# rapidsai/cuvs

Measured on AMD Instinct MI355X. Metric: QPS @ recall@10>=0.9, 100Mx128 fp32 IVF-PQ, batch=10k, higher is better.
Workload: dtype u8 codes, f16 LUT, f32 score; 1 GPU; IVF-PQ 100000000x128 fp32, pq_dim=64 pq_bits=8 n_lists=16384 n_probes=128 batch=10000 k=10; rows and held-out queries from bench.gen_rows (seed 1234 / 4321): Gaussian mixture of 65536 modes ~ N(0, I) in a 32-d latent space, spread 0.35 per mode, embedded in R^128 by a fixed random map + N(0, 0.03^2 I) - NOT SURVEY 8d's generator: the same step on that one is the top-level entry contract_corpus (--; parallelism=single GPU, lut_dtype=f16, internal_distance_dtype=f32

## Files before the change

### cuvs_amd/csrc/common.hpp

```cpp
#pragma once

#include <hip/hip_runtime.h>
#include <hip/hip_fp16.h>

#include <dlpack/dlpack.h>

#include <cstdarg>
#include <cstdint>
#include <cstdio>
#include <cstring>
#include <memory>
#include <stdexcept>
#include <string>
#include <chrono>
#include <vector>

namespace cuvs_amd {

struct error : public std::runtime_error {
  explicit error(const std::string& s) : std::runtime_error(s) {}
};

[[noreturn]] inline void fail(const char* file, int line, const char* fmt, ...)
{
  char buf[1024];
  va_list ap;
  va_start(ap, fmt);
  vsnprintf(buf, sizeof(buf), fmt, ap);
  va_end(ap);
  char out[1200];
  snprintf(out, sizeof(out), "%s (%s:%d)", buf, file, line);
  throw error(out);
}

#define CUVS_EXPECTS(cond, ...)                                              \
  do {                                                                       \
    if (!(cond)) { ::cuvs_amd::fail(__FILE__, __LINE__, __VA_ARGS__); }      \
  } while (0)
#define CUVS_FAIL(...) ::cuvs_amd::fail(__FILE__, __LINE__, __VA_ARGS__)
#define HIP_TRY(expr)                                                                        \
  do {                                                                                       \
    hipError_t e__ = (expr);                                                                 \
    if (e__ != hipSuccess) {                                                                 \
      ::cuvs_amd::fail(__FILE__, __LINE__, "HIP error %d (%s) in %s", (int)e__,              \
                       hipGetErrorString(e__), #expr);                                       \
    }                                                                                        \
  } while (0)

std::string& last_error_text();

template <typename Fn>
int translate_exceptions(Fn&& fn)
{
  try {
    fn();
    return 1;
  } catch (const std::exception& e) {
    last_error_text() = e.what();
    return 0;
  } catch (...) {
    last_error_text() = "unknown exception";
    return 0;
  }
}

struct tuning {
  int pq_head_probes    = -1;
  int pq_scan2          = 1;
  int pq_scan3          = 1;
  int coarse_lowp       = 1;
  int pq_head_rows      = -1;
  int pq_overlap        = 1;
  int coarse_grouped    = 1;
  int pq_filter4        = 1;
  int flat_scan3        = 1;
  int flat_filter2      = 1;
  int flat_bound_head   = 1;
  int pq_wide           = 1;
  int pq_wide_heads     = 0;
  int pq_wide_blocks    = 1;
  bool pq_encode_plain  = false;
  int pq3_surv_cap      = 0;
  int pq_qcap           = 0;
  int scan_debug        = 0;
  int alloc_cache       = 1;
  bool shard_coarse_replicated = false;
  bool bf_fused = false, bf_no_threshold = false, bf_no_fused_filter = false;
  bool bf_host_flags = false;
  bool dist_old         = false;
  int tile_dbg          = 0;
  int flat_head_probes  = -1;
  int cagra_pq_lists = 0, cagra_pq_probes = 0, cagra_kpq = 0, cagra_rank_chunk = 0, prune_dbg = 0;
  bool cagra_auto_multi = false;
  int tiered_path       = 0;
  bool native_format    = false;
  int hnsw_pack_rows    = 0;
  int hnsw_pack_host    = 0;
  int eps_slab_rows     = 0;
};
tuning load_tuning_from_env();

struct resources {
  tuning tune;
  int device              = 0;
  hipStream_t stream      = nullptr;
  bool owns_stream        = false;
  int num_cus             = 256;
  size_t lds_per_block    = 160 * 1024;
  size_t workspace_limit  = size_t(2) << 30;
  size_t ivf_batch_limit  = size_t(8) << 30;
  std::vector<int> mg_devices;
  hipMemPool_t pool       = nullptr;
  hipStream_t aux_stream  = nullptr;
  hipEvent_t aux_events[5] = {nullptr, nullptr, nullptr, nullptr, nullptr};
  bool cagra_guarantee_connectivity = false;
  uint32_t* host_word = nullptr;
  unsigned long long* cagra_work = nullptr;
  struct scratch_cache* cache = nullptr;
};

inline resources* as_res(uintptr_t h)
{
  CUVS_EXPECTS(h != 0, "null cuvsResources_t");
  return reinterpret_cast<resources*>(h);
}

void ensure_aux_stream(resources& res);
void* device_alloc(resources& res, size_t bytes);
void device_free(resources& res, void* p);
void scratch_cache_flush_all();

template <typename T>
struct dev_buf {
  resources* res = nullptr;
  T* ptr         = nullptr;
  size_t n       = 0;
  dev_buf() = default;
  dev_buf(resources& r, size_t count) : res(&r), n(count)
  {
    ptr = count ? static_cast<T*>(device_alloc(r, count * sizeof(T))) : nullptr;
  }
  static dev_buf persistent(size_t count)
  {
    dev_buf b;
    b.n = count;
    if (count) {
      void* p = nullptr;
      if (hipMalloc(&p, count * sizeof(T)) != hipSuccess) {
        (void)hipGetLastError();
        scratch_cache_flush_all();
        HIP_TRY(hipMalloc(&p, count * sizeof(T)));
      }
      b.ptr = static_cast<T*>(p);
    }
    return b;
  }
  dev_buf(const dev_buf&)            = delete;
  dev_buf& operator=(const dev_buf&) = delete;
  dev_buf(dev_buf&& o) noexcept : res(o.res), ptr(o.ptr), n(o.n) { o.ptr = nullptr; o.n = 0; }
  dev_buf& operator=(dev_buf&& o) noexcept
  {
    if (this != &o) {
      release();
      res = o.res; ptr = o.ptr; n = o.n;
      o.ptr = nullptr; o.n = 0;
    }
    return *this;
  }
  ~dev_buf() { release(); }
  void release()
  {
    if (ptr) {
      if (res) device_free(*res, ptr); else (void)hipFree(ptr);
      ptr = nullptr; n = 0;
    }
  }
  T* data() const { return ptr; }
  size_t size() const { return n; }
  size_t bytes() const { return n * sizeof(T); }
};

inline void copy_async(resources& res, void* dst, const void* src, size_t bytes)
{
  if (bytes) HIP_TRY(hipMemcpyAsync(dst, src, bytes, hipMemcpyDefault, res.stream));
}
inline void sync(resources& res) { HIP_TRY(hipStreamSynchronize(res.stream)); }

template <typename T>
std::vector<T> to_host(resources& res, const T* d, size_t n)
{
  std::vector<T> h(n);
  copy_async(res, h.data(), d, n * sizeof(T));
  sync(res);
  return h;
}

inline uint32_t read_word(resources& res, const uint32_t* d)
{
  if (res.host_word == nullptr) HIP_TRY(hipHostMalloc(reinterpret_cast<void**>(&res.host_word), 64));
  HIP_TRY(hipMemcpyAsync(res.host_word, d, sizeof(uint32_t), hipMemcpyDeviceToHost, res.stream));
  sync(res);
  return *res.host_word;
}

struct host_trace {
  bool on;
  const char* what;
  std::vector<std::pair<const char*, std::chrono::steady_clock::time_point>> marks;
  host_trace(bool enabled, const char* name) : on(enabled), what(name) { mark("begin"); }
  void mark(const char* name)
  {
    if (on) marks.emplace_back(name, std::chrono::steady_clock::now());
  }
  ~host_trace()
  {
    if (!on) return;
    mark("buffers freed");
    fprintf(stderr, "[host trace %s]", what);
    for (size_t i = 1; i < marks.size(); ++i)
      fprintf(stderr, " %s %.3f", marks[i].first, std::chrono::duration<double, std::milli>(marks[i].second - marks[i - 1].second).count());
    fprintf(stderr, " | total %.3f ms\n", std::chrono::duration<double, std::milli>(marks.back().second - marks.front().second).count());
  }
};

inline bool is_device_accessible(const DLTensor& t)
// ... 94 lines not shown
```

### cuvs_amd/csrc/core.hip

```cpp
#include <cuvs/version_config.h>
#include "common.hpp"

#include <cuvs/core/c_api.h>

#include "scratch_cache.hpp"

#include <algorithm>
#include <cstdlib>
#include <mutex>
#include <vector>

namespace cuvs_amd {

std::string& last_error_text()
{
  thread_local std::string text;
  return text;
}

namespace {

void* raw_alloc(resources& res, size_t bytes, bool* failed)
{
  void* p = nullptr;
  hipError_t e = res.pool != nullptr ? hipMallocFromPoolAsync(&p, bytes, res.pool, res.stream)
                                     : hipMallocAsync(&p, bytes, res.stream);
  if (e != hipSuccess) {
    (void)hipGetLastError();
    if (failed != nullptr) { *failed = true; return nullptr; }
    HIP_TRY(hipStreamSynchronize(res.stream));
    HIP_TRY(hipMalloc(&p, bytes));
  }
  return p;
}

void raw_free(void* stream_v, void* p)
{
  hipStream_t stream = static_cast<hipStream_t>(stream_v);
  hipError_t e = hipFreeAsync(p, stream);
  if (e != hipSuccess) {
    (void)hipGetLastError();
    (void)hipStreamSynchronize(stream);
    (void)hipFree(p);
  }
}

}

unsigned long long g_pq3_last_stats[6] = {0, 0, 0, 0, 0, 0};

static void flush_cache(scratch_cache& c)
{
  if (!c.caller_stream) { c.flush(raw_free); return; }
  bool drained = false;
  c.flush([&](void*, void* p) {
    if (!drained) { (void)hipDeviceSynchronize(); drained = true; }
    (void)hipFree(p);
    (void)hipGetLastError();
  });
}
void scratch_cache_flush(resources& res)
{
  if (res.cache != nullptr) flush_cache(*res.cache);
}

namespace {
std::mutex g_caches_mu;
std::vector<scratch_cache*> g_caches;
}
void scratch_cache_register(scratch_cache* c, bool add)
{
  std::lock_guard<std::mutex> lk(g_caches_mu);
  if (add) g_caches.push_back(c);
  else g_caches.erase(std::remove(g_caches.begin(), g_caches.end(), c), g_caches.end());
}
void scratch_cache_flush_all()
{
  {
    std::lock_guard<std::mutex> lk(g_caches_mu);
    for (scratch_cache* c : g_caches) flush_cache(*c);
  }
  (void)hipDeviceSynchronize();
  (void)hipGetLastError();
}

void ensure_aux_stream(resources& res)
{
  if (res.aux_stream != nullptr) return;
  int lo = 0, hi = 0;
  HIP_TRY(hipDeviceGetStreamPriorityRange(&lo, &hi));
  HIP_TRY(hipStreamCreateWithPriority(&res.aux_stream, hipStreamNonBlocking, hi));
  for (auto& ev : res.aux_events) HIP_TRY(hipEventCreateWithFlags(&ev, hipEventDisableTiming));
}

void* device_alloc(resources& res, size_t bytes)
{
  if (res.cache == nullptr) return raw_alloc(res, bytes, nullptr);
  return res.cache->alloc(
    res.stream, bytes, [&](size_t n, bool* failed) { return raw_alloc(res, n, failed); }, raw_free);
}

void device_free(resources& res, void* p)
{
  if (!p) return;
  if (res.cache == nullptr) raw_free(res.stream, p);
  else res.cache->release(res.stream, p, raw_free);
}

void fill_dl_view(DLManagedTensor* out, void* data, DLDataType dt, int64_t rows, int64_t cols,
                  int ndim, int device_id)
{
  CUVS_EXPECTS(out != nullptr, "output DLManagedTensor is null");
  out->dl_tensor.data        = data;
  out->dl_tensor.device      = DLDevice{kDLCUDA, device_id};
  out->dl_tensor.ndim        = ndim;
  out->dl_tensor.dtype       = dt;
  out->dl_tensor.shape       = new int64_t[2]{rows, cols};
  out->dl_tensor.strides     = nullptr;
  out->dl_tensor.byte_offset = 0;
  out->manager_ctx           = nullptr;
  out->deleter               = [](DLManagedTensor* self) {
    delete[] self->dl_tensor.shape;
    self->dl_tensor.shape = nullptr;
  };
}

static int g_log_level = CUVS_LOG_LEVEL_INFO;

struct prof_rec {
  std::string name;
  hipEvent_t start, stop;
};
static bool g_prof_on = false;
static std::vector<prof_rec> g_prof;
static std::mutex g_prof_mu;

void profile_begin(resources& res, const char* name)
{
  if (!g_prof_on) return;
  std::lock_guard<std::mutex> lk(g_prof_mu);
  prof_rec r;
  r.name = name;
  HIP_TRY(hipEventCreate(&r.start));
  HIP_TRY(hipEventCreate(&r.stop));
  HIP_TRY(hipEventRecord(r.start, res.stream));
  g_prof.push_back(r);
}
void profile_end(resources& res, const char* name)
{
  if (!g_prof_on) return;
  std::lock_guard<std::mutex> lk(g_prof_mu);
  for (auto it = g_prof.rbegin(); it != g_prof.rend(); ++it)
    if (it->name == name) { HIP_TRY(hipEventRecord(it->stop, res.stream)); return; }
}

static bool debug_switches_on()
{
#ifdef CUVS_AMD_NO_DEBUG_SWITCHES
  return false;
#else
  const char* g = getenv("CUVS_AMD_DEBUG_SWITCHES");
  return g != nullptr && g[0] == '1';
#endif
}

tuning load_tuning_from_env()
{
  tuning t;
  if (!debug_switches_on()) return t;
  auto geti = [](const char* name, int dflt) { const char* e = getenv(name); return e ? atoi(e) : dflt; };
  auto set  = [](const char* name) { return getenv(name) != nullptr; };
  t.pq_head_probes   = geti("CUVS_AMD_PQ_HEAD_PROBES", -1);
  t.pq_scan2         = geti("CUVS_AMD_PQ_SCAN2", 1);
  t.pq_scan3         = geti("CUVS_AMD_PQ_SCAN3", 1);
  t.pq_filter4       = geti("CUVS_AMD_PQ_FILTER4", 1);
  t.coarse_grouped   = geti("CUVS_AMD_COARSE_GROUPED", 1);
  t.pq_overlap       = geti("CUVS_AMD_PQ_OVERLAP", 1);
  t.pq_head_rows     = geti("CUVS_AMD_PQ_HEAD_ROWS", -1);
  t.coarse_lowp      = geti("CUVS_AMD_COARSE_LOWP", 1);
  t.flat_scan3       = geti("CUVS_AMD_FLAT_SCAN3", 1);
  t.flat_filter2     = geti("CUVS_AMD_FLAT_FILTER2", 1);
  t.flat_bound_head  = geti("CUVS_AMD_FLAT_BOUND_HEAD", 1);
  t.pq_wide          = geti("CUVS_AMD_PQ_WIDE", 1);
  t.pq_wide_heads    = geti("CUVS_AMD_PQ_WIDE_HEADS", 0);
  t.pq_wide_blocks   = geti("CUVS_AMD_PQ_WIDE_BLOCKS", 1);
  if (const char* e = getenv("CUVS_AMD_PQ_ENCODE")) t.pq_encode_plain = strcmp(e, "plain") == 0;
  t.pq3_surv_cap     = geti("CUVS_AMD_PQ3_SURV_CAP", 0);
  t.pq_qcap          = geti("CUVS_AMD_PQ_QCAP", 0);
  t.scan_debug       = geti("CUVS_AMD_SCAN_DEBUG", 0);
  t.alloc_cache      = geti("CUVS_AMD_ALLOC_CACHE", 1);
  t.shard_coarse_replicated = set("CUVS_AMD_SHARD_COARSE_REPLICATED");
  t.bf_fused           = set("CUVS_AMD_BF_FUSED");
  t.bf_no_threshold    = set("CUVS_AMD_BF_NO_THRESHOLD");
  t.bf_no_fused_filter = set("CUVS_AMD_BF_NO_FUSED_FILTER");
  t.bf_host_flags = set("CUVS_AMD_BF_HOST_FLAGS");
  t.dist_old           = set("CUVS_AMD_DIST_OLD");
  t.tile_dbg           = geti("CUVS_AMD_TILE_DBG", 0);
  t.flat_head_probes   = geti("CUVS_AMD_FLAT_HEAD_PROBES", -1);
  t.cagra_pq_lists     = geti("CUVS_AMD_CAGRA_PQ_LISTS", 0);
  t.cagra_pq_probes    = geti("CUVS_AMD_CAGRA_PQ_PROBES", 0);
  t.cagra_kpq          = geti("CUVS_AMD_CAGRA_KPQ", 0);
  t.cagra_rank_chunk   = geti("CUVS_AMD_CAGRA_RANK_CHUNK", 0);
  t.prune_dbg          = geti("CUVS_AMD_PRUNE_DBG", 0);
  if (const char* e = getenv("CUVS_AMD_CAGRA_AUTO")) t.cagra_auto_multi = e[0] == 'm';
  if (const char* e = getenv("CUVS_AMD_TIERED_PATH")) t.tiered_path = strcmp(e, "composed") == 0 ? 1 : (strcmp(e, "fused") == 0 ? 2 : 0);
  if (const char* e = getenv("CUVS_AMD_NATIVE_FORMAT")) t.native_format = e[0] == '1';
  t.hnsw_pack_rows   = geti("CUVS_AMD_HNSW_PACK_ROWS", 0);
  t.hnsw_pack_host   = geti("CUVS_AMD_HNSW_PACK_HOST", 0);
  t.eps_slab_rows    = geti("CUVS_AMD_EPS_SLAB_ROWS", 0);
  return t;
}

}

using namespace cuvs_amd;

extern "C" {

const char* cuvsGetLastErrorText()
{
  auto& t = last_error_text();
  return t.empty() ? nullptr : t.c_str();
}

void cuvsSetLastErrorText(const char* error) { last_error_text() = error ? error : ""; }

cuvsLogLevel_t cuvsGetLogLevel() { return (cuvsLogLevel_t)g_log_level; }
void cuvsSetLogLevel(cuvsLogLevel_t l) { g_log_level = (int)l; }

cuvsError_t cuvsResourcesCreate(cuvsResources_t* res)
{
  return (cuvsError_t)translate_exceptions([=] {
    CUVS_EXPECTS(res != nullptr, "res is null");
    auto* r = new resources();
    int dev = 0;
    HIP_TRY(hipGetDevice(&dev));
    r->device = dev;
    hipDeviceProp_t prop;
    HIP_TRY(hipGetDeviceProperties(&prop, dev));
    r->num_cus       = prop.multiProcessorCount;
    r->lds_per_block = prop.sharedMemPerBlock;
    HIP_TRY(hipStreamCreateWithFlags(&r->stream, hipStreamDefault));
    r->owns_stream = true;
    r->tune = load_tuning_from_env();
    {
      size_t free_b = 0, total_b = 0;
      if (hipMemGetInfo(&free_b, &total_b) == hipSuccess && free_b > 0)
        r->ivf_batch_limit = std::max<size_t>(size_t(256) << 20, std::min<size_t>(r->ivf_batch_limit, free_b / 4));
      else
        (void)hipGetLastError();
    }
    if (const char* ws = debug_switches_on() ? getenv("CUVS_AMD_WORKSPACE_MB") : nullptr) {
      long mb = atol(ws);
      if (mb > 0) r->workspace_limit = r->ivf_batch_limit = (size_t)mb << 20;
    }
    hipMemPoolProps props{};
    props.allocType     = hipMemAllocationTypePinned;
    props.handleTypes   = hipMemHandleTypeNone;
    props.location.type = hipMemLocationTypeDevice;
    props.location.id   = dev;
    if (hipMemPoolCreate(&r->pool, &props) == hipSuccess) {
      uint64_t thresh = UINT64_MAX;
      (void)hipMemPoolSetAttribute(r->pool, hipMemPoolAttrReleaseThreshold, &thresh);
    } else {
      r->pool = nullptr;
    }
    (void)hipGetLastError();
    if (r->tune.alloc_cache != 0) {
      r->cache         = new scratch_cache();
      scratch_cache_register(r->cache, true);
      r->cache->stream = r->stream;
      size_t free_b = 0, total_b = 0;
      if (hipMemGetInfo(&free_b, &total_b) != hipSuccess) { (void)hipGetLastError(); total_b = size_t(64) << 30; }
      r->cache->cap_bytes = std::min<size_t>(total_b / 8, size_t(16) << 30);
      if (const char* mb = debug_switches_on() ? getenv("CUVS_AMD_ALLOC_CACHE_MB") : nullptr) r->cache->cap_bytes = (size_t)std::max(0L, atol(mb)) << 20;
    }
    *res = reinterpret_cast<uintptr_t>(r);
  });
}

static std::mutex g_handle_teardown_mu;

cuvsError_t cuvsResourcesDestroy(cuvsResources_t res)
{
  return (cuvsError_t)translate_exceptions([=] {
    auto* r = as_res(res);
    (void)hipStreamSynchronize(r->stream);
    std::lock_guard<std::mutex> teardown(g_handle_teardown_mu);
    if (r->aux_stream != nullptr) {
      (void)hipStreamSynchronize(r->aux_stream);
      (void)hipStreamDestroy(r->aux_stream);
      for (auto& e : r->aux_events) if (e != nullptr) (void)hipEventDestroy(e);
    }
    if (r->cagra_work != nullptr) (void)hipFree(r->cagra_work);
    if (r->host_word != nullptr) (void)hipHostFree(r->host_word);
    if (r->cache != nullptr) {
      scratch_cache_flush(*r);
      (void)hipStreamSynchronize(r->stream);
      scratch_cache_register(r->cache, false);
      delete r->cache;
      r->cache = nullptr;
    }
    if (r->pool != nullptr) (void)hipMemPoolDestroy(r->pool);
    if (r->owns_stream && r->stream) (void)hipStreamDestroy(r->stream);
    delete r;
  });
}

cuvsError_t cuvsStreamSet(cuvsResources_t res, cudaStream_t stream)
{
  return (cuvsError_t)translate_exceptions([=] {
    auto* r = as_res(res);
    if (r->cache != nullptr) {
      scratch_cache_flush(*r);
      if (r->owns_stream) HIP_TRY(hipStreamSynchronize(r->stream));
    }
    if (r->owns_stream && r->stream) {
      HIP_TRY(hipStreamSynchronize(r->stream));
      HIP_TRY(hipStreamDestroy(r->stream));
    }
    r->stream      = reinterpret_cast<hipStream_t>(stream);
    r->owns_stream = false;
    if (r->cache != nullptr) {
      std::lock_guard<std::mutex> lk(r->cache->mu);
      r->cache->stream        = r->stream;
      r->cache->caller_stream = true;
    }
  });
}

// ... 197 lines not shown
```

### cuvs_amd/csrc/ivf_pq_filter4.hip

```cpp
#include "ivf_pq_filter_common.hpp"

#include <cfloat>
#include <type_traits>

namespace cuvs_amd {

namespace {

struct bprep_params {
  const uint32_t* sorted_pairs;
  const uint32_t* pair_off;
  uint32_t n_lists;
  uint32_t lbase;
  const uint32_t* probes;
  const float* rot_queries;
  const float* centers_rot;
  const uint32_t* query_kth;
  uint32_t* qflag;
  uint4* bq;
  float* thr;
  uint32_t n_probes, rot_dim;
  float sc, c1, eps, alpha, cbmax, dmax, bound_max;
  int is_ip, flat;
  uint32_t lpl;
  float4* norms;
};

template <int NST, int PART>
__global__ __launch_bounds__(256) void pq_bprep_kernel(const bprep_params a)
{
  constexpr uint32_t LPP = 2 * NST <= 2 ? 2u : 2 * NST <= 4 ? 4u : 2 * NST <= 8 ? 8u : 2 * NST <= 16 ? 16u : 32u;
  constexpr uint32_t PPW = 64u / LPP;
  const uint32_t s_base = a.pair_off[a.lbase], s_end = a.pair_off[a.lbase + a.n_lists];
  const uint32_t lane = threadIdx.x & 63u, slot = lane % LPP, st = slot >> 1, h = slot & 1u;
  const uint32_t w0 = (blockIdx.x * 4u + (threadIdx.x >> 6)) * 32u;
  if (s_base + w0 >= s_end) return;
  const uint32_t d0 = ((16u * (st >> a.lpl) + 8u * h) << a.lpl) + 8u * (st & ((1u << a.lpl) - 1u));
#pragma unroll 2
  for (uint32_t pass = 0; pass < 32u / PPW; ++pass) {
    const uint32_t s  = s_base + w0 + pass * PPW + lane / LPP;
    const bool pair_ok = s < s_end;
    const bool valid  = pair_ok && slot < 2u * NST;
    const uint32_t p  = a.sorted_pairs[pair_ok ? s : s_end - 1u];
    const uint32_t q  = p / a.n_probes, L = a.probes[p];
    float rn = 0.f, big = 0.f, qc = 0.f, cn = 0.f;
    if (valid) {
      const float* rq = a.rot_queries + (size_t)q * a.rot_dim + d0;
      const float* ct = a.centers_rot + (size_t)L * a.rot_dim + d0;
      const float4 q0 = *reinterpret_cast<const float4*>(rq), q1 = *reinterpret_cast<const float4*>(rq + 4);
      float r[8] = {q0.x, q0.y, q0.z, q0.w, q1.x, q1.y, q1.z, q1.w};
      const float4 c0 = *reinterpret_cast<const float4*>(ct), c1 = *reinterpret_cast<const float4*>(ct + 4);
      const float c[8] = {c0.x, c0.y, c0.z, c0.w, c1.x, c1.y, c1.z, c1.w};
      if (!a.is_ip) {
#pragma unroll
        for (int e = 0; e < 8; ++e) r[e] -= c[e];
      } else {
#pragma unroll
        for (int e = 0; e < 8; ++e) { qc = __fmaf_rn(r[e], c[e], qc); cn = __fmaf_rn(c[e], c[e], cn); }
      }
      f16x8_t v;
#pragma unroll
      for (int e = 0; e < 8; ++e) {
        rn   = __fmaf_rn(r[e], r[e], rn);
        const float x = a.sc * r[e];
        big  = fmaxf(big, fabsf(x));
        v[e] = (_Float16)fminf(fmaxf(x, -60000.f), 60000.f);
      }
      a.bq[(size_t)(s - s_base) * NST * 2 + slot] = __builtin_bit_cast(uint4, v);
    }
#pragma unroll
    for (uint32_t o = 1; o < LPP; o <<= 1) {
      rn += __shfl_xor(rn, o); qc += __shfl_xor(qc, o); cn += __shfl_xor(cn, o);
      big = fmaxf(big, __shfl_xor(big, o));
    }
    if (!pair_ok || slot != 0u) continue;
    if constexpr (PART == 1) {
      a.norms[s - s_base] = make_float4(rn, cn, qc, big);
    } else {
      const uint32_t kk = a.query_kth[q];
      const float bound = key_to_float(kk);
      const bool served = kk < 0xff800000u && big < 60000.f && fabsf(bound) <= a.bound_max;
      if (!a.flat && !served) a.qflag[q] = 1u;
      const float t = a.is_ip ? filter_threshold_ip(bound, rn, cn, qc, a) : filter_threshold(bound, rn, a);
      a.thr[s - s_base] = served ? t / a.c1 : (a.flat ? -INFINITY : INFINITY);
    }
  }
}

__global__ __launch_bounds__(256) void pq_thr_kernel(const bprep_params a)
{
  const uint32_t s_base = a.pair_off[a.lbase], s_end = a.pair_off[a.lbase + a.n_lists];
  const uint32_t s = s_base + blockIdx.x * 256u + threadIdx.x;
  if (s >= s_end) return;
  const uint32_t q  = a.sorted_pairs[s] / a.n_probes;
  const float4 nm   = a.norms[s - s_base];
  const float rn = nm.x, cn = nm.y, qc = nm.z, big = nm.w;
  const uint32_t kk = a.query_kth[q];
  const float bound = key_to_float(kk);
  const bool served = kk < 0xff800000u && big < 60000.f && fabsf(bound) <= a.bound_max;
  if (!a.flat && !served) a.qflag[q] = 1u;
  const float t = a.is_ip ? filter_threshold_ip(bound, rn, cn, qc, a) : filter_threshold(bound, rn, a);
  a.thr[s - s_base] = served ? t / a.c1 : (a.flat ? -INFINITY : INFINITY);
}

constexpr int kF4Threads = 256;
constexpr uint32_t kSurvChunk = 256u;

struct filter4_params {
  const filter_unit* units;
  const uint32_t* n_units;
  uint32_t* xcd_ticket;
  const uint32_t* sorted_pairs;
  const uint32_t* pair_off;
  uint32_t n_lists;
  const uint4* bq;
  const float* thr;
  const uint32_t* cb16;
  const uint8_t* codes;
  const uint32_t* list_offsets;
  const uint32_t* list_sizes;
  const float* row_term;
  uint32_t* qflag;
  uint2* surv;
  uint32_t* surv_cnt;
  uint32_t n_chunks, n_probes, unit_rows;
  unsigned long long* stats;
};

template <int BYTE>
__device__ inline void table_addr(uint32_t& addr, const uint32_t two, const uint32_t w)
{
  if constexpr (BYTE == 0)
    asm("v_lshlrev_b32_sdwa %0, %1, %2 dst_sel:WORD_0 dst_unused:UNUSED_PRESERVE src0_sel:DWORD src1_sel:BYTE_0" : "+v"(addr) : "v"(two), "v"(w));
  else if constexpr (BYTE == 1)
    asm("v_lshlrev_b32_sdwa %0, %1, %2 dst_sel:WORD_0 dst_unused:UNUSED_PRESERVE src0_sel:DWORD src1_sel:BYTE_1" : "+v"(addr) : "v"(two), "v"(w));
  else if constexpr (BYTE == 2)
    asm("v_lshlrev_b32_sdwa %0, %1, %2 dst_sel:WORD_0 dst_unused:UNUSED_PRESERVE src0_sel:DWORD src1_sel:BYTE_2" : "+v"(addr) : "v"(two), "v"(w));
  else
    asm("v_lshlrev_b32_sdwa %0, %1, %2 dst_sel:WORD_0 dst_unused:UNUSED_PRESERVE src0_sel:DWORD src1_sel:BYTE_3" : "+v"(addr) : "v"(two), "v"(w));
}

typedef __attribute__((address_space(3))) const uint32_t lds_u32_t;

template <int NCH, int PL, bool TERM, int DBG, bool STATS = false, bool PC = false>
__global__ __launch_bounds__(kF4Threads) void pq_filter4_kernel(const filter4_params a)
{
  constexpr int NST = PL * NCH;
  constexpr int NGM = NST <= 8 ? 4 : 2;
  constexpr int NGA = 8 / PL;
  constexpr uint32_t kEntry = 2u * PL;
  constexpr uint32_t kSlot  = 256u * kEntry;
  constexpr uint32_t kHalf1 = 65536u;
  extern __shared__ __attribute__((aligned(16))) char smem[];
  uint32_t s_chunk = 0xffffffffu, s_fill = kSurvChunk;
  for (uint32_t i = threadIdx.x; i < (PC ? 0u : (uint32_t)NCH * 16u * (kSlot / 16u)); i += kF4Threads) {
    const uint32_t s = i / (kSlot / 16u), half = (s >> 3) & 1u, slot = (s >> 4) * 8u + (s & 7u);
    *reinterpret_cast<uint4*>(smem + half * kHalf1 + slot * kSlot + (i % (kSlot / 16u)) * 16u) = reinterpret_cast<const uint4*>(a.cb16)[i];
  }
  __syncthreads();

  const uint32_t lane = threadIdx.x & 63u, ql = lane & 31u, h = lane >> 5;
  const uint32_t n_units = *a.n_units;
  const uint32_t chunk   = (n_units + 7u) / 8u;
  const uint32_t s_base  = a.pair_off[a.n_lists];
  uint32_t xcd = blockIdx.x & 7u, hops = 0u;
  const uint32_t two = PL == 1 ? 1u : PL == 2 ? 2u : PL == 4 ? 3u : 4u;
  const uint32_t lane_code_off = ql * 16u + h * 8u, lane_term_off = h * 16u;

  unsigned long long st_pairs = 0, st_surv = 0, st_sub = 0, st_slow = 0, st_units = 0, st_t[3] = {0, 0, 0};
  uint32_t tk_v = 0u;
  uint4 d0 = {0u, 0u, 0u, 0u};
  uint2 d1 = {0u, 0u};
  bool desc_ok = false;
  auto draw_ticket = [&]() {
    if (lane == 0) tk_v = atomicAdd(a.xcd_ticket + xcd * 32, 1u);
  };
  auto load_desc = [&]() {
    const uint32_t share0 = min(n_units, xcd * chunk), share_len = min(chunk, n_units - share0);
    const uint32_t t = __builtin_amdgcn_readfirstlane(tk_v);
    desc_ok = t < share_len;
    if (desc_ok) {
      const filter_unit* up = a.units + share0 + t;
      d0 = *reinterpret_cast<const uint4*>(up);
      d1 = *reinterpret_cast<const uint2*>(reinterpret_cast<const char*>(up) + 16);
    }
  };
  draw_ticket();
  load_desc();
  for (;;) {
    while (!desc_ok) {
      if (++hops == 8u) break;
      xcd = (xcd + 1u) & 7u;
      draw_ticket();
      load_desc();
    }
    if (!desc_ok) break;
    if constexpr (PC) {
      const uint32_t list = __builtin_amdgcn_readfirstlane(d0.x);
      const uint4* src    = reinterpret_cast<const uint4*>(a.cb16) + (size_t)list * (kSlot / 16u);
      char* dst           = smem + (threadIdx.x >> 6) * 4096u;
#pragma unroll
      for (uint32_t i = 0; i < (kSlot / 16u + 63u) / 64u; ++i)
        if (i * 64u + lane < kSlot / 16u) *reinterpret_cast<uint4*>(dst + (i * 64u + lane) * 16u) = src[i * 64u + lane];
    }
    const uint32_t first = __builtin_amdgcn_readfirstlane(d0.y), count = __builtin_amdgcn_readfirstlane(d0.z),
                   row0 = __builtin_amdgcn_readfirstlane(d0.w), base_row = __builtin_amdgcn_readfirstlane(d1.x),
                   r_end = __builtin_amdgcn_readfirstlane(d1.y);
    const uint32_t u0 = row0 >> 5, u1 = (r_end + 31u) >> 5;
    const unsigned long long t_unit = STATS ? __builtin_readcyclecounter() : 0ull;
    unsigned long long t_loop = 0ull;
    draw_ticket();
    bool desc_pending = true;
    const char* code_base = reinterpret_cast<const char*>(a.codes) + (size_t)(base_row >> 6) * NCH * 1024;
    const char* term_base = reinterpret_cast<const char*>(a.row_term + base_row);

    auto load_codes = [&](const uint32_t u, uint2 (&cw)[NCH]) {
      uint32_t uc = min(u, u1 - 1u);
      if constexpr ((DBG & 64) != 0) uc = u0;
      const char* p = code_base + ((size_t)(uc >> 1) * NCH * 1024 + (uc & 1u) * 512u) + lane_code_off;
#pragma unroll
      for (int c = 0; c < NCH; ++c) {
        if constexpr ((DBG & 8) != 0) cw[c] = make_uint2(u * 2654435761u + c, lane);
        else cw[c] = *reinterpret_cast<const uint2*>(p + c * 1024);
      }
    };
    uint32_t ad[NGA];
#pragma unroll
    for (int e = 0; e < NGA; ++e) ad[e] = h << 16;
    auto decode_addr = [&](const uint2 (&cw)[NCH], const int st) {
      const int c = st / PL, b0 = (st % PL) * NGA;
      if constexpr (PC) {
        const uint32_t base = (threadIdx.x >> 6) * 4096u;
#pragma unroll
        for (int e = 0; e < NGA; ++e) {
          const int b = b0 + e;
          const uint32_t w = b < 4 ? cw[c].x : cw[c].y;
          ad[e] = base + (((w >> (8 * (b & 3))) & 255u) << two);
        }
        return;
      }
      if constexpr ((DBG & 1) != 0) {
        const uint32_t w = ql * 0x01010101u;
        if constexpr (NGA >= 1) table_addr<0>(ad[0], two, w);
        if constexpr (NGA >= 2) table_addr<1>(ad[1], two, w);
        if constexpr (NGA >= 4) { table_addr<2>(ad[2], two, w); table_addr<3>(ad[3], two, w); }
        return;
      }
      auto one = [&](const int e) {
        const int b = b0 + e;
        const uint32_t w = b < 4 ? cw[c].x : cw[c].y;
        switch (b & 3) {
          case 0: table_addr<0>(ad[e], two, w); break;
          case 1: table_addr<1>(ad[e], two, w); break;
          case 2: table_addr<2>(ad[e], two, w); break;
          default: table_addr<3>(ad[e], two, w); break;
        }
      };
#pragma unroll
      for (int e = 0; e < NGA; ++e) one(e);
    };
    auto decode_gather = [&](const int st, u32x4_t (&av)[NST]) {
      constexpr uint32_t kNone = 0u;
      const uint32_t slot0 = PC ? 0u : (8u * (st / PL) + (uint32_t)((st % PL) * NGA)) * kSlot;
      constexpr uint32_t kStep = PC ? 0u : kSlot;
      if constexpr ((DBG & 2) != 0) {
#pragma unroll
        for (int e = 0; e < 4; ++e) av[st][e] = ad[e % NGA] + kNone;
        return;
      }
      if constexpr (PL == 1) {
        typedef __attribute__((address_space(3))) const _Float16 lds_f16_t;
        f16x8_t v;
#pragma unroll
        for (int e = 0; e < 8; ++e) v[e] = *reinterpret_cast<lds_f16_t*>(ad[e] + slot0 + e * kStep);
        av[st] = __builtin_bit_cast(u32x4_t, v);
      } else if constexpr (PL == 2) {
#pragma unroll
        for (int e = 0; e < 4; ++e) av[st][e] = *reinterpret_cast<lds_u32_t*>(ad[e] + slot0 + e * kStep);
      } else if constexpr (PL == 4) {
        typedef uint32_t u32x2_t __attribute__((ext_vector_type(2)));
        typedef __attribute__((address_space(3))) const u32x2_t lds_u64_t;
#pragma unroll
        for (int e = 0; e < 2; ++e) {
          const u32x2_t v = *reinterpret_cast<lds_u64_t*>(ad[e] + slot0 + e * kStep);
          av[st][2 * e] = v[0]; av[st][2 * e + 1] = v[1];
        }
      } else {
        typedef __attribute__((address_space(3))) const u32x4_t lds_u128_t;
        av[st] = *reinterpret_cast<lds_u128_t*>(ad[0] + slot0);
      }
    };
    auto decode_step = [&](const uint2 (&cw)[NCH], const int st, u32x4_t (&av)[NST]) {
      decode_addr(cw, st);
      decode_gather(st, av);
    };
    auto load_term = [&](const uint32_t u, f32x16_t& tv) {
      if constexpr (!TERM) { tv = f32x16_t{}; return; }
      uint32_t uc = min(u, u1 - 1u);
      if constexpr ((DBG & 16) != 0) uc = u0;
      const char* p = term_base + (size_t)uc * 128u + lane_term_off;
#pragma unroll
      for (int j = 0; j < 4; ++j) {
        const float4 v = *reinterpret_cast<const float4*>(p + j * 32);
        tv[4 * j] = v.x; tv[4 * j + 1] = v.y; tv[4 * j + 2] = v.z; tv[4 * j + 3] = v.w;
      }
    };

    auto run = [&](auto ng_tag) {
      constexpr int NG = decltype(ng_tag)::value;
      f16x8_t bop[NG][NST];
      float thr[NG];
      uint32_t pairid[NG];
#pragma unroll
      for (int g = 0; g < NG; ++g) {
        const uint32_t jj  = g * 32u + ql;
        const uint32_t jc  = min(jj, count - 1u);
        const uint4* bp    = a.bq + ((size_t)(first - s_base + jc) * NST * 2 + h);
#pragma unroll
        for (int st = 0; st < NST; ++st) bop[g][st] = __builtin_bit_cast(f16x8_t, bp[st * 2]);
        thr[g]    = jj < count ? a.thr[first - s_base + jc] : INFINITY;
        pairid[g] = a.sorted_pairs[first + jc];
      }
      uint2 cw[4][NCH];
      u32x4_t av[2][NST];
      f32x16_t tv[2], acc[2][NG];
#pragma unroll
      for (int k = 0; k < 4; ++k) load_codes(u0 + k, cw[k]);
      load_term(u0, tv[0]);
      load_term(u0 + 1, tv[1]);
#pragma unroll
      for (int g = 0; g < NG; ++g)
#pragma unroll
        for (int st = 0; st < NST; ++st) {
          asm volatile("" : "+a"(bop[g][st]));
        }
#pragma unroll
      for (int st = 0; st < NST; ++st) decode_step(cw[0], st, av[0]);
      load_codes(u0 + 4, cw[0]);
      if (STATS) t_loop = __builtin_readcyclecounter();

      unsigned long long gmask[NG];
      auto screen_group = [&](const f32x16_t (&ac)[NG], const int g, const bool valid) {
        float m = fmaxf(fmaxf(ac[g][0], ac[g][1]), ac[g][2]);
#pragma unroll
        for (int i = 3; i < 15; i += 2) m = fmaxf(fmaxf(m, ac[g][i]), ac[g][i + 1]);
        m        = fmaxf(m, ac[g][15]);
        gmask[g] = valid ? __ballot(m >= thr[g]) : 0ull;
      };
      auto screen_finish = [&](const f32x16_t (&ac)[NG], const uint32_t u, const bool valid) {
        unsigned long long any_mask = 0ull;
#pragma unroll
        for (int g = 0; g < NG; ++g) any_mask |= gmask[g];
        if (STATS && valid) { st_pairs += 32u * count; st_sub += 1u; }
        if (any_mask == 0ull) return;
        if (STATS) st_slow += 1u;
#pragma unroll
        for (int g = 0; g < NG; ++g) {
          if (gmask[g] == 0ull) continue;
          uint32_t hits = 0u;
#pragma unroll
          for (int i = 0; i < 16; ++i) hits |= (ac[g][i] >= thr[g] ? 1u : 0u) << i;
          unsigned long long lm = gmask[g];
          while (lm != 0ull) {
            const uint32_t src = (uint32_t)__ffsll((long long)lm) - 1u;
            lm &= lm - 1ull;
            uint32_t hb        = __builtin_amdgcn_readlane(hits, src);
            const uint32_t pid = __builtin_amdgcn_readlane(pairid[g], src);
            while (hb != 0u) {
              const uint32_t i = (uint32_t)__ffs((int)hb) - 1u;
              hb &= hb - 1u;
              const uint32_t v = (u << 5) + (i & 3u) + 8u * (i >> 2) + 4u * (src >> 5);
              if (v >= r_end) continue;
              if (s_fill == kSurvChunk) {
                uint32_t c = 0u;
                if (lane == 0u) c = atomicAdd(a.surv_cnt, 1u);
                s_chunk = __builtin_amdgcn_readfirstlane(c);
                s_fill  = 0u;
              }
              if (s_chunk < a.n_chunks) {
                if (lane == 0u) a.surv[(size_t)s_chunk * kSurvChunk + s_fill] = make_uint2(pid, base_row + v);
              } else if (lane == 0u) {
                a.qflag[pid / a.n_probes] = 1u;
              }
              s_fill += 1u;
              if (STATS) st_surv += 1u;
            }
          }
        }
      };
      auto step = [&](auto p_tag, const uint32_t u) {
        constexpr int P = decltype(p_tag)::value;
        constexpr int C = P & 1, N = (P + 1) & 1, S = (P + 1) & 3;
        const bool prev = u > u0 && u <= u1;
        auto part_chunk = [](const int p) { return p + 1 < NST ? p + 1 : NST - 1; };
#pragma unroll
        for (int st = 0; st < NST; ++st) {
          const f16x8_t aop = __builtin_bit_cast(f16x8_t, av[C][st]);
          auto mfma = [&](const int g) {
            if constexpr ((DBG & 4) != 0) {
              if (st == 0) acc[C][g] = tv[C];
              acc[C][g][st & 15] += (float)aop[0] * (float)bop[g][st][0];
            } else {
              acc[C][g] = __builtin_amdgcn_mfma_f32_32x32x16_f16(aop, bop[g][st], st == 0 ? tv[C] : acc[C][g], 0, 0, 0);
            }
            __builtin_amdgcn_sched_barrier(0);
          };
          mfma(0);
          if (st == 1) load_term(u + 2, tv[C]);
          decode_addr(cw[S], st);
          __builtin_amdgcn_sched_barrier(0);
          if constexpr (NG >= 2) mfma(1);
          decode_gather(st, av[N]);
          if (st == NST - 1) load_codes(u + 5, cw[S]);
          __builtin_amdgcn_sched_barrier(0);
          if constexpr (NG >= 3) mfma(2);
#pragma unroll
          for (int p = 0; p < NG; ++p)
            if (part_chunk(p) == st) screen_group(acc[N], p, prev);
          if (part_chunk(NG) == st) screen_finish(acc[N], u - 1u, prev);
          __builtin_amdgcn_sched_barrier(0);
          if constexpr (NG >= 4) mfma(3);
        }
        if constexpr (NST == 1) load_term(u + 2, tv[C]);
      };
      using P0 = std::integral_constant<int, 0>; using P1 = std::integral_constant<int, 1>;
      using P2 = std::integral_constant<int, 2>; using P3 = std::integral_constant<int, 3>;
      uint32_t u = u0;
      for (; u < u1; u += 4u) {
        step(P0{}, u);
        step(P1{}, u + 1u);
        step(P2{}, u + 2u);
        step(P3{}, u + 3u);
        if (desc_pending && u >= u0 + 4u) { load_desc(); desc_pending = false; }
      }
      if (u == u1) {
#pragma unroll
        for (int g = 0; g < NG; ++g) screen_group(acc[1], g, true);
        screen_finish(acc[1], u - 1u, true);
      }
    };
    if (u0 < u1) {
      const uint32_t ng = (count + 31u) >> 5;
      if constexpr (NGM == 4) {
        if (ng >= 4u) run(std::integral_constant<int, 4>{});
        else if (ng == 3u) run(std::integral_constant<int, 3>{});
        else if (ng == 2u) run(std::integral_constant<int, 2>{});
        else run(std::integral_constant<int, 1>{});
      } else {
        if (ng >= 2u) run(std::integral_constant<int, 2>{});
        else run(std::integral_constant<int, 1>{});
      }
    }
    if (desc_pending) load_desc();
    if (STATS) {
      const unsigned long long t_end = __builtin_readcyclecounter();
      st_t[0] += t_loop - t_unit;
      st_t[1] += t_end - t_loop;
      st_units += 1u;
    }
  }
  if (STATS && lane == 0) {
    atomicAdd(&a.stats[1], st_surv);
    atomicAdd(&a.stats[0], st_pairs); atomicAdd(&a.stats[2], st_sub);
    atomicAdd(&a.stats[3], st_slow);  atomicAdd(&a.stats[4], st_t[0]); atomicAdd(&a.stats[5], st_t[1]);
    atomicAdd(&a.stats[6], st_t[2]);  atomicAdd(&a.stats[7], st_units);
  }
  if (s_chunk < a.n_chunks)
    for (uint32_t i = s_fill + lane; i < kSurvChunk; i += 64u) a.surv[(size_t)s_chunk * kSurvChunk + i] = make_uint2(0xffffffffu, 0u);
}

}

void pq4_filter(resources& res, const filter4_launch& l)
{
  bprep_params b{};
  b.sorted_pairs = l.sorted_pairs; b.pair_off = l.pair_off; b.n_lists = l.n_lists; b.probes = l.probes;
  b.rot_queries = l.rot_queries; b.centers_rot = l.centers_rot; b.query_kth = l.query_kth; b.qflag = l.qflag;
  b.bq = static_cast<uint4*>(l.bq); b.thr = l.thr; b.n_probes = l.n_probes; b.rot_dim = l.rot_dim;
  b.sc = l.sc; b.c1 = l.c1; b.eps = l.eps; b.alpha = l.alpha; b.cbmax = l.cbmax; b.dmax = l.dmax; b.bound_max = l.bound_max;
  b.is_ip = l.is_ip; b.flat = l.flat; b.lbase = l.head_labels ? 0u : l.n_lists;
  b.lpl = l.pl == 1 ? 0u : l.pl == 2 ? 1u : l.pl == 4 ? 2u : 3u;
  const int nst = l.nch * l.pl;
  const unsigned pgrid = (unsigned)grid_blocks(l.n_pairs, 128);
  b.norms = static_cast<float4*>(l.pair_norms);
  if (l.stage != 2) {
    profile_begin(res, "pq_bprep_kernel");
    auto prep = [&](auto nst_tag) {
      constexpr int N = decltype(nst_tag)::value;
      if (l.stage == 1) hipLaunchKernelGGL((pq_bprep_kernel<N, 1>), dim3(pgrid), dim3(256), 0, res.stream, b);
      else              hipLaunchKernelGGL((pq_bprep_kernel<N, 0>), dim3(pgrid), dim3(256), 0, res.stream, b);
    };
    switch (nst) {
#ifndef CUVS_AMD_F4_DEV
      case 1: prep(std::integral_constant<int, 1>{}); break;
      case 2: prep(std::integral_constant<int, 2>{}); break;
      case 3: prep(std::integral_constant<int, 3>{}); break;
      case 4: prep(std::integral_constant<int, 4>{}); break;
      case 5: prep(std::integral_constant<int, 5>{}); break;
      case 6: prep(std::integral_constant<int, 6>{}); break;
      case 7: prep(std::integral_constant<int, 7>{}); break;
      case 10: prep(std::integral_constant<int, 10>{}); break;
      case 12: prep(std::integral_constant<int, 12>{}); break;
      case 14: prep(std::integral_constant<int, 14>{}); break;
      case 16: prep(std::integral_constant<int, 16>{}); break;
#endif
      default: prep(std::integral_constant<int, 8>{}); break;
    }
    profile_end(res, "pq_bprep_kernel");
    HIP_TRY(hipGetLastError());
    if (l.stage == 1 || l.bprep_only) return;
  } else {
    hipLaunchKernelGGL(pq_thr_kernel, dim3((unsigned)grid_blocks(l.n_pairs, 256)), dim3(256), 0, res.stream, b);
  }
  filter4_params g{};
  g.units = l.units; g.n_units = l.n_units; g.xcd_ticket = l.xcd_ticket; g.sorted_pairs = l.sorted_pairs; g.pair_off = l.pair_off;
  g.n_lists = l.n_lists; g.bq = b.bq; g.thr = l.thr; g.cb16 = l.cb16; g.codes = l.codes; g.list_offsets = l.list_offsets;
  g.list_sizes = l.list_sizes; g.row_term = l.row_term; g.qflag = l.qflag; g.surv = static_cast<uint2*>(l.surv);
  g.surv_cnt = l.surv_cnt; g.n_chunks = l.surv_entries / kSurvChunk; g.n_probes = l.n_probes; g.unit_rows = l.unit_rows;
  g.stats = l.stats;
  const size_t fsmem = l.per_cluster ? 4 * 4096 : 65536 + (size_t)l.nch * 8 * 512 * l.pl;
  const bool term = l.row_term != nullptr;
  auto launch = [&](auto kern) {
    HIP_TRY(hipFuncSetAttribute(reinterpret_cast<const void*>(kern), hipFuncAttributeMaxDynamicSharedMemorySize, (int)fsmem));
    profile_begin(res, "pq_filter_kernel");
    hipLaunchKernelGGL(kern, dim3(l.grid), dim3(kF4Threads), fsmem, res.stream, g);
    profile_end(res, "pq_filter_kernel");
  };
#ifndef CUVS_AMD_F4_DEV
  if (l.nch == 4 && l.pl == 2 && !l.per_cluster) {
    switch (l.dbg) {
      case 1:  launch(pq_filter4_kernel<4, 2, true, 1>); break;
      case 2:  launch(pq_filter4_kernel<4, 2, true, 2>); break;
      case 4:  launch(pq_filter4_kernel<4, 2, true, 4>); break;
      case 8:  launch(pq_filter4_kernel<4, 2, true, 8>); break;
      case 16: launch(pq_filter4_kernel<4, 2, true, 16>); break;
      case 64: launch(pq_filter4_kernel<4, 2, true, 64>); break;
      case 80: launch(pq_filter4_kernel<4, 2, true, 80>); break;
      case 81: launch(pq_filter4_kernel<4, 2, true, 81>); break;
      default:
        if (l.stats != nullptr && term) launch(pq_filter4_kernel<4, 2, true, 0, true>);
        else if (term) launch(pq_filter4_kernel<4, 2, true, 0>);
        else launch(pq_filter4_kernel<4, 2, false, 0>);
        break;
    }
    return;
  }
  auto pick = [&](auto nch_tag, auto pl_tag) {
    constexpr int N = decltype(nch_tag)::value, P = decltype(pl_tag)::value;
    if (l.per_cluster) {
      if (term) launch(pq_filter4_kernel<N, P, true, 0, false, true>); else launch(pq_filter4_kernel<N, P, false, 0, false, true>);
    } else {
      if (term) launch(pq_filter4_kernel<N, P, true, 0>); else launch(pq_filter4_kernel<N, P, false, 0>);
    }
  };
  using N1 = std::integral_constant<int, 1>; using N2 = std::integral_constant<int, 2>; using N3 = std::integral_constant<int, 3>;
  using N4 = std::integral_constant<int, 4>; using N5 = std::integral_constant<int, 5>; using N6 = std::integral_constant<int, 6>;
  using N7 = std::integral_constant<int, 7>; using N8 = std::integral_constant<int, 8>;
  CUVS_EXPECTS(nst >= 1 && nst <= 16 && l.nch >= 1 && l.nch <= 8, "ivf_pq: shape outside the matrix-core filter (pq3_supported)");
  if (l.pl == 2) {
    switch (l.nch) {
      case 1: pick(N1{}, N2{}); break;
      case 2: pick(N2{}, N2{}); break;
      case 3: pick(N3{}, N2{}); break;
      case 4: pick(N4{}, N2{}); break;
      case 5: pick(N5{}, N2{}); break;
      case 6: pick(N6{}, N2{}); break;
      case 7: pick(N7{}, N2{}); break;
      default: pick(N8{}, N2{}); break;
    }
  } else if (l.pl == 1) {
    switch (l.nch) {
      case 1: pick(N1{}, N1{}); break;
      case 2: pick(N2{}, N1{}); break;
      case 3: pick(N3{}, N1{}); break;
      case 4: pick(N4{}, N1{}); break;
      case 5: pick(N5{}, N1{}); break;
      case 6: pick(N6{}, N1{}); break;
      case 7: pick(N7{}, N1{}); break;
      default: pick(N8{}, N1{}); break;
    }
  } else if (l.pl == 4) {
    switch (l.nch) {
      case 1: pick(N1{}, N4{}); break;
      case 2: pick(N2{}, N4{}); break;
      case 3: pick(N3{}, N4{}); break;
      default: pick(N4{}, N4{}); break;
    }
  } else {
    if (l.nch == 1) pick(N1{}, N8{}); else pick(N2{}, N8{});
  }
#else
  launch(pq_filter4_kernel<4, 2, true, 0>);
#endif
}

}
```

### cuvs_amd/csrc/ivf_pq_filter_common.hpp

```cpp
#pragma once
#include "ivf_pq.hpp"
#include "device_utils.hpp"

#include <cmath>

namespace cuvs_amd {

typedef _Float16 f16x8_t __attribute__((ext_vector_type(8)));
typedef float f32x16_t __attribute__((ext_vector_type(16)));
typedef uint32_t u32x4_t __attribute__((ext_vector_type(4)));

struct filter_unit {
  uint32_t list, first, count, row0;
  uint32_t base_row, r_end;
  uint32_t pad0, pad1;
};

template <typename P>
__device__ inline float filter_threshold(const float bound, const float rn, const P& a)
{
  const double mabs = 1.1920929e-07  / (double)a.sc *
                      (sqrt((double)a.rot_dim * (double)rn) + (double)a.rot_dim * (double)a.cbmax);
  const double b = ((double)bound + (double)a.alpha) * (1.0 + 2.0 * (double)a.eps) + mabs - (double)rn * (1.0 - 1.0 / 512.0);
  float f = (float)b;
  f += fabsf(f) * 2.4e-7f + 1e-37f;
  return f;
}

template <typename P>
__device__ inline float filter_threshold_ip(const float bound, const float qn, const float cn, const float qc, const P& a)
{
  const double nq = sqrt((double)qn), nc = sqrt((double)cn);
  const double mabs = 1.1920929e-07  / (double)a.sc * (sqrt((double)a.rot_dim) * nq + (double)a.rot_dim * (double)a.cbmax);
  const double m = nq * (((double)a.eps + 7.63e-6) * nc + ((double)a.eps + 1.0 / 512.0) * (double)a.dmax);
  const double b = (double)bound + (double)qc + (fabs((double)qc) + fabs((double)bound)) * 1e-6 + m + mabs + (double)a.alpha;
  float f = (float)b;
  f += fabsf(f) * 2.4e-7f + 1e-37f;
  return f;
}


struct filter4_launch {
  const filter_unit* units;
  const uint32_t* n_units;
  uint32_t* xcd_ticket;
  const uint32_t* sorted_pairs;
  const uint32_t* pair_off;
  uint32_t n_lists;
  const uint32_t* probes;
  const float* rot_queries;
  const float* centers_rot;
  const uint32_t* query_kth;
  uint32_t* qflag;
  void* bq;
  float* thr;
  const uint32_t* cb16;
  const uint8_t* codes;
  const uint32_t* list_offsets;
  const uint32_t* list_sizes;
  const float* row_term;
  void* surv;
  uint32_t* surv_cnt;
  uint32_t surv_entries, n_probes, rot_dim, unit_rows;
  float sc, c1, eps, alpha, cbmax, dmax, bound_max;
  int is_ip, dbg, nch, pl, per_cluster;
  int64_t n_pairs;
  unsigned long long* stats;
  unsigned grid;
  int stage = 0;
  void* pair_norms = nullptr;
  int flat = 0;
  int bprep_only = 0;
  int head_labels = 0;
};
void pq4_filter(resources& res, const filter4_launch& l);

bool pqw_shape(uint32_t rot_dim);
uint32_t pqw_group();
void pqw_decode(resources& res, const uint8_t* codes8, uint32_t n_chunks, const uint32_t* cb16, uint32_t pq_len, int64_t padded_rows,
                uint32_t rot_dim, void* rows16);
struct wide_prep {
  const uint32_t* sorted_pairs;
  const uint32_t* pair_off;
  uint32_t n_lists;
  const uint32_t* probes;
  const float* rot_queries;
  const float* centers_rot;
  const uint32_t* query_kth;
  uint32_t* qflag;
  void* bq;
  uint32_t* blk_off;
  float* thr;
  void* norms;
  uint32_t n_probes, rot_dim, heads;
  float sc, c1, eps, alpha, cbmax, dmax, bound_max;
  int head;
  int is_ip;
  int flat = 0;
  int64_t n_pairs;
};
void pqw_bprep(resources& res, const wide_prep& l);
struct wide_filter {
  const filter_unit* units;
  const uint32_t* n_units;
  uint32_t* xcd_ticket;
  const uint32_t* sorted_pairs;
  const uint32_t* pair_off;
  uint32_t n_lists;
  const void* bq;
  const uint32_t* blk_off;
  const float* thr;
  const void* rows16;
  const float* row_term;
  const float* zeros;
  const uint32_t* filter_bits;
  const int64_t* indices;
  uint32_t* qflag;
  void* surv;
  uint32_t* surv_cnt;
  uint32_t surv_cap, spill_cap, n_probes, rot_dim;
  float* xbuf;
  uint32_t ldx, heads;
  int emit;
  unsigned grid;
  unsigned long long* stats;
  uint32_t* fail = nullptr;
  const char* profile_name = nullptr;
};
void pqw_filter(resources& res, const wide_filter& l);

}
```

### cuvs_amd/csrc/ivf_pq_scan3.hip

```cpp
#include "ivf_pq.hpp"
#include "ops.hpp"
#include "device_utils.hpp"
#include "ivf_common.hpp"
#include "pq_lut_math.hpp"
#include "ivf_pq_scan3.hpp"
#include "ivf_pq_filter_common.hpp"

#include <cfloat>
#include <cmath>
#include <cstring>
#include <map>
#include <mutex>
#include <type_traits>
#include <utility>

namespace cuvs_amd {

namespace {

constexpr int kFThreads = 512;
constexpr int kFWaves   = kFThreads / 64;



__global__ void cb16_kernel(const float* __restrict__ pq_centers, uint32_t pq_dim, uint32_t pq_len, uint32_t book, float sc,
                            uint16_t* __restrict__ cb16)
{
  const uint32_t e = blockIdx.x * blockDim.x + threadIdx.x;
  if (e >= pq_dim * 256u) return;
  const uint32_t s = e >> 8, code = e & 255u;
  for (uint32_t l = 0; l < pq_len; ++l)
    cb16[(size_t)e * pq_len + l] =
      code < book ? __builtin_bit_cast(uint16_t, (_Float16)(sc * pq_centers[(size_t)(s * pq_len + l) * book + code])) : (uint16_t)0;
}

__global__ void cbt_kernel(const float* __restrict__ pq_centers, uint32_t pq_dim, uint32_t pq_len, uint32_t book, float* __restrict__ cbt)
{
  const uint32_t e = blockIdx.x * blockDim.x + threadIdx.x;
  if (e >= pq_dim * 256u) return;
  const uint32_t s = e >> 8, code = e & 255u;
  for (uint32_t l = 0; l < pq_len; ++l) cbt[(size_t)e * pq_len + l] = code < book ? pq_centers[(size_t)(s * pq_len + l) * book + code] : 0.f;
}

__global__ void expand_codes_kernel(const uint8_t* __restrict__ codes, int64_t rows, uint32_t n_chunks, uint32_t cpc, uint32_t bits,
                                    uint32_t pq_dim, uint8_t* __restrict__ out)
{
  const uint32_t nch8 = pq_dim / 16;
  const int64_t i = (int64_t)blockIdx.x * blockDim.x + threadIdx.x;
  if (i >= rows * nch8) return;
  const int64_t row = i / nch8;
  const uint32_t c8 = (uint32_t)(i % nch8);
  uint32_t w[4] = {0u, 0u, 0u, 0u};
#pragma unroll
  for (int b = 0; b < 16; ++b) {
    const uint32_t s = c8 * 16 + b, ch = s / cpc, bit = (s % cpc) * bits;
    const uint8_t* base = codes + ((size_t)(row >> 6) * n_chunks + ch) * 1024 + (size_t)(row & 63) * 16;
    uint32_t v = base[bit >> 3];
    if ((bit & 7) + bits > 8) v |= (uint32_t)base[(bit >> 3) + 1] << 8;
    w[b >> 2] |= ((v >> (bit & 7)) & ((1u << bits) - 1u)) << ((b & 3) * 8);
  }
  reinterpret_cast<uint4*>(out)[((size_t)(row >> 6) * nch8 + c8) * 64 + (row & 63)] = make_uint4(w[0], w[1], w[2], w[3]);
}

__device__ inline float wave_reduce_max_f32(float v)
{
#pragma unroll
  for (int off = 32; off > 0; off >>= 1) v = fmaxf(v, __shfl_xor(v, off));
  return v;
}

__global__ void row_term_kernel(const uint8_t* __restrict__ codes, const float* __restrict__ pq_centers, int64_t rows, float sc,
                                uint32_t* __restrict__ term, uint32_t* __restrict__ dn_max_bits, int n_chunks, int fp32, int pq_len,
                                uint32_t book, const uint32_t* __restrict__ list_offsets, uint32_t n_lists)
{
  const int64_t r0 = (int64_t)blockIdx.x * blockDim.x + threadIdx.x;
  const int64_t r  = min(r0, rows - 1);
  uint32_t L = 0u;
  if (list_offsets != nullptr) {
    uint32_t lo = 0u, hi = n_lists;
    while (hi - lo > 1u) {
      const uint32_t mid = (lo + hi) >> 1;
      if ((int64_t)list_offsets[mid] <= r) lo = mid; else hi = mid;
    }
    L = lo;
  }
  const uint4* cp = reinterpret_cast<const uint4*>(codes) + ((size_t)(r >> 6) * n_chunks) * 64 + (r & 63);
  float dn = 0.f;
  for (int c = 0; c < n_chunks; ++c) {
    const uint4 cw       = cp[c * 64];
    const uint32_t ws[4] = {cw.x, cw.y, cw.z, cw.w};
#pragma unroll
    for (int b = 0; b < 16; ++b) {
      const uint32_t code = (ws[b >> 2] >> ((b & 3) * 8)) & 0xffu;
      const uint32_t s    = c * 16 + b;
      for (int l = 0; l < pq_len; ++l) {
        const float p = pq_centers[(size_t)((list_offsets != nullptr ? L : s) * pq_len + l) * book + code];
        dn = __fmaf_rn(p, p, dn);
      }
    }
  }
  const float wmax = wave_reduce_max_f32(dn);
  if ((threadIdx.x & 63) == 0) atomicMax(dn_max_bits, __float_as_uint(wmax));
  const float x     = -0.5f * sc * sc * (dn * (1.0f - 1.0f / 512.0f));
  const _Float16 hi = (_Float16)x;
  const _Float16 lo = (_Float16)(x - (float)hi);
  if (r0 < rows)
    term[r] = fp32 ? __float_as_uint(x) : ((uint32_t)__builtin_bit_cast(uint16_t, hi) | ((uint32_t)__builtin_bit_cast(uint16_t, lo) << 16));
}


__global__ __launch_bounds__(1024) void count_units_kernel(const uint32_t* __restrict__ pair_off, uint32_t n_lists,
                                                           const uint32_t* __restrict__ list_sizes, uint32_t unit_rows,
                                                           uint32_t* __restrict__ unit_off, uint32_t group, uint32_t lbase)
{
  __shared__ int smem[17];
  const uint32_t per = (n_lists + 1023u) / 1024u;
  const uint32_t b = threadIdx.x * per, e = min(n_lists, b + per);
  auto units_of = [&](uint32_t i) {
    const uint32_t np = pair_off[lbase + i + 1] - pair_off[lbase + i];
    const uint32_t len = list_sizes[i];
    return (int)(((np + group - 1u) / group) * ((len + unit_rows - 1u) / unit_rows));
  };
  int s = 0;
  for (uint32_t i = b; i < e; ++i) s += units_of(i);
  int total;
  int run = block_exclusive_scan(s, smem, &total);
  for (uint32_t i = b; i < e; ++i) {
    unit_off[i] = (uint32_t)run;
    run += units_of(i);
  }
  if (threadIdx.x == 0) unit_off[n_lists] = (uint32_t)total;
}

__global__ void fill_units_kernel(const uint32_t* __restrict__ pair_off, uint32_t n_lists,
                                  const uint32_t* __restrict__ list_offsets, const uint32_t* __restrict__ list_sizes,
                                  uint32_t unit_rows, const uint32_t* __restrict__ unit_off, filter_unit* __restrict__ units,
                                  uint32_t group, uint32_t lbase)
{
  const uint32_t L = blockIdx.x * blockDim.x + threadIdx.x;
  if (L >= n_lists) return;
  const uint32_t b = pair_off[lbase + L], e = pair_off[lbase + L + 1], len = list_sizes[L];
  uint32_t w = unit_off[L];
  if (b == e || len == 0u) return;
  const uint32_t n_ch = (len + unit_rows - 1u) / unit_rows;
  const uint32_t rows = ((len + n_ch - 1u) / n_ch + 63u) & ~63u;
  const uint32_t base = list_offsets[L];
  for (uint32_t c = 0; c < n_ch; ++c) {
    const uint32_t r0 = c * rows, r1 = min(len, r0 + rows);
    if (r0 >= r1) continue;
    for (uint32_t p = b; p < e; p += group) units[w++] = filter_unit{L, p, min(group, e - p), r0, base, r1, 0u, 0u};
  }
  const uint32_t w_end = unit_off[L] + ((e - b + group - 1u) / group) * n_ch;
  for (; w < w_end; ++w) units[w] = filter_unit{L, b, 1u, 0u, base, 0u, 0u, 0u};
}

struct filter_params {
  const filter_unit* units;
  const uint32_t* n_units;
  uint32_t* xcd_ticket;
  const uint32_t* sorted_pairs;
  const float* rot_queries;
  const float* centers_rot;
  const uint32_t* cb16;
  const uint8_t* codes;
  const uint32_t* list_offsets;
  const uint32_t* list_sizes;
  const uint32_t* row_term;
  const uint32_t* query_kth;
  uint32_t* qflag;
  uint2* surv;
  uint32_t* surv_cnt;
  uint32_t surv_cap;
  uint32_t spill_cap;
  uint32_t n_probes, rot_dim, unit_rows;
  float sc;
  float c1;
  float eps, alpha;
  float cbmax, dmax;
  float bound_max;
  int is_ip;
  unsigned long long* stats;
  int dbg;
  const uint4* rows16;
  uint32_t* fail;
  const uint4* bq;
  const float* thr_pair;
  const uint32_t* pair_off;
  uint32_t n_lists;
  float* xbuf;
  uint32_t ldx, lbase;
};

template <int NCH, int DBG, bool FLAT = false>
__global__ __launch_bounds__(kFThreads) void pq_filter_kernel(const filter_params a)
{
  constexpr int NST = 2 * NCH;
  constexpr int NG  = NCH <= 4 ? 2 : 1;
  extern __shared__ __attribute__((aligned(16))) char smem[];
  uint32_t* cb = reinterpret_cast<uint32_t*>(smem);
  uint32_t* wg_fill = reinterpret_cast<uint32_t*>(smem + (FLAT ? 0 : NCH * 16 * 1024));
  uint2* my_surv    = a.surv + (size_t)blockIdx.x * a.surv_cap;
  if (threadIdx.x == 0) *wg_fill = 0u;
  if constexpr (!FLAT)
    for (uint32_t i = threadIdx.x; i < (uint32_t)NCH * 16u * 256u / 4u; i += kFThreads)
      reinterpret_cast<uint4*>(cb)[i] = reinterpret_cast<const uint4*>(a.cb16)[i];
  __syncthreads();

  const int lane = threadIdx.x & 63;
  const uint32_t ql = (uint32_t)lane & 31u, h = (uint32_t)lane >> 5;
  const uint32_t* cbh = cb + h * (8u * 256u);

  const uint32_t n_units = *a.n_units;
  const uint32_t chunk = (n_units + 7u) / 8u;
  uint32_t xcd = blockIdx.x & 7u, hops = 0u;
  const uint4* codes16 = reinterpret_cast<const uint4*>(a.codes);

  unsigned long long st_pairs = 0, st_surv = 0, st_sub = 0, st_slow = 0, st_units = 0, st_t[3] = {0, 0, 0};
  for (;;) {
    const uint32_t share0 = min(n_units, xcd * chunk), share_len = min(chunk, n_units - share0);
    const filter_unit* share = a.units + share0;
    uint32_t t = 0;
    if (lane == 0) t = atomicAdd(a.xcd_ticket + xcd * 32, 1u);
    t = __builtin_amdgcn_readfirstlane(t);
    if (t >= share_len) {
      if (++hops == 8u) break;
      xcd = (xcd + 1u) & 7u;
      continue;
    }
    const uint4 uu = *reinterpret_cast<const uint4*>(share + t);
    const uint32_t L = __builtin_amdgcn_readfirstlane(uu.x), first = __builtin_amdgcn_readfirstlane(uu.y),
                   count = __builtin_amdgcn_readfirstlane(uu.z), row0 = __builtin_amdgcn_readfirstlane(uu.w);
    const uint32_t base_row = a.list_offsets[L], len = a.list_sizes[L];
    const bool two = NG == 2 && count > 32u;
    const unsigned long long t_unit = a.stats != nullptr ? __builtin_readcyclecounter() : 0ull;
    unsigned long long t_slow = 0ull;

    f16x8_t bop[NG][NST];
    float thr[2] = {INFINITY, INFINITY};
    uint32_t pairid[2] = {0u, 0u};
#pragma unroll
    for (int g = 0; g < NG; ++g) {
      const uint32_t jj = g * 32u + ql;
      const bool valid  = jj < count;
      const uint32_t p  = valid ? a.sorted_pairs[first + jj] : 0u;
      const uint32_t q  = p / a.n_probes;
      pairid[g]         = p;
      const float* rq   = a.rot_queries + (size_t)q * a.rot_dim;
      const float* ct   = a.centers_rot + (size_t)L * a.rot_dim;
      float rn = 0.f, big = 0.f, qc = 0.f, cn = 0.f;
#pragma unroll
      for (int st = 0; st < NST; ++st) {
        const uint32_t s0 = 16u * (st >> 1) + 8u * h + 4u * (st & 1);
        const float4 q0 = *reinterpret_cast<const float4*>(rq + 2 * s0), q1 = *reinterpret_cast<const float4*>(rq + 2 * s0 + 4);
        float r[8] = {q0.x, q0.y, q0.z, q0.w, q1.x, q1.y, q1.z, q1.w};
        const float4 c0 = *reinterpret_cast<const float4*>(ct + 2 * s0), c1 = *reinterpret_cast<const float4*>(ct + 2 * s0 + 4);
        const float c[8] = {c0.x, c0.y, c0.z, c0.w, c1.x, c1.y, c1.z, c1.w};
        if (!a.is_ip) {
#pragma unroll
          for (int e = 0; e < 8; ++e) r[e] -= c[e];
        } else {
#pragma unroll
          for (int e = 0; e < 8; ++e) { qc = __fmaf_rn(r[e], c[e], qc); cn = __fmaf_rn(c[e], c[e], cn); }
        }
        f16x8_t v;
#pragma unroll
        for (int e = 0; e < 8; ++e) {
          rn   = __fmaf_rn(r[e], r[e], rn);
          const float x = a.sc * r[e];
          big  = fmaxf(big, fabsf(x));
          v[e] = (_Float16)fminf(fmaxf(x, -60000.f), 60000.f);
        }
        bop[g][st] = v;
      }
      rn  += __shfl_xor(rn, 32);
      qc  += __shfl_xor(qc, 32);
      cn  += __shfl_xor(cn, 32);
      big  = fmaxf(big, __shfl_xor(big, 32));
      const uint32_t kk = valid ? a.query_kth[q] : 0u;
      const float bound = key_to_float(kk);
      const bool served = valid && kk < 0xff800000u && big < 60000.f && fabsf(bound) <= a.bound_max && (FLAT || a.qflag[q] == 0u);
      if (!FLAT && valid && !served) a.qflag[q] = 1u;
      const float t = a.is_ip ? filter_threshold_ip(bound, rn, cn, qc, a) : filter_threshold(bound, rn, a);
      thr[g] = served ? t / a.c1 : ((FLAT && valid) ? -INFINITY : INFINITY);
    }
    const u32x4_t oq   = {h == 0u ? 0x3c003c00u : 0u, 0u, 0u, 0u};
    const f16x8_t ones = __builtin_bit_cast(f16x8_t, oq);

    const uint32_t r_end = __builtin_amdgcn_readfirstlane(share[t].r_end);
    const uint32_t u0 = row0 >> 5, u1 = (r_end + 31u) >> 5;
    auto load_codes = [&](const uint32_t u, uint2 (&cw)[NCH]) {
      const uint32_t fr = base_row + (min(u, u1 - 1u) << 5) + ql;
      const char* p = reinterpret_cast<const char*>(codes16 + ((size_t)(fr >> 6) * NCH) * 64 + (fr & 63u)) + 8u * h;
#pragma unroll
      for (int c = 0; c < NCH; ++c) {
        if constexpr ((DBG & 8) != 0) cw[c] = make_uint2(u * 2654435761u + c, fr);
        else cw[c] = *reinterpret_cast<const uint2*>(p + (size_t)c * 64 * 16);
      }
    };
    auto decode = [&](const uint2 (&cw)[NCH], u32x4_t (&av)[NST]) {
#pragma unroll
      for (int st = 0; st < NST; ++st) {
        const uint32_t w = (st & 1) ? cw[st >> 1].y : cw[st >> 1].x;
#pragma unroll
        for (int e = 0; e < 4; ++e) {
          uint32_t code = (w >> (8 * e)) & 0xffu;
          if constexpr ((DBG & 1) != 0) code = ql;
          av[st][e] = (DBG & 2) ? code : cbh[((16u * (st >> 1) + 4u * (st & 1) + e) << 8) + code];
        }
      }
    };
    auto load_rows = [&](const uint32_t u, u32x4_t (&av)[NST]) {
      const uint4* p = a.rows16 + ((size_t)((base_row >> 5) + min(u, u1 - 1u)) * NST) * 64 + lane;
#pragma unroll
      for (int st = 0; st < NST; ++st) {
        const uint4 v = p[(size_t)st * 64];
        av[st] = u32x4_t{v.x, v.y, v.z, v.w};
      }
    };
    auto run = [&](auto two_tag) {
      constexpr bool TWO = decltype(two_tag)::value;
      constexpr bool DOUBLE = NCH <= 4;
      uint2 cw1[NCH], cw2[NCH];
      u32x4_t avA[NST], avB[DOUBLE ? NST : 1];
      if constexpr (FLAT) {
        load_rows(u0, avA);
      } else {
        load_codes(u0, cw1);
        load_codes(u0 + 1, cw2);
        decode(cw1, avA);
#pragma unroll
        for (int c = 0; c < NCH; ++c) cw1[c] = cw2[c];
        load_codes(u0 + 2, cw2);
      }
      auto step = [&](const uint32_t u, u32x4_t (&cur)[NST], auto& nxt) {
        uint32_t term = 0u;
        if (a.row_term != nullptr && h == 0u) term = a.row_term[base_row + (u << 5) + ql];
        if constexpr (FLAT) {
          if constexpr (DOUBLE) load_rows(u + 1, nxt);
        } else if constexpr (DOUBLE) {
          decode(cw1, nxt);
#pragma unroll
          for (int c = 0; c < NCH; ++c) cw1[c] = cw2[c];
          load_codes(u + 3, cw2);
        }
        f32x16_t acc0 = {}, acc1 = {};
#pragma unroll
        for (int st = 0; st < NST; ++st) {
          const f16x8_t aop = __builtin_bit_cast(f16x8_t, cur[st]);
          if constexpr ((DBG & 4) != 0) { acc0[st] += (float)aop[0]; continue; }
          acc0 = __builtin_amdgcn_mfma_f32_32x32x16_f16(aop, bop[0][st], acc0, 0, 0, 0);
          if constexpr (TWO) acc1 = __builtin_amdgcn_mfma_f32_32x32x16_f16(aop, bop[NG - 1][st], acc1, 0, 0, 0);
        }
        if constexpr (!DOUBLE) {
          if constexpr (FLAT) {
            load_rows(u + 1, cur);
          } else {
            decode(cw1, cur);
#pragma unroll
            for (int c = 0; c < NCH; ++c) cw1[c] = cw2[c];
            load_codes(u + 3, cw2);
          }
        }
        if (a.row_term != nullptr) {
          const u32x4_t tq  = {term, 0u, 0u, 0u};
          const f16x8_t top = __builtin_bit_cast(f16x8_t, tq);
          acc0 = __builtin_amdgcn_mfma_f32_32x32x16_f16(top, ones, acc0, 0, 0, 0);
          if constexpr (TWO) acc1 = __builtin_amdgcn_mfma_f32_32x32x16_f16(top, ones, acc1, 0, 0, 0);
        }
        float m0 = -INFINITY, m1 = -INFINITY;
#pragma unroll
        for (int i = 0; i < 16; ++i) {
          m0 = fmaxf(m0, acc0[i]);
          if constexpr (TWO) m1 = fmaxf(m1, acc1[i]);
        }
        const bool any = (m0 >= thr[0]) || (TWO && m1 >= thr[1]);
        if (a.stats != nullptr) { st_pairs += 32u * count; st_sub += 1u; }
        if (__ballot(any) == 0ull) return;
        if (a.stats != nullptr) st_slow += 1u;
        const unsigned long long t_s0 = a.stats != nullptr ? __builtin_readcyclecounter() : 0ull;
        if (any) {
#pragma unroll
          for (int g = 0; g < (TWO ? 2 : 1); ++g)
#pragma unroll
            for (int i = 0; i < 16; ++i) {
              const uint32_t v = (u << 5) + (uint32_t)((i & 3) + 8 * (i >> 2)) + 4u * h;
              const float x    = g == 0 ? acc0[i] : acc1[i];
              if (x >= thr[g] && v < r_end) {
                const uint32_t pos = atomicAdd(wg_fill, 1u);
                if (pos < a.surv_cap) {
                  my_surv[pos] = make_uint2(pairid[g], base_row + v);
                } else {
                  const uint32_t sp = atomicAdd(a.surv_cnt + gridDim.x, 1u);
                  if (sp < a.spill_cap) a.surv[(size_t)gridDim.x * a.surv_cap + sp] = make_uint2(pairid[g], base_row + v);
                  else if (FLAT) *a.fail = 1u;
                  else a.qflag[pairid[g] / a.n_probes] = 1u;
                }
                if (a.stats != nullptr) st_surv += 1u;
              }
            }
        }
        if (a.stats != nullptr) t_slow += __builtin_readcyclecounter() - t_s0;
      };
      if constexpr (DOUBLE) {
        for (uint32_t u = u0; u < u1; u += 2) {
          step(u, avA, avB);
          if (u + 1 < u1) step(u + 1, avB, avA);
        }
      } else {
        for (uint32_t u = u0; u < u1; ++u) step(u, avA, avA);
      }
    };
    const unsigned long long t_loop = a.stats != nullptr ? __builtin_readcyclecounter() : 0ull;
    if (u0 < u1) {
      if (two) run(std::true_type{}); else run(std::false_type{});
    }
    if (a.stats != nullptr) {
      const unsigned long long t_end = __builtin_readcyclecounter();
      st_t[0] += t_loop - t_unit;
      st_t[1] += t_end - t_loop;
      st_t[2] += t_slow;
      st_units += 1u;
    }
  }
  if (a.stats != nullptr) atomicAdd(&a.stats[1], st_surv);
  if (a.stats != nullptr && lane == 0) {
    atomicAdd(&a.stats[0], st_pairs); atomicAdd(&a.stats[2], st_sub);
    atomicAdd(&a.stats[3], st_slow);  atomicAdd(&a.stats[4], st_t[0]); atomicAdd(&a.stats[5], st_t[1]);
    atomicAdd(&a.stats[6], st_t[2]);  atomicAdd(&a.stats[7], st_units);
  }
  __syncthreads();
  if (threadIdx.x == 0) a.surv_cnt[blockIdx.x] = min(*wg_fill, a.surv_cap);
}

constexpr int kF2Threads = 256;
constexpr int kF2Waves   = kF2Threads / 64;

template <int NST, bool EMIT = false>
__global__ __launch_bounds__(kF2Threads, 2) void flat_filter2_kernel(const filter_params a)
{
  constexpr int NGM      = 8;
  constexpr bool DOUBLE  = NST <= 8;
// ... 1868 lines not shown
    const uint32_t s = s0 + lane;
    float d = INFINITY;
    uint32_t rk = 0xffffffffu, row = 0xffffffffu;
    if (s < n) {
      d   = cand_d[o + s];
      row = cand_i[o + s];
      rk  = (flagged || s < head * k) ? s / k : cand_r[o + s];
    } else if (s < n + n_ov) {
      const uint4 e = overflow[ov0 + s - n];
      d = __uint_as_float(e.y); rk = e.z; row = e.w;
    }
    unsigned long long m = __ballot(row != 0xffffffffu && top3<E>::before(d, rk, row, kd, krk, krow));
    while (m != 0ull) {
      const int src = (int)__ffsll((long long)m) - 1;
      m &= m - 1ull;
      const float cd    = __uint_as_float(__builtin_amdgcn_readlane(__float_as_uint(d), src));
      const uint32_t cr = __builtin_amdgcn_readlane(rk, src), cw = __builtin_amdgcn_readlane(row, src);
      if (top3<E>::before(cd, cr, cw, kd, krk, krow)) {
        best.insert(cd, cr, cw, lane);
        best.at(kr, kd, krk, krow);
      }
    }
  }
  wave_top<E> out;
  out.init();
  for (int r = 0; r < (int)k; ++r) {
    float cd = 0.f;
    uint32_t cr = 0u, cw = 0xffffffffu;
    best.at(r, cd, cr, cw);
    if (cw == 0xffffffffu) break;
    out.insert(cd, cw, lane);
  }
#pragma unroll
  for (int e = 0; e < E; ++e) {
    const int r = e * 64 + lane;
    if (r < (int)k) {
      const bool ok = out.i[e] != 0xffffffffu;
      top_d[q * k + r] = ok ? out.d[e] : FLT_MAX;
      top_i[q * k + r] = ok ? out.i[e] : 0xffffffffu;
    }
  }
}

}

unsigned pq3_grid(const resources& res) { return (unsigned)std::max(8, res.num_cus / 8 * 8); }
unsigned pq3_regions(const resources& res) { return 2 * pq3_grid(res); }

bool pq3_supported(const ivf_pq_index& idx, int k)
{
  return idx.pq_bits >= 4 && idx.pq_bits <= 8 && (idx.pq_len == 1 || idx.pq_len == 2 || idx.pq_len == 4 || idx.pq_len == 8) && idx.pq_dim % 16 == 0 &&
         idx.pq_dim >= 16 && idx.pq_dim <= 128 && idx.rot_dim == idx.pq_len * idx.pq_dim && idx.rot_dim <= 256 &&
         k <= 256;
}

bool pq3_bound_useful(const ivf_pq_index& idx, int k)
{
  uint64_t rows = 0, lists = 0;
  if (idx.shard_world > 1 && idx.shard_comm != nullptr) {
    if (!idx.shard_stats_valid) return k <= 128;
    rows = idx.shard_global_rows; lists = idx.shard_global_lists;
  } else {
    for (uint32_t v : idx.h_list_sizes) { rows += v; lists += v != 0u; }
  }
  return lists != 0 && (uint64_t)k * 25u * lists <= rows;
}

static std::recursive_mutex g_pq3_mu;

const uint8_t* pq3_codes(resources& res, const ivf_pq_index& idx, uint32_t* n_chunks)
{
  *n_chunks = idx.pq_dim / 16;
  if (idx.pq_bits == 8) return idx.codes.data();
  std::lock_guard<std::recursive_mutex> lock(g_pq3_mu);
  auto& c = idx.scan3;
  if (c.codes8_src != idx.codes.data() || c.codes8_rows != idx.padded_rows || c.codes8_size != idx.size) {
    const int64_t rows = std::max<int64_t>(idx.padded_rows, 1);
    c.codes8 = dev_buf<uint8_t>::persistent((size_t)rows * idx.pq_dim);
    if (idx.padded_rows > 0)
      hipLaunchKernelGGL(expand_codes_kernel, dim3(grid_blocks(idx.padded_rows * (int64_t)(idx.pq_dim / 16), 256)), dim3(256), 0, res.stream,
                         idx.codes.data(), idx.padded_rows, idx.n_chunks, idx.codes_per_chunk, idx.pq_bits, idx.pq_dim, c.codes8.data());
    c.codes8_src = idx.codes.data(); c.codes8_rows = idx.padded_rows; c.codes8_size = idx.size;
  }
  return c.codes8.data();
}

pq3_tables pq3_prepare(resources& res, const ivf_pq_index& idx, const bool term_fp32)
{
  std::lock_guard<std::recursive_mutex> lock(g_pq3_mu);
  auto& c = idx.scan3;
  if (c.codes_ptr != idx.codes.data() || c.rows != idx.padded_rows || c.size != idx.size || c.pq_ptr != idx.pq_centers.data() ||
      c.term_fp32 != term_fp32) {
    std::vector<float> h = to_host(res, idx.pq_centers.data(), idx.pq_centers.size());
    float mx = 0.f;
    for (float v : h) mx = std::max(mx, std::fabs(v));
    c.sc    = mx > 0.f ? std::exp2(std::floor(std::log2(16.0f / mx))) : 1.0f;
    c.cbmax = mx;
    const uint32_t n_tables = idx.codebook_kind == 0 ? idx.pq_dim : idx.n_lists;
    c.cb16  = dev_buf<uint32_t>::persistent((size_t)n_tables * 256 * idx.pq_len / 2 + 1);
    hipLaunchKernelGGL(cb16_kernel, dim3(grid_blocks((int64_t)n_tables * 256, 256)), dim3(256), 0, res.stream,
                       idx.pq_centers.data(), n_tables, idx.pq_len, idx.pq_book, c.sc, reinterpret_cast<uint16_t*>(c.cb16.data()));
    c.row_term = dev_buf<uint32_t>::persistent((size_t)std::max<int64_t>(idx.padded_rows, 1));
    dev_buf<uint32_t> mxd(res, 1);
    HIP_TRY(hipMemsetAsync(mxd.data(), 0, sizeof(uint32_t), res.stream));
    uint32_t nch8 = 0;
    const uint8_t* codes8 = pq3_codes(res, idx, &nch8);
    if (idx.padded_rows > 0)
      hipLaunchKernelGGL(row_term_kernel, dim3(grid_blocks(idx.padded_rows, 256)), dim3(256), 0, res.stream, codes8,
                         idx.pq_centers.data(), idx.padded_rows, c.sc, c.row_term.data(), mxd.data(), (int)nch8, term_fp32 ? 1 : 0,
                         (int)idx.pq_len, idx.pq_book, idx.codebook_kind == 0 ? nullptr : idx.list_offsets.data(), idx.n_lists);
    const uint32_t mbits = to_host(res, mxd.data(), 1)[0];
    float dn_max;
    memcpy(&dn_max, &mbits, 4);
    c.dmax = std::sqrt(dn_max) * 1.0001f;
    c.codes_ptr = idx.codes.data(); c.rows = idx.padded_rows; c.size = idx.size; c.pq_ptr = idx.pq_centers.data();
    c.term_fp32 = term_fp32;
  }
  return pq3_tables{c.cb16.data(), c.row_term.data(), c.sc, c.cbmax, c.dmax};
}

size_t pq3_max_units(const ivf_pq_index& idx, int64_t n_pairs, uint32_t* unit_rows, bool filter4)
{
  uint32_t max_len = 0;
  for (uint32_t v : idx.h_list_sizes) max_len = std::max(max_len, v);
  const uint32_t ur = std::max<uint32_t>(filter4 ? 8192u : 4096u, (uint32_t)round_up((int64_t)(max_len + 15) / 16, 64));
  *unit_rows = ur;
  return (size_t)16 * ((size_t)n_pairs / 32 + idx.n_lists + 1);
}

void pq3_warm(resources& res, const ivf_pq_index& idx, bool filter4)
{
  uint32_t n_chunks = 0;
  (void)pq3_codes(res, idx, &n_chunks);
  (void)pq3_prepare(res, idx, filter4);
}

void pq3_tail(resources& res, const ivf_pq_index& idx, const pq3_run& r)
{
  const bool f4 = r.bq != nullptr;
  CUVS_EXPECTS(r.stage == 0 || f4, "ivf_pq: the two-stream schedule is pq_filter4_kernel's");
  const pq3_tables tb = pq3_prepare(res, idx, f4);
  if (r.stage != 1) profile_begin(res, "pq_scan_kernel");
  const int nch        = (int)idx.pq_dim / 16;
  const int nst        = nch * (int)idx.pq_len;
  const uint32_t group = f4 ? (nst <= 8 ? 128u : 64u) : (nch <= 4 ? 64u : 32u);
  CUVS_EXPECTS(f4 || (idx.pq_len == 2 && idx.codebook_kind == 0), "ivf_pq: pq_filter_kernel decodes pq_len 2, PER_SUBSPACE only");
  auto* units = static_cast<filter_unit*>(r.units);
  if (r.stage != 2) {
    hipLaunchKernelGGL(count_units_kernel, dim3(1), dim3(1024), 0, res.stream, r.pair_off, idx.n_lists, idx.list_sizes.data(),
                       r.unit_rows, r.unit_off, group, idx.n_lists);
    hipLaunchKernelGGL(fill_units_kernel, dim3(grid_blocks(idx.n_lists, 256)), dim3(256), 0, res.stream, r.pair_off, idx.n_lists,
                       idx.list_offsets.data(), idx.list_sizes.data(), r.unit_rows, r.unit_off, units, group, idx.n_lists);
  }
  filter_params f{};
  f.units = units; f.n_units = r.unit_off + idx.n_lists; f.xcd_ticket = r.xcd_ticket;
  f.sorted_pairs = r.sorted_pairs; f.rot_queries = r.rot_queries; f.centers_rot = idx.centers_rot.data();
  uint32_t nch8 = 0;
  const uint8_t* codes8 = pq3_codes(res, idx, &nch8);
  f.cb16 = tb.cb16; f.codes = codes8; f.list_offsets = idx.list_offsets.data(); f.list_sizes = idx.list_sizes.data();
  f.row_term = r.is_ip ? nullptr : tb.row_term; f.query_kth = r.query_kth; f.qflag = r.qflag;
  const unsigned grid = pq3_grid(res);
  const unsigned regions = grid;
  f.surv = static_cast<uint2*>(r.surv); f.surv_cnt = r.surv_cnt; f.surv_cap = (uint32_t)((uint64_t)r.surv_cap * 3 / 4 / regions);
  f.spill_cap = r.surv_cap - f.surv_cap * regions;
  f.n_probes = r.n_probes; f.rot_dim = idx.rot_dim; f.unit_rows = r.unit_rows;
  f.sc = tb.sc; f.c1 = (r.is_ip ? -1.0f : -2.0f) / (tb.sc * tb.sc);
  f.cbmax = tb.cbmax; f.dmax = tb.dmax; f.is_ip = r.is_ip; f.stats = r.stats; f.dbg = r.filter_dbg;
  f.bound_max = FLT_MAX;
  const float ne = std::max(1.0f, (float)idx.pq_dim / 64.0f);
  if (r.lut_mode == 0)      { f.eps = ne / 65536.0f; f.alpha = 0.f; }
  else if (r.lut_mode == 1) { f.eps = r.acc_half ? 0.04f * ne : 1.0f / 1024.0f; f.alpha = ne * 64.0f / 16777216.0f; f.bound_max = 60000.f; }
  else                      { f.eps = r.acc_half ? 0.07f + 0.04f * ne : 0.07f; f.alpha = ne * 64.0f / 32768.0f; f.bound_max = 30000.f; }
  if (r.is_ip && r.lut_mode == 2) f.eps = r.acc_half ? 0.14f + 0.04f * ne : 0.14f;
  const size_t fsmem = (size_t)nch * 16 * 1024 + 16;
  if (f4) {
    filter4_launch l{};
    l.units = units; l.n_units = f.n_units; l.xcd_ticket = r.xcd_ticket; l.sorted_pairs = r.sorted_pairs; l.pair_off = r.pair_off;
    l.n_lists = idx.n_lists; l.probes = r.probes; l.rot_queries = r.rot_queries; l.centers_rot = f.centers_rot;
    l.query_kth = r.query_kth; l.qflag = r.qflag; l.bq = r.bq; l.thr = r.thr; l.cb16 = tb.cb16; l.codes = f.codes;
    l.list_offsets = f.list_offsets; l.list_sizes = f.list_sizes; l.row_term = reinterpret_cast<const float*>(f.row_term);
    l.surv = f.surv; l.surv_cnt = f.surv_cnt; l.surv_entries = r.surv_cap; l.n_probes = r.n_probes;
    l.rot_dim = idx.rot_dim; l.unit_rows = r.unit_rows; l.sc = f.sc; l.c1 = f.c1; l.eps = f.eps; l.alpha = f.alpha;
    l.cbmax = f.cbmax; l.dmax = f.dmax; l.bound_max = f.bound_max; l.is_ip = r.is_ip; l.dbg = r.filter_dbg; l.nch = nch;
    l.pl = (int)idx.pq_len; l.per_cluster = idx.codebook_kind != 0 ? 1 : 0;
    l.n_pairs = r.nq * (int64_t)r.n_probes; l.stats = r.stats; l.grid = grid;
    l.stage = r.stage; l.pair_norms = r.pair_norms;
    pq4_filter(res, l);
    if (r.stage == 1) return;
  } else {
  auto launch_filter = [&](auto kern) {
    HIP_TRY(hipFuncSetAttribute(reinterpret_cast<const void*>(kern), hipFuncAttributeMaxDynamicSharedMemorySize, (int)fsmem));
    profile_begin(res, "pq_filter_kernel");
    hipLaunchKernelGGL(kern, dim3(grid), dim3(kFThreads), fsmem, res.stream, f);
    profile_end(res, "pq_filter_kernel");
  };
  if (nch == 4) {
    switch (r.filter_dbg) {
      case 1:  launch_filter(pq_filter_kernel<4, 1>); break;
      case 2:  launch_filter(pq_filter_kernel<4, 2>); break;
      case 4:  launch_filter(pq_filter_kernel<4, 4>); break;
      default: launch_filter(pq_filter_kernel<4, 0>); break;
    }
  } else {
    switch (nch) {
      case 1: launch_filter(pq_filter_kernel<1, 0>); break;
      case 2: launch_filter(pq_filter_kernel<2, 0>); break;
      case 3: launch_filter(pq_filter_kernel<3, 0>); break;
      case 5: launch_filter(pq_filter_kernel<5, 0>); break;
      case 6: launch_filter(pq_filter_kernel<6, 0>); break;
      case 7: launch_filter(pq_filter_kernel<7, 0>); break;
      default: launch_filter(pq_filter_kernel<8, 0>); break;
    }
  }
  }

  rescore_params s{};
  s.surv = f.surv; s.surv_cnt = r.surv_cnt; s.surv_cap = f.surv_cap; s.spill_cap = f.spill_cap; s.probes = r.probes; s.rot_queries = r.rot_queries;
  s.n_regions = regions; s.sub = f4 ? 0u : 1u;
  if (f4) s.surv_cap = r.surv_cap;
  s.centers_rot = idx.centers_rot.data(); s.pq_centers = idx.pq_centers.data(); s.codes = codes8;
  s.query_kth = r.query_kth; s.qflag = r.qflag; s.qcnt = r.qcnt; s.cand_d = r.cand_d; s.cand_i = r.cand_i; s.cand_r = r.cand_r;
  s.n_probes = r.n_probes; s.rot_dim = idx.rot_dim; s.k = r.k; s.head = r.head; s.is_ip = r.is_ip; s.n_chunks = nch8;
  s.head_rows = r.head_rows; s.list_offsets = idx.list_offsets.data();
  s.filter_bits = r.filter_bits; s.indices = idx.indices.data();
  s.overflow = static_cast<uint4*>(r.overflow); s.overflow_cnt = r.counters + 1; s.overflow_cap = r.overflow_cap; s.fail = nullptr;
  const size_t cb_bytes = (size_t)idx.rot_dim * idx.pq_book * sizeof(float);
  s.pq_len = idx.pq_len; s.book = idx.pq_book; s.per_cluster = idx.codebook_kind != 0 ? 1 : 0;
  s.cb_lds = (cb_bytes <= 128 * 1024 && !s.per_cluster) ? 1 : 0;
  const size_t rsmem = s.cb_lds ? cb_bytes : 16;
  const dim3 rg(f4 && s.cb_lds ? grid : grid + 1, f4 && s.cb_lds ? 1 : 2), rb(kRThreads);
  profile_begin(res, "pq_rescore_kernel");
  auto launch_rescore = [&](auto kern) {
    HIP_TRY(hipFuncSetAttribute(reinterpret_cast<const void*>(kern), hipFuncAttributeMaxDynamicSharedMemorySize, (int)rsmem));
    hipLaunchKernelGGL(kern, rg, rb, rsmem, res.stream, s);
  };
  auto pick_rescore = [&](auto lut_tag, auto acc_tag) {
    constexpr int LUT = decltype(lut_tag)::value;
    constexpr bool ACC = decltype(acc_tag)::value;
    if (s.cb_lds) launch_rescore(pq_rescore_kernel<LUT, ACC, true>); else launch_rescore(pq_rescore_kernel<LUT, ACC, false>);
  };
  using L0 = std::integral_constant<int, 0>; using L1 = std::integral_constant<int, 1>; using L2 = std::integral_constant<int, 2>;
  if (r.lut_mode == 0)      pick_rescore(L0{}, std::false_type{});
  else if (r.lut_mode == 1) { if (r.acc_half) pick_rescore(L1{}, std::true_type{}); else pick_rescore(L1{}, std::false_type{}); }
  else                      { if (r.acc_half) pick_rescore(L2{}, std::true_type{}); else pick_rescore(L2{}, std::false_type{}); }
  profile_end(res, "pq_rescore_kernel");
  hipLaunchKernelGGL(reset_flagged_kernel, dim3((unsigned)r.nq), dim3(256), 0, res.stream, r.qflag, r.nq, r.n_probes, r.k, r.head,
                     r.cand_d, r.cand_i);
  hipLaunchKernelGGL(fallback_items_kernel, dim3(grid * 4), dim3(256), 0, res.stream, r.sorted_pairs, r.pair_off, idx.n_lists,
                     r.probes, r.n_probes, r.qflag, static_cast<work_item*>(r.fb_items), r.counters, 0);
  profile_end(res, "pq_scan_kernel");
}

static size_t head_smem_fixed(const ivf_pq_index& idx, int lut_mode, bool acc_half, int nt, int k)
{
  const bool lut32 = lut_mode == 0 || (lut_mode == 2 && !acc_half);
  return (size_t)idx.pq_dim * 256 * (lut32 ? 4 : 2) + 2 * 256 * 4 + 16 + 32 + 16 + (size_t)nt * 4 + 4 * (size_t)head_cand(k) * 4;
}

static int head_occupancy(const void* fn, int nt, size_t smem)
{
  static std::mutex mu;
  static std::map<std::pair<const void*, size_t>, int> known;
  std::lock_guard<std::mutex> lock(mu);
  auto it = known.find({fn, smem});
  if (it != known.end()) return it->second;
  hipFuncAttributes fa{};
  HIP_TRY(hipFuncGetAttributes(&fa, fn));
  CUVS_EXPECTS(fa.sharedSizeBytes == 0, "ivf_pq: the head kernel's LUT has to sit at LDS address 0");
  int n = 0;
  HIP_TRY(hipOccupancyMaxActiveBlocksPerMultiprocessor(&n, fn, nt, smem));
  CUVS_EXPECTS(n >= 1, "ivf_pq: the head kernel does not fit a CU");
  known[{fn, smem}] = n;
  return n;
}

int pq3_head_scan(resources& res, const ivf_pq_index& idx, const pq3_head& h)
{
  head_params a{};
  a.items = static_cast<const work_item*>(h.items); a.item_begin = h.item_begin; a.item_end = h.item_end; a.n_lists = idx.n_lists;
  a.xcd_ticket = h.xcd_ticket; a.sorted_pairs = h.sorted_pairs; a.rot_queries = h.rot_queries; a.centers_rot = idx.centers_rot.data();
  a.pq_centers = idx.pq_centers.data(); a.codes = pq3_codes(res, idx, &a.n_chunks); a.list_offsets = idx.list_offsets.data();
  a.list_sizes = idx.list_sizes.data(); a.out_d = h.cand_d; a.out_i = h.cand_i; a.query_kth = h.query_kth;
  a.n_probes = h.n_probes; a.rot_dim = idx.rot_dim; a.k = h.k; a.is_ip = h.is_ip; a.pq_dim = idx.pq_dim;
  a.pq_len = idx.pq_len; a.book = idx.pq_book; a.per_cluster = idx.codebook_kind != 0 ? 1 : 0;
  a.filter_bits = h.filter_bits; a.indices = idx.indices.data(); a.stats = h.stats; a.hcand = head_cand((int)h.k);
  const bool lut32 = h.lut_mode == 0 || (h.lut_mode == 2 && !h.acc_half);
  const size_t lut_bytes = (size_t)idx.pq_dim * 256 * (lut32 ? 4 : 2);
  const bool nt512 = lut_bytes <= 64 * 1024;
  const int nt = nt512 ? 512 : 1024;
  const size_t smem = head_smem_fixed(idx, h.lut_mode, h.acc_half != 0, nt, (int)h.k);
  CUVS_EXPECTS(smem <= 160 * 1024 - 64, "ivf_pq: the head-phase LUT does not fit the LDS");
  a.cap_rows = (uint32_t)(kHeadRowsPerThread * nt);
  if (h.max_list_len > 0) a.cap_rows = std::min<uint32_t>(a.cap_rows, (uint32_t)round_up(h.max_list_len, 64));
  a.one_shot          = h.one_shot;
  a.row_limit         = h.row_limit;
  int wgs_per_cu = 0;
  auto go = [&](auto kern) {
    const void* fn = reinterpret_cast<const void*>(kern);
    HIP_TRY(hipFuncSetAttribute(fn, hipFuncAttributeMaxDynamicSharedMemorySize, (int)smem));
    wgs_per_cu = head_occupancy(fn, nt, smem);
    const unsigned grid = h.one_shot != 0u ? h.one_shot : pq3_grid(res) * (unsigned)wgs_per_cu;
    profile_begin(res, "pq_scan_kernel");
    profile_begin(res, "pq_head_kernel");
    hipLaunchKernelGGL(kern, dim3(grid), dim3(nt), smem, res.stream, a);
    profile_end(res, "pq_head_kernel");
    profile_end(res, "pq_scan_kernel");
  };
  auto pick = [&](auto lut_tag, auto acc_tag) {
    constexpr int LUT = decltype(lut_tag)::value;
    constexpr bool ACC = decltype(acc_tag)::value;
    constexpr bool L32 = LUT == 0 || (LUT == 2 && !ACC);
    if (nt512) go(pq_head_kernel<LUT, ACC, 512, L32 ? 4 : 6>); else go(pq_head_kernel<LUT, ACC, 1024, 4>);
  };
  using I0 = std::integral_constant<int, 0>; using I1 = std::integral_constant<int, 1>; using I2 = std::integral_constant<int, 2>;
  if (h.lut_mode == 0)      pick(I0{}, std::false_type{});
  else if (h.lut_mode == 1) { if (h.acc_half) pick(I1{}, std::true_type{}); else pick(I1{}, std::false_type{}); }
  else                      { if (h.acc_half) pick(I2{}, std::true_type{}); else pick(I2{}, std::false_type{}); }
  return wgs_per_cu;
}

bool flat3_wide(uint32_t dim) { return dim > 128 && pqw_shape(dim); }
bool flat3_supported(uint32_t dim, int k) { return ((dim % 32 == 0 && dim >= 32 && dim <= 256) || flat3_wide(dim)) && k <= 128; }

static bool flat3_prepare(resources& res, const flat3_view& v, flat3_cache& c)
{
  static std::mutex mu;
  std::lock_guard<std::mutex> lock(mu);
  if (c.data_ptr == v.data && c.rows == v.padded_rows && c.size == v.size) return true;
  if (c.failed_ptr == v.data && c.failed_rows == v.padded_rows && c.failed_size == v.size) return false;
  const int64_t rows = std::max<int64_t>(v.padded_rows, 64);
  {
    c.rows16   = dev_buf<uint4>();
    c.row_term = dev_buf<uint32_t>();
    c.data_ptr = nullptr;
    size_t free_b = 0, total_b = 0;
    HIP_TRY(hipMemGetInfo(&free_b, &total_b));
    const size_t need = (size_t)rows * v.dim * 2 + (size_t)rows * 16 + (size_t(1) << 30);
    if (free_b < need) {
      scratch_cache_flush_all();
// ... 301 lines not shown
  pqw_margins(idx, r, &eps, &alpha, &bound_max);
  hipLaunchKernelGGL(fill_f32_kernel, dim3(1024), dim3(256), 0, res.stream, hb.xbuf, (size_t)r.nq * r.head * hb.ldx, -INFINITY);
  wide_prep l{};
  l.sorted_pairs = r.sorted_pairs; l.pair_off = r.pair_off; l.n_lists = idx.n_lists; l.probes = r.probes; l.rot_queries = r.rot_queries;
  l.centers_rot = idx.centers_rot.data(); l.query_kth = r.query_kth; l.qflag = r.qflag; l.bq = r.bq; l.thr = hb.head_c; l.norms = hb.norms;
  l.n_probes = r.n_probes; l.rot_dim = idx.rot_dim; l.heads = r.head; l.sc = tb.sc; l.c1 = c1; l.eps = eps; l.alpha = alpha;
  l.cbmax = tb.cbmax; l.dmax = tb.dmax; l.bound_max = bound_max; l.head = 1; l.n_pairs = r.nq * (int64_t)r.head; l.blk_off = hb.blk_off; l.is_ip = r.is_ip;
  pqw_bprep(res, l);
  auto* units = static_cast<filter_unit*>(r.units);
  hipLaunchKernelGGL(count_units_kernel, dim3(1), dim3(1024), 0, res.stream, r.pair_off, idx.n_lists, idx.list_sizes.data(), r.unit_rows,
                     r.unit_off, pqw_group(), 0u);
  hipLaunchKernelGGL(fill_units_kernel, dim3(grid_blocks(idx.n_lists, 256)), dim3(256), 0, res.stream, r.pair_off, idx.n_lists,
                     idx.list_offsets.data(), idx.list_sizes.data(), r.unit_rows, r.unit_off, units, pqw_group(), 0u);
  wide_filter f{};
  f.units = units; f.n_units = r.unit_off + idx.n_lists; f.xcd_ticket = hb.tickets; f.sorted_pairs = r.sorted_pairs; f.pair_off = r.pair_off;
  f.n_lists = idx.n_lists; f.bq = r.bq; f.blk_off = hb.blk_off; f.thr = hb.head_c; f.rows16 = rows16;
  f.row_term = r.is_ip ? nullptr : reinterpret_cast<const float*>(tb.row_term); f.zeros = idx.scan3.zeros.data();
  f.qflag = r.qflag; f.surv = r.surv; f.surv_cnt = r.surv_cnt; f.surv_cap = 0; f.spill_cap = 0; f.n_probes = r.n_probes; f.rot_dim = idx.rot_dim;
  f.xbuf = hb.xbuf; f.ldx = hb.ldx; f.heads = r.head; f.emit = 1; f.grid = pq3_grid(res); f.stats = nullptr;
  f.filter_bits = r.filter_bits; f.indices = idx.indices.data();
  pqw_filter(res, f);
  select_k<uint32_t, uint32_t>(res, hb.xbuf, nullptr, r.nq, (int64_t)r.head * hb.ldx, (int64_t)r.head * hb.ldx, (int)r.k, hb.kth_val, hb.kth_idx,
                               false);
  uint32_t nch8 = 0;
  const uint8_t* codes8 = pq3_codes(res, idx, &nch8);
  wbound_params b{};
  b.rs = pqw_score_inputs(idx, r, codes8, nch8);
  b.kth_val = hb.kth_val; b.kth_idx = hb.kth_idx; b.norms = static_cast<const float4*>(hb.norms); b.probes = r.probes;
  b.list_offsets = idx.list_offsets.data(); b.nq = r.nq; b.k = r.k; b.heads = r.head; b.ldx = hb.ldx; b.n_probes = r.n_probes;
  b.rot_dim = idx.rot_dim; b.query_kth = const_cast<uint32_t*>(r.query_kth); b.qflag = r.qflag; b.thr_head = hb.thr_head;
  b.sc = tb.sc; b.c1 = c1; b.eps = eps; b.alpha = alpha; b.cbmax = tb.cbmax; b.dmax = tb.dmax; b.bound_max = bound_max; b.is_ip = r.is_ip;
  const dim3 bgrid((unsigned)grid_blocks(r.nq, 4));
  const bool bblocks = idx.pq_len == 2 && idx.pq_dim % 64 == 0 && res.tune.pq_wide_blocks != 0 && hb.bound_tmp != nullptr;
  auto bound = [&](auto lut_tag, auto acc_tag) {
    constexpr int LUT = decltype(lut_tag)::value;
    constexpr bool ACC = decltype(acc_tag)::value;
    if (bblocks) {
      HIP_TRY(hipMemsetAsync(hb.bound_tmp, 0, (size_t)2 * r.nq * sizeof(uint32_t), res.stream));
      const size_t smb = (size_t)64 * 2 * idx.pq_book * sizeof(float);
      auto kb = pqw_bound_blocks_kernel<LUT, ACC>;
      HIP_TRY(hipFuncSetAttribute(reinterpret_cast<const void*>(kb), hipFuncAttributeMaxDynamicSharedMemorySize, (int)smb));
      const unsigned gb = (unsigned)std::min<int64_t>(pq3_grid(res), grid_blocks(r.nq * (int64_t)r.k, kRBThreads * kRBItems));
      hipLaunchKernelGGL(kb, dim3(gb), dim3(kRBThreads), smb, res.stream, b, hb.bound_tmp);
      hipLaunchKernelGGL(pqw_bound_finish_kernel, bgrid, dim3(256), 0, res.stream, b, hb.bound_tmp);
      return;
    }
    const size_t sm = 4 * wave_score_tile<LUT, ACC>::kBytes;
    auto kern = pqw_head_bound_kernel<LUT, ACC>;
    HIP_TRY(hipFuncSetAttribute(reinterpret_cast<const void*>(kern), hipFuncAttributeMaxDynamicSharedMemorySize, (int)sm));
    hipLaunchKernelGGL(kern, bgrid, dim3(256), sm, res.stream, b);
  };
  using B0 = std::integral_constant<int, 0>; using B1 = std::integral_constant<int, 1>; using B2 = std::integral_constant<int, 2>;
  if (r.lut_mode == 0)      bound(B0{}, std::false_type{});
  else if (r.lut_mode == 1) { if (r.acc_half) bound(B1{}, std::true_type{}); else bound(B1{}, std::false_type{}); }
  else                      { if (r.acc_half) bound(B2{}, std::true_type{}); else bound(B2{}, std::false_type{}); }
  profile_end(res, "pq_head_kernel");
  profile_end(res, "pq_scan_kernel");
  HIP_TRY(hipGetLastError());
  return true;
}

void pqw_tail(resources& res, const ivf_pq_index& idx, const pq3_run& r, const pqw_bufs& hb)
{
  pq3_tables tb{};
  const void* rows16 = pqw_rows(res, idx, &tb);
  CUVS_EXPECTS(rows16 != nullptr, "ivf_pq: the wide path's decoded rows are gone between the head and the tail phase");
  profile_begin(res, "pq_scan_kernel");
  const float c1 = (r.is_ip ? -1.0f : -2.0f) / (tb.sc * tb.sc);
  float eps = 0.f, alpha = 0.f, bound_max = FLT_MAX;
  pqw_margins(idx, r, &eps, &alpha, &bound_max);
  wide_prep l{};
  l.sorted_pairs = r.sorted_pairs; l.pair_off = r.pair_off; l.n_lists = idx.n_lists; l.probes = r.probes; l.rot_queries = r.rot_queries;
  l.centers_rot = idx.centers_rot.data(); l.query_kth = r.query_kth; l.qflag = r.qflag; l.bq = r.bq; l.thr = r.thr; l.norms = nullptr;
  l.n_probes = r.n_probes; l.rot_dim = idx.rot_dim; l.heads = r.head; l.sc = tb.sc; l.c1 = c1; l.eps = eps; l.alpha = alpha;
  l.cbmax = tb.cbmax; l.dmax = tb.dmax; l.bound_max = bound_max; l.head = 0; l.n_pairs = r.nq * (int64_t)r.n_probes; l.blk_off = hb.blk_off; l.is_ip = r.is_ip;
  profile_begin(res, "pq_bprep_kernel");
  pqw_bprep(res, l);
  profile_end(res, "pq_bprep_kernel");
  auto* units = static_cast<filter_unit*>(r.units);
  hipLaunchKernelGGL(count_units_kernel, dim3(1), dim3(1024), 0, res.stream, r.pair_off, idx.n_lists, idx.list_sizes.data(), r.unit_rows,
                     r.unit_off, pqw_group(), idx.n_lists);
  hipLaunchKernelGGL(fill_units_kernel, dim3(grid_blocks(idx.n_lists, 256)), dim3(256), 0, res.stream, r.pair_off, idx.n_lists,
                     idx.list_offsets.data(), idx.list_sizes.data(), r.unit_rows, r.unit_off, units, pqw_group(), idx.n_lists);
  const unsigned grid = pq3_grid(res);
  wide_filter f{};
  f.units = units; f.n_units = r.unit_off + idx.n_lists; f.xcd_ticket = r.xcd_ticket; f.sorted_pairs = r.sorted_pairs; f.pair_off = r.pair_off;
  f.n_lists = idx.n_lists; f.bq = r.bq; f.blk_off = hb.blk_off; f.thr = r.thr; f.rows16 = rows16;
  f.row_term = r.is_ip ? nullptr : reinterpret_cast<const float*>(tb.row_term); f.zeros = idx.scan3.zeros.data();
  f.qflag = r.qflag; f.surv = r.surv; f.surv_cnt = r.surv_cnt; f.surv_cap = (uint32_t)((uint64_t)r.surv_cap * 3 / 4 / grid);
  f.spill_cap = r.surv_cap - f.surv_cap * grid; f.n_probes = r.n_probes; f.rot_dim = idx.rot_dim; f.xbuf = nullptr; f.ldx = 0; f.heads = r.head;
  f.emit = 0; f.grid = grid; f.stats = r.stats;
  pqw_filter(res, f);
  hipLaunchKernelGGL(pqw_head_survivors_kernel, dim3((unsigned)grid_blocks(r.nq * (int64_t)r.head, 4)), dim3(256), 0, res.stream, hb.xbuf, hb.ldx,
                     hb.thr_head, r.head, r.sorted_pairs, r.pair_off, idx.n_lists, r.probes, r.n_probes, idx.list_offsets.data(),
                     idx.list_sizes.data(), static_cast<uint2*>(r.surv), r.surv_cnt, grid, f.surv_cap, f.spill_cap, r.qflag);
  uint32_t nch8 = 0;
  const uint8_t* codes8 = pq3_codes(res, idx, &nch8);
  rescore_params s = pqw_score_inputs(idx, r, codes8, nch8);
  s.surv = static_cast<const uint2*>(r.surv); s.surv_cnt = r.surv_cnt; s.surv_cap = f.surv_cap; s.spill_cap = f.spill_cap;
  s.n_regions = grid; s.sub = 1u;
  s.query_kth = r.query_kth; s.qflag = r.qflag; s.qcnt = r.qcnt; s.cand_d = r.cand_d; s.cand_i = r.cand_i; s.cand_r = r.cand_r;
  s.head_rows = 0u; s.list_offsets = idx.list_offsets.data(); s.filter_bits = r.filter_bits; s.indices = idx.indices.data();
  s.overflow = static_cast<uint4*>(r.overflow); s.overflow_cnt = r.counters + 1; s.overflow_cap = r.overflow_cap; s.fail = nullptr;
  s.cb_lds = 0;
  const dim3 rg(grid, 8), rb(256);
  profile_begin(res, "pq_rescore_kernel");
  const bool blocks = idx.pq_len == 2 && idx.pq_dim % 64 == 0 && res.tune.pq_wide_blocks != 0;
  auto rescore = [&](auto lut_tag, auto acc_tag) {
    constexpr int LUT = decltype(lut_tag)::value;
    constexpr bool ACC = decltype(acc_tag)::value;
    if (blocks) {
      const size_t sm = (size_t)64 * 2 * idx.pq_book * sizeof(float) + ((size_t)grid + 3) * sizeof(uint32_t);
      auto kern = pq_rescore_blocks_kernel<LUT, ACC>;
      HIP_TRY(hipFuncSetAttribute(reinterpret_cast<const void*>(kern), hipFuncAttributeMaxDynamicSharedMemorySize, (int)sm));
      hipLaunchKernelGGL(kern, dim3(grid), dim3(kRBThreads), sm, res.stream, s);
      return;
    }
    const size_t sm = 4 * wave_score_tile<LUT, ACC>::kBytes + ((size_t)grid + 3) * sizeof(uint32_t);
    auto kern = pq_rescore_wave_kernel<LUT, ACC>;
    HIP_TRY(hipFuncSetAttribute(reinterpret_cast<const void*>(kern), hipFuncAttributeMaxDynamicSharedMemorySize, (int)sm));
    hipLaunchKernelGGL(kern, rg, rb, sm, res.stream, s);
  };
  using R0 = std::integral_constant<int, 0>; using R1 = std::integral_constant<int, 1>; using R2 = std::integral_constant<int, 2>;
  if (r.lut_mode == 0)      rescore(R0{}, std::false_type{});
  else if (r.lut_mode == 1) { if (r.acc_half) rescore(R1{}, std::true_type{}); else rescore(R1{}, std::false_type{}); }
  else                      { if (r.acc_half) rescore(R2{}, std::true_type{}); else rescore(R2{}, std::false_type{}); }
  profile_end(res, "pq_rescore_kernel");
  hipLaunchKernelGGL(reset_flagged_kernel, dim3((unsigned)r.nq), dim3(256), 0, res.stream, r.qflag, r.nq, r.n_probes, r.k, 0u, r.cand_d,
                     r.cand_i);
  hipLaunchKernelGGL(fallback_items_kernel, dim3(grid * 4), dim3(256), 0, res.stream, r.sorted_pairs, r.pair_off, idx.n_lists, r.probes,
                     r.n_probes, r.qflag, static_cast<work_item*>(r.fb_items), r.counters, 1);
  profile_end(res, "pq_scan_kernel");
  HIP_TRY(hipGetLastError());
}

void pq3_merge(resources& res, const pq3_run& r, float* top_d, uint32_t* top_i)
{
  auto* ov = static_cast<uint4*>(r.overflow);
  hipLaunchKernelGGL(ov_count_kernel, dim3(256), dim3(256), 0, res.stream, ov, r.counters + 1, r.overflow_cap, r.ov_cnt);
  hipLaunchKernelGGL(ov_scan_kernel, dim3(1), dim3(1024), 0, res.stream, r.ov_cnt, r.nq, r.ov_off);
  hipLaunchKernelGGL(ov_fill_kernel, dim3(256), dim3(256), 0, res.stream, ov, r.counters + 1, r.overflow_cap, r.ov_off, r.ov_cnt,
                     ov + r.overflow_cap);
  auto go = [&](auto kern) {
    hipLaunchKernelGGL(kern, dim3(grid_blocks(r.nq, 4)), dim3(256), 0, res.stream, r.cand_d, r.cand_i, r.cand_r, r.qcnt, r.qflag, r.nq,
                       r.n_probes, r.k, r.head, top_d, top_i, ov + r.overflow_cap, r.ov_off);
  };
  if (r.k <= 64)       go(pool_merge_kernel<1>);
  else if (r.k <= 128) go(pool_merge_kernel<2>);
  else if (r.k <= 192) go(pool_merge_kernel<3>);
  else                 go(pool_merge_kernel<4>);
}

}
```

### cuvs_amd/csrc/ivf_pq_scan3.hpp

```cpp
#pragma once
#include "ivf_pq.hpp"

namespace cuvs_amd {

struct pq3_tables {
  const uint32_t* cb16;
  const uint32_t* row_term;
  float sc, cbmax, dmax;
};

struct pq3_run {
  int64_t nq;
  uint32_t n_probes, k, head;
  int is_ip, lut_mode , acc_half;
  const uint32_t* sorted_pairs;
  const uint32_t* pair_off;
  const uint32_t* probes;
  const float* rot_queries;
  const float* rescore_queries = nullptr;
  int cosine = 0;
  const uint32_t* query_kth;
  float* cand_d;
  uint32_t* cand_i;
  uint32_t* cand_r;
  uint32_t* qflag;
  uint32_t* qcnt;
  uint32_t* counters;
  void* overflow;
  uint32_t overflow_cap;
  uint32_t* ov_cnt;
  uint32_t* ov_off;
  uint32_t* surv_cnt;
  void* surv;
  uint32_t surv_cap;
  void* units;
  uint32_t* unit_off;
  uint32_t unit_rows;
  uint32_t* xcd_ticket;
  void* fb_items;
  const uint32_t* filter_bits;
  uint32_t* fail;
  void* bq;
  float* thr;
  int filter_dbg;
  unsigned long long* stats;
  int stage = 0;
  void* pair_norms = nullptr;
  const float* hb_xbuf = nullptr;
  uint32_t hb_ldx = 0;
  const float* hb_thr = nullptr;
  uint32_t head_rows = 0;
};

struct pq3_head {
  const void* items;
  const uint32_t* item_begin;
  const uint32_t* item_end;
  uint32_t* xcd_ticket;
  const uint32_t* sorted_pairs;
  const float* rot_queries;
  float* cand_d;
  uint32_t* cand_i;
  uint32_t* query_kth;
  uint32_t n_probes, k, max_list_len;
  int is_ip, lut_mode, acc_half;
  const uint32_t* filter_bits;
  unsigned long long* stats;
  uint32_t one_shot = 0;
  uint32_t row_limit = 0;
};
int pq3_head_scan(resources& res, const ivf_pq_index& idx, const pq3_head& h);

struct flat3_cache {
  dev_buf<uint4> rows16;
  dev_buf<uint32_t> row_term;
  dev_buf<float> row_term32;
  dev_buf<float> zeros;
  float sc = 1.f, maxres = 0.f, maxnorm = 0.f;
  const void* data_ptr = nullptr;
  int64_t rows = -1, size = -1;
  const void* failed_ptr = nullptr;
  int64_t failed_rows = -1, failed_size = -1;
};
struct flat3_view {
  const uint8_t* data;
  const float* centers;
  const uint32_t* list_offsets;
  const uint32_t* list_sizes;
  const int64_t* indices;
  uint32_t n_lists, dim, n_chunks;
  int64_t padded_rows, size;
  uint32_t max_list_len;
  int elem;
  bool unit_rows = false;
};
bool flat3_supported(uint32_t dim, int k);
bool flat3_wide(uint32_t dim);
bool flat3_tail(resources& res, const flat3_view& v, flat3_cache& cache, const pq3_run& r);
struct flat3_head_bufs {
  float* xbuf; uint32_t ldx;
  float* kth_val; uint32_t* kth_idx;
  float* thr_head;
  void* norms;
  uint32_t* tickets;
};
bool flat3_head_bounds(resources& res, const flat3_view& v, flat3_cache& cache, const pq3_run& r, const flat3_head_bufs& hb);

unsigned pq3_grid(const resources& res);
unsigned pq3_regions(const resources& res);
bool pq3_supported(const ivf_pq_index& idx, int k);
bool pq3_bound_useful(const ivf_pq_index& idx, int k);
size_t pq3_max_units(const ivf_pq_index& idx, int64_t n_pairs, uint32_t* unit_rows, bool filter4);
void pq3_warm(resources& res, const ivf_pq_index& idx, bool filter4);
void pq3_tail(resources& res, const ivf_pq_index& idx, const pq3_run& r);
void pq3_merge(resources& res, const pq3_run& r, float* top_d, uint32_t* top_i);

bool pqw_supported(const ivf_pq_index& idx, int k);
uint32_t pqw_heads(const ivf_pq_index& idx, int k, uint32_t n_probes);
bool pqw_ready(resources& res, const ivf_pq_index& idx);
struct pqw_bufs {
  float* xbuf; uint32_t ldx;
  float* kth_val; uint32_t* kth_idx;
  float* thr_head;
  float* head_c;
  void* norms;
  uint32_t* tickets;
  uint32_t* blk_off;
  uint32_t* bound_tmp;
};
bool pqw_head_bounds(resources& res, const ivf_pq_index& idx, const pq3_run& r, const pqw_bufs& hb);
void pqw_tail(resources& res, const ivf_pq_index& idx, const pq3_run& r, const pqw_bufs& hb);

}
```

### cuvs_amd/csrc/ivf_pq_search.hip

```cpp
#include "ivf_pq.hpp"
#include "ops.hpp"
#include "device_utils.hpp"
#include "ivf_common.hpp"
#include "ivf_lists.hpp"
#include "pq_lut_math.hpp"
#include "ivf_pq_scan3.hpp"

#include <cuvs/neighbors/ivf_pq.h>

#include <cfloat>
#include <cstdlib>
#include <functional>
#include <mutex>
#include <type_traits>

namespace cuvs_amd {
extern unsigned long long g_pq3_last_stats[6];

namespace {

constexpr int kScanThreads = 1024;
constexpr int kScanWaves   = kScanThreads / 64;
constexpr int kQueueRows   = 320;

// ... 1794 lines not shown
  int64_t max_batch = 0, bs_alloc = 0, n_pairs_max = 0, max_items = 0;
  uint32_t surv_cap = 0, overflow_cap = 0, unit_rows = 0;
  size_t max_units = 0;
  bool all_scores() const { return path == pq_path::all_scores; }
  bool mc_tail() const { return path == pq_path::matrix_core_tail || path == pq_path::wide; }
  int lut_mode() const { return lut_fp8 ? 2 : (lut_half ? 1 : 0); }
};

bool pq_mc_tail_eligible(const ivf_pq_index& idx, int k, const tuning& tune)
{
  return pq3_supported(idx, k) && pq3_bound_useful(idx, k) && tune.pq_scan3 != 0 &&
         ((idx.pq_len == 2 && idx.codebook_kind == 0) || tune.pq_filter4 != 0);
}

pq_search_plan make_pq_search_plan(const ivf_pq_index& idx, const ivf_pq_search_params& p, int k, int64_t n_queries,
                                          const tuning& tune, int num_cus, size_t ivf_batch_limit, size_t largest_total,
                                          const std::function<bool()>& wide_rows_ready)
{
  pq_search_plan pl;
  const uint32_t n_probes = pl.n_probes = std::min<uint32_t>(p.n_probes, idx.n_lists);
  pl.lut_fp8          = p.lut_dtype == 8 || p.lut_dtype == 3;
  pl.acc_half         = p.lut_dtype != 0 && p.internal_distance_dtype == 2;
  pl.lut_half         = pl.lut_fp8 ? pl.acc_half : p.lut_dtype != 0;
  pl.bits8            = idx.pq_bits == 8 && idx.pq_dim == 64;
  const bool large_k  = k > 256;
  pl.big_k            = k > 64 && !large_k;
  pl.k_scan           = large_k ? 1 : k;
  pl.grid             = (unsigned)std::max(8, num_cus / 8 * 8);
  pl.largest_total    = largest_total;
  const size_t lds_cap = 160 * 1024;

  int qpb = 0;
  size_t smem = 0;
  if (!pl.lut_half) {
    if ((smem = scan_smem_bytes<float, float, 2>(idx, pl.k_scan)) <= lds_cap) qpb = 2;
    else if ((smem = scan_smem_bytes<float, float, 1>(idx, pl.k_scan)) <= lds_cap) qpb = 1;
  } else {
    if ((smem = scan_smem_bytes<__half, float, 4>(idx, pl.k_scan)) <= lds_cap) qpb = 4;
    else if ((smem = scan_smem_bytes<__half, float, 2>(idx, pl.k_scan)) <= lds_cap) qpb = 2;
    else if ((smem = scan_smem_bytes<__half, float, 1>(idx, pl.k_scan)) <= lds_cap) qpb = 1;
  }
  pl.glut = qpb == 0;
  if (pl.glut) {
    qpb  = pl.lut_half ? 4 : 2;
    smem = scan_layout(0, qpb, idx.rot_dim, (uint32_t)pl.k_scan).total;
    CUVS_EXPECTS(smem <= lds_cap, "ivf_pq::search: rot_dim %u / k %d do not fit 160 KiB of LDS", idx.rot_dim, pl.k_scan);
    pl.glut_stride = ((size_t)idx.pq_dim * idx.pq_book * 8  + 255) & ~size_t(255);
  }
  pl.qpb  = qpb;
  pl.smem = smem;

  const bool mc_ok = pq_mc_tail_eligible(idx, k, tune);
  if (!large_k && n_probes > 8 && n_queries >= 256 && tune.pq_scan3 != 0 && tune.pq_wide != 0 && tune.pq_head_probes < 0 &&
      idx.shard_world <= 1 && idx.shard_comm == nullptr && pqw_supported(idx, k) && !mc_ok) {
    pl.wheads = tune.pq_wide_heads > 0 ? std::min<uint32_t>((uint32_t)tune.pq_wide_heads, n_probes / 2) : pqw_heads(idx, k, n_probes);
    if (pl.wheads > 0 && !wide_rows_ready()) pl.wheads = 0;
  }
  const bool usew = pl.wheads > 0;
  for (uint32_t v : idx.h_list_sizes) pl.max_list_len = std::max(pl.max_list_len, v);
  pl.w_ldx = usew ? (uint32_t)round_up((int64_t)pl.max_list_len + 64, 64) : 0u;
  int64_t max_batch = std::max<uint32_t>(1, p.max_internal_batch_size);
  {
    int64_t per_q = (int64_t)idx.n_lists * 4 + (int64_t)n_probes * pl.k_scan * 8 + (int64_t)idx.rot_dim * 4 + idx.dim * 4;
    if (large_k) per_q += (int64_t)largest_total * 8;
    if (!large_k && (pq3_supported(idx, k) || usew) && tune.pq_scan3 != 0)
      per_q += (int64_t)n_probes * ((int64_t)idx.rot_dim * 2 + (int64_t)k * 4 + 128 + 16 + 4 + 16 + 8);
    if (usew) per_q += (int64_t)pl.wheads * ((int64_t)pl.w_ldx * 4 + 32) + (int64_t)k * (8 + 32 * 8);
    int64_t fit   = std::max<int64_t>(1, (int64_t)ivf_batch_limit / per_q);
    max_batch     = balanced_batch(n_queries, std::min(max_batch, fit));
  }
  pl.max_batch   = max_batch;
  pl.bs_alloc    = std::min<int64_t>(max_batch, n_queries);
  pl.n_pairs_max = pl.bs_alloc * n_probes;
  uint32_t head = (n_probes > 8 && n_queries >= 256 && !large_k) ? 1u : 0u;
  if (tune.pq_head_probes >= 0) head = std::min<uint32_t>((uint32_t)tune.pq_head_probes, n_probes);
  const bool metric_ip = idx.metric == M_InnerProduct || idx.metric == M_CosineExpanded;
  if (metric_ip && !(mc_ok && tune.pq_head_probes != 0)) head = 0;
  if (usew) head = pl.wheads;
  pl.head = head;
  const bool sharded = idx.shard_world > 1;
  pl.n_ranges        = head > 0 ? 2 * idx.n_lists : idx.n_lists;
  pl.n_labels        = pl.n_ranges + (sharded ? 1u : 0u);
  pl.max_items = pl.n_pairs_max / qpb + pl.bs_alloc * (int64_t)head + pl.n_labels + 1;
  const bool use3 = !usew && head > 0 && mc_ok;
  pl.filter4      = use3 && tune.pq_filter4 != 0 && (idx.metric != M_InnerProduct || idx.pq_len != 2 || idx.codebook_kind != 0);
  if (usew || use3) {
    pl.max_units = pq3_max_units(idx, pl.n_pairs_max, &pl.unit_rows, pl.filter4);
    pl.surv_cap  = (uint32_t)std::min<int64_t>(std::max<int64_t>(pl.n_pairs_max * 16, 1 << 22), 1 << 28);
    if (usew) pl.surv_cap = (uint32_t)std::min<int64_t>(std::max<int64_t>((int64_t)pl.surv_cap, pl.bs_alloc * (int64_t)k * 32), 1 << 28);
    if (tune.pq3_surv_cap > 0) pl.surv_cap = (uint32_t)tune.pq3_surv_cap;
    pl.overflow_cap = tune.pq3_surv_cap > 0 ? (uint32_t)tune.pq3_surv_cap : (1u << 22);
  }
  pl.overlap = use3 && pl.filter4 && head == 1 && !pl.glut && tune.pq_overlap != 0;
  if (pl.overlap && tune.pq_head_rows >= 0) {
    pl.head_rows = (uint32_t)tune.pq_head_rows / 64u * 64u;
    if (pl.head_rows != 0u && pl.head_rows < 4u * (uint32_t)k) pl.head_rows = 0u;
  }
  const bool use2 = head > 0 && pl.bits8 && idx.pq_len == 2 && idx.codebook_kind == 0 && k <= 64 &&
                    ((pl.lut_half && qpb == 4) || (!pl.lut_half && qpb == 2)) && tune.pq_scan2 != 0 && !(use3 || usew);
  pl.head1 = (use3 && !pl.glut) ||
             (usew && !pl.glut && idx.rot_dim <= 256  && (size_t)idx.pq_dim * 256 * (pl.lut_half ? 2 : 4) <= 96 * 1024);
  pl.shard_coarse = idx.shard_comm != nullptr && p.coarse_search_dtype == 0 && !tune.shard_coarse_replicated;
  pl.path = large_k ? pq_path::all_scores
          : usew    ? pq_path::wide
          : use3    ? pq_path::matrix_core_tail
          : head == 0 ? pq_path::lut_one_phase
          : use2    ? pq_path::scan2_tail
                    : pq_path::lut_two_phase;
  return pl;
}

struct pq_search_scratch {
  dev_buf<float> qf, rot_q, qc;
  dev_buf<uint32_t> probes, sorted_pairs, pair_off, item_off, phase_labels;
  dev_buf<work_item> items;
  dev_buf<float> cand_d;
  dev_buf<uint32_t> cand_i, pair_seg;
  dev_buf<float> top_d;
  dev_buf<uint32_t> top_i, query_kth, tickets;
  dev_buf<uint32_t> cand_r, qstate, unit_off;
  dev_buf<uint2> surv;
  dev_buf<uint4> units3, overflow3;
  dev_buf<work_item> fb_items;
  dev_buf<uint4> bq3;
  dev_buf<float> thr3;
  dev_buf<float> w_x, w_kv, w_thr, w_c;
  dev_buf<uint32_t> w_ki, w_blk, w_bt;
  dev_buf<float4> w_nm;
  dev_buf<work_item> hitems;
  dev_buf<uint32_t> hpairs;
  dev_buf<float4> pair_norms;
  dev_buf<uint32_t> group_scratch;
  dev_buf<char> glut_buf;
  dev_buf<unsigned long long> stats;

  pq_search_scratch(resources& res, const ivf_pq_index& idx, const ivf_pq_search_params& p, const pq_search_plan& pl, int k)
  {
    const size_t bs = (size_t)pl.bs_alloc, np = (size_t)pl.n_pairs_max, nl = idx.n_lists;
    const bool mc = pl.mc_tail(), w = pl.path == pq_path::wide, ov = pl.overlap, f4w = pl.filter4 || w;
    const size_t wh = w ? bs * pl.wheads : 0, scores = pl.all_scores() ? bs * pl.largest_total : np * k;
    qf = dev_buf<float>(res, bs * idx.dim); rot_q = dev_buf<float>(res, bs * idx.rot_dim);
    qc = dev_buf<float>(res, p.coarse_search_dtype != 0 ? bs * idx.dim : 0);
    probes = dev_buf<uint32_t>(res, np + (size_t)std::max(1, idx.shard_world) * pl.n_probes);
    sorted_pairs = dev_buf<uint32_t>(res, np);
    pair_off = dev_buf<uint32_t>(res, pl.n_labels + 1); item_off = dev_buf<uint32_t>(res, pl.n_labels + 1);
    phase_labels = dev_buf<uint32_t>(res, (pl.head > 0 || idx.shard_world > 1) ? np : 0);
    items = dev_buf<work_item>(res, (size_t)pl.max_items);
    cand_d = dev_buf<float>(res, scores); cand_i = dev_buf<uint32_t>(res, scores);
    pair_seg = dev_buf<uint32_t>(res, pl.all_scores() ? np : 0);
    top_d = dev_buf<float>(res, bs * k); top_i = dev_buf<uint32_t>(res, bs * k);
    query_kth = dev_buf<uint32_t>(res, bs); tickets = dev_buf<uint32_t>(res, 4 * 8 * 32);
    cand_r = dev_buf<uint32_t>(res, mc ? np * k : 0); qstate = dev_buf<uint32_t>(res, mc ? 4 * bs + 8 + pq3_regions(res) : 0);
    unit_off = dev_buf<uint32_t>(res, mc ? nl + 1 : 0); surv = dev_buf<uint2>(res, pl.surv_cap);
    units3 = dev_buf<uint4>(res, 2 * pl.max_units); overflow3 = dev_buf<uint4>(res, (size_t)2 * pl.overflow_cap);
    fb_items = dev_buf<work_item>(res, mc ? np : 0);
    bq3 = dev_buf<uint4>(res, f4w ? (np + (w ? (size_t)32 * (nl + 1) : 0)) * (idx.rot_dim / 8) : 0);
    thr3 = dev_buf<float>(res, f4w ? np : 0);
    w_x = dev_buf<float>(res, w ? bs * pl.wheads * pl.w_ldx : 0); w_kv = dev_buf<float>(res, w ? bs * k : 0);
    w_thr = dev_buf<float>(res, wh); w_c = dev_buf<float>(res, wh);
    w_ki = dev_buf<uint32_t>(res, w ? bs * k : 0); w_blk = dev_buf<uint32_t>(res, w ? nl + 1 : 0);
    w_bt = dev_buf<uint32_t>(res, w ? 2 * bs : 0); w_nm = dev_buf<float4>(res, wh);
    hitems = dev_buf<work_item>(res, ov ? bs : 0); hpairs = dev_buf<uint32_t>(res, ov ? bs + 1 : 0);
    pair_norms = dev_buf<float4>(res, ov ? np : 0); group_scratch = dev_buf<uint32_t>(res, ov ? np + pl.n_labels + 1 : 0);
    glut_buf = dev_buf<char>(res, pl.glut_stride * pl.grid);
    stats = dev_buf<unsigned long long>(res, (res.tune.scan_debug & (128 | 512)) ? (size_t)ST_COUNT * pl.grid * kScanWaves : 0);
  }
};

struct aux_fork_guard {
  hipStream_t s = nullptr;
  bool armed    = false;
  ~aux_fork_guard() { if (armed && s != nullptr) (void)hipStreamSynchronize(s); }
};

struct pq_search_ctx {
  resources& res;
  resources& gres;
  const ivf_pq_search_params& p;
  const ivf_pq_index& idx;
  const pq_search_plan& pl;
  pq_search_scratch& s;
  aux_fork_guard& fork_guard;
  int k;
  const uint32_t* filter_bits;
};

void report_head_stats(resources& res, const unsigned long long* d_stats, int wgs_per_cu)
{
  auto hs = to_host(res, d_stats, 8);
  const double n = (double)std::max<unsigned long long>(1, hs[5]);
  fprintf(stderr, "[pq_head] items %llu; workgroup cycles per item: header %.0f, LUT %.0f, scores %.0f, select %.0f, output %.0f; "
          "workgroups per CU %d\n", hs[5], hs[0] / n, hs[1] / n, hs[2] / n, hs[3] / n, hs[4] / n, wgs_per_cu);
}

void report_filter_stats(resources& res, const unsigned long long* d_stats, const uint32_t* counters)
{
  auto hs = to_host(res, d_stats, 8);
  g_pq3_last_stats[0] = hs[0]; g_pq3_last_stats[1] = hs[1]; g_pq3_last_stats[2] = hs[2]; g_pq3_last_stats[3] = hs[7];
  fprintf(stderr, "[pq_scan3] units %llu; wave cycles per unit: prologue %.0f, loop %.0f (slow path %.0f); per subtile %.0f\n", hs[7],
          (double)hs[4] / std::max<unsigned long long>(1, hs[7]), (double)hs[5] / std::max<unsigned long long>(1, hs[7]),
          (double)hs[6] / std::max<unsigned long long>(1, hs[7]), (double)hs[5] / std::max<unsigned long long>(1, hs[2]));
  auto hc = to_host(res, counters, 2);
  g_pq3_last_stats[4] = hc[0]; g_pq3_last_stats[5] = hc[1];
  fprintf(stderr, "[pq_scan3] overflow entries %u\n", hc[1]);
  hc[1] = hc[0];
  fprintf(stderr, "[pq_scan3] pairs screened %llu, survivors %llu (%.4f%%), subtiles %llu (slow path %llu), fallback pairs %u\n",
          hs[0], hs[1], 100.0 * hs[1] / (double)std::max<unsigned long long>(1, hs[0]), hs[2], hs[3], hc[1]);
}

void report_scan_stats(resources& res, const dev_buf<unsigned long long>& stats, unsigned grid, int dbg)
{
  std::vector<unsigned long long> hw(stats.n);
  HIP_TRY(hipMemcpyAsync(hw.data(), stats.data(), stats.bytes(), hipMemcpyDeviceToHost, res.stream));
  HIP_TRY(hipStreamSynchronize(res.stream));
  unsigned long long h[ST_COUNT] = {};
  for (size_t i = 0; i < hw.size(); ++i) h[i % ST_COUNT] += hw[i];
  const double w = 1.0 / (16.0 * grid);
  if (dbg & 4096) {
    for (int which : {(int)ST_SCAN, (int)ST_ALIVE2, (int)ST_F_GATHER, (int)ST_F_FLUSH, (int)ST_STAGE2, (int)ST_CAND, (int)ST_S2_CALLS}) {
      fprintf(stderr, "[pq_scan per-wave stat %d, Mcycles]", which);
      for (int wv = 0; wv < kScanWaves; ++wv) {
        unsigned long long t = 0;
        for (unsigned b = 0; b < grid; ++b) t += hw[((size_t)b * kScanWaves + wv) * ST_COUNT + which];
        fprintf(stderr, " %.2f", (double)t / grid * 1e-6);
      }
      fprintf(stderr, "\n");
    }
  }
  fprintf(stderr,
          "[pq_scan stats] items %llu rows %llu queued %llu (%.2f%%) stage2 calls %llu alive after chunk1/2/3 %llu/%llu/%llu"
          " | cycles per wave: header %.3g lut %.3g scan %.3g (stage2 %.3g) merge+sync %.3g\n",
          h[ST_ITEMS], h[ST_ROWS], h[ST_QUEUED], 100.0 * h[ST_QUEUED] / (double)std::max<unsigned long long>(1, h[ST_ROWS]),
          h[ST_S2_CALLS], h[ST_ALIVE1], h[ST_ALIVE2], h[ST_ALIVE3], h[ST_HEADER] * w, h[ST_LUT] * w, h[ST_SCAN] * w,
          h[ST_STAGE2] * w, (double)(h[ST_MERGE] - h[ST_HEADER] - h[ST_LUT] - h[ST_SCAN]) * w);
  fprintf(stderr, "[pq_scan2 waits, cycles per wave] after filter LUT %.3g, after filter pass %.3g, before LUT B %.3g, after exact LUT "
          "%.3g, after exact pass %.3g, merge %.3g | filter pass: code-load wait %.3g, gather block %.3g, flush %.3g\n",
          h[ST_ALIVE1] * w, h[ST_ALIVE2] * w, h[ST_S2_CALLS] * w, h[ST_ALIVE3] * w, h[ST_CAND] * w, h[ST_MERGE] * w,
          h[ST_F_LOAD] * w, h[ST_F_GATHER] * w, h[ST_F_FLUSH] * w);
}

void launch_lut_scan(resources& res, const pq_search_plan& pl, const scan_args& a, bool tail = false)
{
  const unsigned grid = pl.grid;
  if (tail && pl.path == pq_path::scan2_tail) {
    if (!pl.lut_half)      launch_scan2<float, float, 2, 4>(res, a, grid);
    else if (!pl.acc_half) launch_scan2<__half, float, 4, 2>(res, a, grid);
    else                   launch_scan2<__half, __half, 4, 2>(res, a, grid);
    return;
  }
  const size_t smem = pl.smem;
  const bool bits8 = pl.bits8, big_k = pl.big_k;
  if (pl.glut) {
    if (!pl.lut_half)      launch_scan_glut<float, float, 2>(res, a, smem, grid, big_k);
    else if (!pl.acc_half) launch_scan_glut<__half, float, 4>(res, a, smem, grid, big_k);
    else                   launch_scan_glut<__half, __half, 4>(res, a, smem, grid, big_k);
    return;
  }
  if (!pl.lut_half) {
    if (pl.qpb == 2) launch_scan_qpb<float, float, 2>(res, a, smem, grid, bits8, big_k);
    else             launch_scan_qpb<float, float, 1>(res, a, smem, grid, bits8, big_k);
  } else if (!pl.acc_half) {
    if (pl.qpb == 4)      launch_scan_qpb<__half, float, 4>(res, a, smem, grid, bits8, big_k);
    else if (pl.qpb == 2) launch_scan_qpb<__half, float, 2>(res, a, smem, grid, bits8, big_k);
    else                  launch_scan_qpb<__half, float, 1>(res, a, smem, grid, bits8, big_k);
  } else {
    if (pl.qpb == 4)      launch_scan_qpb<__half, __half, 4>(res, a, smem, grid, bits8, big_k);
    else if (pl.qpb == 2) launch_scan_qpb<__half, __half, 2>(res, a, smem, grid, bits8, big_k);
    else                  launch_scan_qpb<__half, __half, 1>(res, a, smem, grid, bits8, big_k);
  }
}

void launch_head_scan(const pq_search_ctx& c, const scan_args& sa)
{
  pq3_head h{};
  h.items = sa.items; h.item_begin = sa.item_begin; h.item_end = sa.item_end; h.xcd_ticket = sa.xcd_ticket;
  h.sorted_pairs = sa.sorted_pairs; h.rot_queries = sa.rot_queries; h.cand_d = sa.out_d; h.cand_i = sa.out_i;
  h.query_kth = sa.query_kth; h.n_probes = c.pl.n_probes; h.k = (uint32_t)c.k; h.max_list_len = c.pl.max_list_len; h.is_ip = sa.is_ip;
  h.lut_mode = c.pl.lut_mode(); h.acc_half = c.pl.acc_half ? 1 : 0; h.filter_bits = c.filter_bits;
  h.one_shot = sa.one_shot; h.row_limit = sa.row_limit;
  dev_buf<unsigned long long> hst(c.res, (sa.dbg & 2048) ? 8 : 0);
  if (sa.dbg & 2048) HIP_TRY(hipMemsetAsync(hst.data(), 0, hst.bytes(), c.res.stream));
  h.stats = hst.data();
  const int wgs_per_cu = pq3_head_scan(c.res, c.idx, h);
  if (sa.dbg & 2048) report_head_stats(c.res, hst.data(), wgs_per_cu);
}

void run_filter_tail(const pq_search_ctx& c, scan_args a, int64_t nq)
{
  resources& res = c.res;
  const pq_search_plan& pl = c.pl;
  pq_search_scratch& s = c.s;
  const int64_t bs = pl.bs_alloc;
  const bool wide = pl.path == pq_path::wide;
  HIP_TRY(hipMemsetAsync(s.qstate.data(), 0, s.qstate.bytes(), res.stream));
  pq3_run r{};
  r.pair_norms = s.pair_norms.data(); r.head_rows = pl.head_rows;
  r.nq = nq; r.n_probes = pl.n_probes; r.k = (uint32_t)c.k; r.head = pl.head; r.is_ip = a.is_ip;
  r.lut_mode = pl.lut_mode(); r.acc_half = pl.acc_half ? 1 : 0;
  r.sorted_pairs = s.sorted_pairs.data(); r.pair_off = s.pair_off.data(); r.probes = s.probes.data();
  r.rot_queries = s.rot_q.data(); r.query_kth = s.query_kth.data();
  r.cand_d = s.cand_d.data(); r.cand_i = s.cand_i.data(); r.cand_r = s.cand_r.data();
  r.qflag = s.qstate.data(); r.qcnt = s.qstate.data() + bs; r.counters = s.qstate.data() + 2 * bs;
  r.surv_cnt = s.qstate.data() + 2 * bs + 2;
  r.ov_cnt = s.qstate.data() + 2 * bs + 4 + pq3_regions(res); r.ov_off = r.ov_cnt + bs;
  r.surv = s.surv.data(); r.surv_cap = pl.surv_cap; r.units = s.units3.data(); r.unit_off = s.unit_off.data();
  r.unit_rows = pl.unit_rows; r.xcd_ticket = s.tickets.data() + 2 * 8 * 32; r.fb_items = s.fb_items.data();
  r.filter_bits = c.filter_bits; r.overflow = s.overflow3.data(); r.overflow_cap = pl.overflow_cap;
  r.bq = (pl.filter4 || wide) ? s.bq3.data() : nullptr; r.thr = s.thr3.data();
  dev_buf<unsigned long long> st3(res, (a.dbg & 1024) ? 8 : 0);
  if (a.dbg & 1024) HIP_TRY(hipMemsetAsync(st3.data(), 0, st3.bytes(), res.stream));
  r.stats = st3.data(); r.filter_dbg = (a.dbg >> 16) & 255;
  if (pl.overlap) {
    r.stage = 1;
    pq3_tail(c.gres, c.idx, r);
    HIP_TRY(hipEventRecord(res.aux_events[1], c.gres.stream));
    HIP_TRY(hipStreamWaitEvent(res.stream, res.aux_events[1], 0));
    c.fork_guard.armed = false;
    r.stage = 2;
  }
  if (wide) {
    const pqw_bufs hb{s.w_x.data(), pl.w_ldx, s.w_kv.data(), s.w_ki.data(), s.w_thr.data(), s.w_c.data(), s.w_nm.data(),
                      s.tickets.data(), s.w_blk.data(), s.w_bt.data()};
    const bool ok = pqw_head_bounds(res, c.idx, r, hb);
    CUVS_EXPECTS(ok, "ivf_pq: the wide path's decoded rows are gone");
    pqw_tail(res, c.idx, r, hb);
  } else {
    pq3_tail(res, c.idx, r);
  }
  a.items = s.fb_items.data(); a.item_begin = nullptr; a.item_end = r.counters;
  a.xcd_ticket = s.tickets.data() + 3 * 8 * 32;
  if (pl.head1) launch_head_scan(c, a); else launch_lut_scan(res, pl, a);
  pq3_merge(res, r, s.top_d.data(), s.top_i.data());
  if (a.dbg & 1024) report_filter_stats(res, st3.data(), r.counters);
}

void pq_search_batch(const pq_search_ctx& c, const void* queries, elem_t et, int64_t q0, int64_t nq, int64_t* neighbors,
                            float* distances)
{
  resources& res = c.res;
  const ivf_pq_index& idx = c.idx;
  const pq_search_plan& pl = c.pl;
  pq_search_scratch& s = c.s;
  const int k = c.k;
  const uint32_t n_probes = pl.n_probes;
  const int64_t n_pairs = nq * n_probes;
  load_range_as_float(res, queries, et, false , idx.dim, q0, nq, s.qf.data());
  if (idx.metric == M_CosineExpanded) normalize_rows(res, s.qf.data(), nq, idx.dim);
  if (pl.shard_coarse) {
    const int64_t slice = (nq + idx.shard_world - 1) / idx.shard_world;
    const int64_t s0    = std::min<int64_t>(nq, (int64_t)idx.shard_rank * slice);
    const int64_t s1    = std::min<int64_t>(nq, s0 + slice);
    if (s1 > s0)
      select_clusters(res, idx, s.qf.data() + s0 * idx.dim, s1 - s0, n_probes,
                      s.probes.data() + (size_t)idx.shard_rank * slice * n_probes, 0, s.qc.data());
    shard_allgather_inplace_u32(res, idx.shard_comm, s.probes.data(), (size_t)slice * n_probes);
  } else {
    select_clusters(res, idx, s.qf.data(), nq, n_probes, s.probes.data(), c.p.coarse_search_dtype, s.qc.data());
  }
  rotate_queries(res, idx, s.qf.data(), s.qc.data(), nq, c.p.coarse_search_dtype, s.rot_q.data());
  if (c.p.coarse_search_dtype != 0 && idx.metric == M_CosineExpanded) normalize_rows(res, s.rot_q.data(), nq, idx.rot_dim);
  const uint32_t* labels = s.probes.data();
  if (pl.overlap) {
    pq3_warm(res, idx, true);
    HIP_TRY(hipEventRecord(res.aux_events[0], res.stream));
    HIP_TRY(hipStreamWaitEvent(c.gres.stream, res.aux_events[0], 0));
    c.fork_guard.armed = true;
  }
  if (pl.head > 0 || idx.shard_world > 1) {
    hipLaunchKernelGGL(phase_labels_kernel, dim3(nblk(n_pairs, 256)), dim3(256), 0, c.gres.stream, s.probes.data(),
                       n_pairs, n_probes, pl.head, idx.n_lists, s.phase_labels.data(), (uint32_t)idx.shard_world,
                       (uint32_t)idx.shard_rank, pl.n_ranges, idx.list_owner.data(), pl.head_rows != 0u);
    labels = s.phase_labels.data();
  }
  build_work_items(c.gres, labels, n_pairs, pl.n_labels, pl.head1 ? 1 : pl.qpb, s.sorted_pairs.data(), s.pair_off.data(),
                   s.item_off.data(), s.items.data(), (int)idx.n_lists, pl.path == pq_path::scan2_tail ? 8 : pl.qpb,
                   pl.overlap ? s.group_scratch.data() : nullptr,
                   pl.n_ranges , n_probes, nq);
  if (pl.overlap)
    hipLaunchKernelGGL(head_items_kernel, dim3(nblk(nq, 256)), dim3(256), 0, res.stream, s.probes.data(), nq, n_probes,
                       (uint32_t)idx.shard_world, (uint32_t)idx.shard_rank, idx.list_owner.data(), s.hitems.data(), s.hpairs.data(),
                       s.hpairs.data() + pl.bs_alloc);
  HIP_TRY(hipMemsetAsync(s.query_kth.data(), 0xff, (size_t)nq * sizeof(uint32_t), res.stream));
  HIP_TRY(hipMemsetAsync(s.tickets.data(), 0, s.tickets.bytes(), res.stream));
  const size_t scores_ld = pl.largest_total;
  if (pl.mc_tail()) {
    hipLaunchKernelGGL(init_head_rows_kernel, dim3(nblk(nq * (int64_t)pl.head * k, 256)), dim3(256), 0, res.stream, s.cand_d.data(),
                       s.cand_i.data(), nq, (int64_t)n_probes * k, (uint32_t)(pl.head * k));
  } else if (!pl.all_scores()) {
    HIP_TRY(hipMemsetD32Async(reinterpret_cast<hipDeviceptr_t>(s.cand_d.data()), 0x7f7fffff, (size_t)n_pairs * k, res.stream));
    HIP_TRY(hipMemsetAsync(s.cand_i.data(), 0xff, (size_t)n_pairs * k * sizeof(uint32_t), res.stream));
  } else {
    HIP_TRY(hipMemsetD32Async(reinterpret_cast<hipDeviceptr_t>(s.cand_d.data()), 0x7f7fffff, (size_t)nq * scores_ld, res.stream));
    HIP_TRY(hipMemsetAsync(s.cand_i.data(), 0xff, (size_t)nq * scores_ld * sizeof(uint32_t), res.stream));
    hipLaunchKernelGGL(pair_segments_kernel, dim3(nblk(nq, 256)), dim3(256), 0, res.stream, s.probes.data(),
                       idx.list_sizes.data(), nq, n_probes, s.pair_seg.data());
  }
  scan_args a;
  a.query_kth = s.query_kth.data();
  a.items = s.items.data(); a.sorted_pairs = s.sorted_pairs.data(); a.n_lists = idx.n_lists;
  a.rot_queries = s.rot_q.data(); a.centers_rot = idx.centers_rot.data(); a.pq_centers = idx.pq_centers.data();
  a.per_cluster = idx.codebook_kind == 1;
  a.codes = idx.codes.data(); a.list_offsets = idx.list_offsets.data(); a.list_sizes = idx.list_sizes.data();
  a.out_d = s.cand_d.data(); a.out_i = s.cand_i.data();
  a.all_scores = pl.all_scores() ? s.cand_d.data() : nullptr; a.all_rows = s.cand_i.data(); a.pair_seg = s.pair_seg.data();
  a.scores_ld = scores_ld;
  a.n_probes = n_probes; a.rot_dim = idx.rot_dim; a.pq_dim = idx.pq_dim; a.pq_len = idx.pq_len;
  a.pq_bits = idx.pq_bits; a.n_chunks = idx.n_chunks; a.cpc = idx.codes_per_chunk; a.k = (uint32_t)pl.k_scan;
  a.is_ip = idx.metric == M_InnerProduct || idx.metric == M_CosineExpanded;
  a.lut_fp8 = pl.lut_fp8 ? 1 : 0;
  a.dbg   = res.tune.scan_debug;
  a.qcap  = (uint32_t)std::max(0, res.tune.pq_qcap);
  a.filter_bits = c.filter_bits; a.indices = idx.indices.data();
  a.stats = s.stats.data();
  if (a.dbg & (128 | 512)) HIP_TRY(hipMemsetAsync(s.stats.data(), 0, s.stats.bytes(), res.stream));
  a.global_lut_stride = pl.glut_stride;
  a.global_lut = pl.glut ? s.glut_buf.data() : nullptr;
  a.xcd_ticket = s.tickets.data();
  a.item_begin = nullptr; a.item_end = s.item_off.data() + idx.n_lists;
  if (pl.head > 0) {
    if (pl.path == pq_path::wide) {
    } else if (pl.overlap) {
      scan_args ah = a;
      ah.items = s.hitems.data(); ah.sorted_pairs = s.hpairs.data(); ah.item_end = s.hpairs.data() + pl.bs_alloc;
      ah.one_shot = (uint32_t)nq;
      ah.row_limit = pl.head_rows;
      launch_head_scan(c, ah);
    } else if (pl.head1) launch_head_scan(c, a); else launch_lut_scan(res, pl, a);
    if (idx.shard_comm != nullptr) shard_allreduce_min_u32(res, idx.shard_comm, s.query_kth.data(), (size_t)nq);
    a.xcd_ticket = s.tickets.data() + 8 * 32;
    a.item_begin = s.item_off.data() + idx.n_lists;  a.item_end = s.item_off.data() + 2 * idx.n_lists;
    if (pl.mc_tail()) run_filter_tail(c, a, nq);
    else              launch_lut_scan(res, pl, a, true);
  } else {
    launch_lut_scan(res, pl, a);
  }
  if (a.dbg & (128 | 512)) report_scan_stats(res, s.stats, pl.grid, a.dbg);
  if (!pl.mc_tail()) {
    const int64_t row = pl.all_scores() ? (int64_t)scores_ld : (int64_t)n_probes * k;
    select_k<uint32_t, uint32_t>(res, s.cand_d.data(), s.cand_i.data(), nq, row, row, k, s.top_d.data(), s.top_i.data(), true);
  }
  const float sc = ivf_pq_index::scale(et);
  hipLaunchKernelGGL(postprocess_kernel, dim3(nblk(nq * k, 256)), dim3(256), 0, res.stream, s.top_i.data(),
                     s.top_d.data(), nq * k, idx.indices.data(), idx.metric, sc * sc, neighbors + q0 * k,
                     distances + q0 * k);
}

}

void ivf_pq_search(resources& res, const ivf_pq_search_params& p, const ivf_pq_index& idx, const void* queries,
                   elem_t et, int64_t n_queries, int k, int64_t* neighbors, float* distances, const uint32_t* filter_bits)
{
  CUVS_EXPECTS(k > 0, "parameter `k` in top-k must be positive.");
  CUVS_EXPECTS((int64_t)k <= idx.size || idx.shard_world > 1,
               "parameter `k` (%d) in top-k must not be larger that the total size of the index (%ld)", k,
               (long)idx.size);
  CUVS_EXPECTS(p.n_probes > 0, "n_probes (number of clusters to probe in the search) must be positive.");
  CUVS_EXPECTS(p.internal_distance_dtype == 0 || p.internal_distance_dtype == 2,
               "internal_distance_dtype must be either CUDA_R_16F or CUDA_R_32F");
  CUVS_EXPECTS(p.lut_dtype == 0 || p.lut_dtype == 2 || p.lut_dtype == 8 || p.lut_dtype == 3,
               "lut_dtype must be CUDA_R_16F, CUDA_R_32F, CUDA_R_8U or CUDA_R_8I");
  CUVS_EXPECTS(p.coarse_search_dtype == 0 || p.coarse_search_dtype == 2 || p.coarse_search_dtype == 3,
               "Unsupported coarse_search_dtype (only CUDA_R_32F, CUDA_R_16F, and CUDA_R_8I are supported)");
  CUVS_EXPECTS(!idx.dtype_known || et == idx.dtype, "queries dtype differs from the index dtype");
  if (n_queries == 0) return;
  if (idx.shard_comm != nullptr && !idx.shard_stats_valid) shard_exchange_stats(res, idx);
  const bool large_k   = k > 256;
  size_t largest_total = large_k ? largest_lists_total(idx.h_list_sizes, std::min<uint32_t>(p.n_probes, idx.n_lists)) : 0;
  if (large_k && idx.shard_comm != nullptr) {
    dev_buf<uint32_t> key(res, 1);
    const uint32_t mine = ~(uint32_t)std::min<size_t>(largest_total, 0xfffffffeu);
    copy_async(res, key.data(), &mine, sizeof(mine));
    shard_allreduce_min_u32(res, idx.shard_comm, key.data(), 1);
    largest_total = (size_t)~to_host(res, key.data(), 1)[0];
  }
  const pq_search_plan pl = make_pq_search_plan(idx, p, k, n_queries, res.tune, res.num_cus, res.ivf_batch_limit, largest_total,
                                                [&] { return pqw_ready(res, idx); });
  if (res.tune.scan_debug & 1024)
    fprintf(stderr, "[pq_wide] heads %u (supported %d, matrix-core tail of the narrow shapes %d, probes %u, queries %ld, k %d)\n", pl.wheads,
            (int)pqw_supported(idx, k), (int)(pq3_supported(idx, k) && pq3_bound_useful(idx, k)), pl.n_probes, (long)n_queries, k);
  pq_search_scratch scratch(res, idx, p, pl, k);
  resources aux = res;
  if (pl.overlap) {
    ensure_aux_stream(res);
    aux.aux_stream = res.aux_stream;
    aux.stream     = res.aux_stream;
  }
// ... 39 lines not shown
```

### include/cuvs_amd/extensions.h

```cpp
#pragma once
#include <cuvs/core/c_api.h>
#include <cuvs/core/export.h>
#include <cuvs/neighbors/all_neighbors.h>
#include <cuvs/neighbors/cagra.h>
#include <cuvs/neighbors/common.h>
#include <cuvs/neighbors/ivf_pq.h>
#include <cuvs/neighbors/tiered_index.h>
#include <cuvs/neighbors/vamana.h>
#include <cuvs/preprocessing/quantize/binary.h>
#include <cuvs/preprocessing/quantize/pq.h>
#include <stdint.h>

#ifdef __cplusplus
extern "C" {
#endif

CUVS_EXPORT cuvsError_t cuvsAmdIvfPqSearchFiltered(cuvsResources_t res, cuvsIvfPqSearchParams_t search_params,
                                                   cuvsIvfPqIndex_t index, DLManagedTensor* queries,
                                                   DLManagedTensor* neighbors, DLManagedTensor* distances,
                                                   cuvsFilter filter);

CUVS_EXPORT cuvsError_t cuvsAmdCagraWorkCounters(cuvsResources_t res, int enable, uint64_t out[3]);

CUVS_EXPORT cuvsError_t cuvsAmdCagraSetGuaranteeConnectivity(cuvsResources_t res, int on);

CUVS_EXPORT cuvsError_t cuvsAmdCagraOptimize(cuvsResources_t res, DLManagedTensor* knn_graph, DLManagedTensor* graph,
                                             int guarantee_connectivity);

CUVS_EXPORT cuvsError_t cuvsAmdCagraBuildKnnGraph(cuvsResources_t res, cuvsCagraIndexParams_t params, DLManagedTensor* dataset,
                                                  DLManagedTensor* knn_graph);

CUVS_EXPORT cuvsError_t cuvsAmdCagraIndexGetVpqInfo(cuvsCagraIndex_t index, uint32_t out[5]);
CUVS_EXPORT cuvsError_t cuvsAmdCagraIndexGetVpq(cuvsResources_t res, cuvsCagraIndex_t index, DLManagedTensor* vq_book,
                                                DLManagedTensor* pq_book, DLManagedTensor* codes);

CUVS_EXPORT cuvsError_t cuvsAmdIvfPqIndexGetCodesLayout(cuvsIvfPqIndex_t index, int* layout);

CUVS_EXPORT cuvsError_t cuvsAmdBinaryQuantizerGetThreshold(cuvsResources_t res, cuvsBinaryQuantizer_t quantizer,
                                                           DLManagedTensor* out);

CUVS_EXPORT cuvsError_t cuvsAmdProductQuantizerFromCodebooks(cuvsResources_t res, cuvsProductQuantizerParams_t params,
                                                             DLManagedTensor* pq_codebook, DLManagedTensor* vq_codebook,
                                                             cuvsProductQuantizer_t quantizer);
CUVS_EXPORT void cuvsAmdPqEncodeCounters(unsigned long long out[3]);

CUVS_EXPORT cuvsError_t cuvsAmdAllNeighborsPartition(cuvsResources_t res, cuvsAllNeighborsIndexParams_t params,
                                                     DLManagedTensor* dataset_host, DLManagedTensor* centroids_out,
                                                     DLManagedTensor* nearest_clusters_out);
CUVS_EXPORT cuvsError_t cuvsAmdAllNeighborsMerge(cuvsResources_t res, DLManagedTensor* inverted_indices,
                                                 DLManagedTensor* batch_indices, DLManagedTensor* batch_distances,
                                                 DLManagedTensor* global_indices, DLManagedTensor* global_distances,
                                                 int select_min);

CUVS_EXPORT cuvsError_t cuvsAmdTieredIndexGetInfo(cuvsTieredIndex_t index, int64_t* size, int64_t* ann_rows, int64_t* capacity,
                                                  int64_t* dim);
CUVS_EXPORT cuvsError_t cuvsAmdTieredIndexCompact(cuvsResources_t res, cuvsTieredIndex_t index);
CUVS_EXPORT cuvsError_t cuvsAmdTieredIndexSearchTiers(cuvsResources_t res, void* search_params, cuvsTieredIndex_t index,
                                                      DLManagedTensor* queries, DLManagedTensor* ann_neighbors,
                                                      DLManagedTensor* ann_distances, DLManagedTensor* tail_neighbors,
                                                      DLManagedTensor* tail_distances, cuvsFilter prefilter);
CUVS_EXPORT cuvsError_t cuvsAmdTieredTailSearch(cuvsResources_t res, cuvsDistanceType metric, DLManagedTensor* tail, int64_t ann_rows,
                                                DLManagedTensor* queries, DLManagedTensor* seed_neighbors,
                                                DLManagedTensor* seed_distances, DLManagedTensor* bitset, int path,
                                                DLManagedTensor* neighbors, DLManagedTensor* distances);
CUVS_EXPORT cuvsError_t cuvsAmdTieredMerge(cuvsResources_t res, DLManagedTensor* a_neighbors, DLManagedTensor* a_distances,
                                           DLManagedTensor* b_neighbors, DLManagedTensor* b_distances, int64_t ann_rows,
                                           int select_min, DLManagedTensor* out_neighbors, DLManagedTensor* out_distances);
CUVS_EXPORT void cuvsAmdTieredCounters(unsigned long long out[3]);

CUVS_EXPORT cuvsError_t cuvsAmdVamanaIndexGetGraph(cuvsResources_t res, cuvsVamanaIndex_t index, DLManagedTensor* out);
CUVS_EXPORT cuvsError_t cuvsAmdVamanaIndexGetMedoid(cuvsVamanaIndex_t index, uint32_t* medoid);
CUVS_EXPORT cuvsError_t cuvsAmdVamanaGreedySearch(cuvsResources_t res, cuvsVamanaIndexParams_t params, DLManagedTensor* dataset,
                                                  DLManagedTensor* graph, uint32_t medoid, DLManagedTensor* query_ids,
                                                  DLManagedTensor* out_ids, DLManagedTensor* out_dists);
CUVS_EXPORT cuvsError_t cuvsAmdVamanaRobustPrune(cuvsResources_t res, cuvsVamanaIndexParams_t params, DLManagedTensor* dataset,
                                                 DLManagedTensor* graph, DLManagedTensor* node_ids, DLManagedTensor* cand_ids,
                                                 DLManagedTensor* cand_dists, DLManagedTensor* out_ids);
CUVS_EXPORT cuvsError_t cuvsAmdVamanaSerializeSectorAligned(cuvsResources_t res, const char* filename, cuvsVamanaIndex_t index,
                                                            bool include_dataset);

CUVS_EXPORT int cuvsAmdDebugSwitchesCompiledIn(void);
CUVS_EXPORT void cuvsAmdProfileEnable(int on);
CUVS_EXPORT int cuvsAmdProfileCollect(const char* name, double* total_ms);
CUVS_EXPORT void cuvsAmdIvfPqLastFilterStats(unsigned long long out[4]);
CUVS_EXPORT void cuvsAmdIvfPqLastFilterStats6(unsigned long long out[6]);

CUVS_EXPORT cuvsError_t cuvsAmdPcaLastSweeps(int* sweeps);

#ifdef __cplusplus
}
#endif
```

Before: 1.847 million queries/s.

## Order filter work units by estimated cost and stride them across XCD queues

Adds a single-block kernel that buckets the PQ filter work units by an estimated cost key (rows times a weight for the query-group count). It moves the expensive head units first and orders the rest by decreasing cost. The filter kernels then fetch units in a strided pattern across the eight per-XCD ticket queues rather than in contiguous chunks, so each XCD gets a balanced mix and long units start early. The aim is to cut the tail imbalance at the end of the scan. The cost is an extra serial single-block pass over all units, a second unit buffer, and extra stats instrumentation.

```diff
diff --git a/cuvs_amd/csrc/common.hpp b/cuvs_amd/csrc/common.hpp
--- a/cuvs_amd/csrc/common.hpp
+++ b/cuvs_amd/csrc/common.hpp
@@ -71,6 +71,7 @@
   int coarse_lowp       = 1;
   int pq_head_rows      = -1;
   int pq_overlap        = 1;
+  int pq_unit_order     = 2;
   int coarse_grouped    = 1;
   int pq_filter4        = 1;
   int flat_scan3        = 1;
diff --git a/cuvs_amd/csrc/core.hip b/cuvs_amd/csrc/core.hip
--- a/cuvs_amd/csrc/core.hip
+++ b/cuvs_amd/csrc/core.hip
@@ -176,6 +176,7 @@
   t.pq_filter4       = geti("CUVS_AMD_PQ_FILTER4", 1);
   t.coarse_grouped   = geti("CUVS_AMD_COARSE_GROUPED", 1);
   t.pq_overlap       = geti("CUVS_AMD_PQ_OVERLAP", 1);
+  t.pq_unit_order    = geti("CUVS_AMD_PQ_UNIT_ORDER", t.pq_unit_order);
   t.pq_head_rows     = geti("CUVS_AMD_PQ_HEAD_ROWS", -1);
   t.coarse_lowp      = geti("CUVS_AMD_COARSE_LOWP", 1);
   t.flat_scan3       = geti("CUVS_AMD_FLAT_SCAN3", 1);
diff --git a/cuvs_amd/csrc/ivf_pq_filter4.hip b/cuvs_amd/csrc/ivf_pq_filter4.hip
--- a/cuvs_amd/csrc/ivf_pq_filter4.hip
+++ b/cuvs_amd/csrc/ivf_pq_filter4.hip
@@ -125,6 +125,7 @@
   uint32_t* surv_cnt;
   uint32_t n_chunks, n_probes, unit_rows;
   unsigned long long* stats;
+  uint32_t strided;
 };
 
 template <int BYTE>
@@ -161,13 +162,16 @@
 
   const uint32_t lane = threadIdx.x & 63u, ql = lane & 31u, h = lane >> 5;
   const uint32_t n_units = *a.n_units;
-  const uint32_t chunk   = (n_units + 7u) / 8u;
+  const bool strided     = a.strided != 0u;
   const uint32_t s_base  = a.pair_off[a.n_lists];
   uint32_t xcd = blockIdx.x & 7u, hops = 0u;
   const uint32_t two = PL == 1 ? 1u : PL == 2 ? 2u : PL == 4 ? 3u : 4u;
   const uint32_t lane_code_off = ql * 16u + h * 8u, lane_term_off = h * 16u;
 
   unsigned long long st_pairs = 0, st_surv = 0, st_sub = 0, st_slow = 0, st_units = 0, st_t[3] = {0, 0, 0};
+  unsigned long long st_ng_t[4] = {0, 0, 0, 0}, st_ng_sub[4] = {0, 0, 0, 0};
+  const unsigned long long w_start = STATS ? wall_clock64() : 0ull;
+  unsigned long long w_end = w_start;
   uint32_t tk_v = 0u;
   uint4 d0 = {0u, 0u, 0u, 0u};
   uint2 d1 = {0u, 0u};
@@ -176,11 +180,10 @@
     if (lane == 0) tk_v = atomicAdd(a.xcd_ticket + xcd * 32, 1u);
   };
   auto load_desc = [&]() {
-    const uint32_t share0 = min(n_units, xcd * chunk), share_len = min(chunk, n_units - share0);
     const uint32_t t = __builtin_amdgcn_readfirstlane(tk_v);
-    desc_ok = t < share_len;
+    desc_ok = t < unit_share_len(n_units, xcd, strided);
     if (desc_ok) {
-      const filter_unit* up = a.units + share0 + t;
+      const filter_unit* up = a.units + unit_position(n_units, xcd, t, strided);
       d0 = *reinterpret_cast<const uint4*>(up);
       d1 = *reinterpret_cast<const uint2*>(reinterpret_cast<const char*>(up) + 16);
     }
@@ -457,6 +460,11 @@
       st_t[0] += t_loop - t_unit;
       st_t[1] += t_end - t_loop;
       st_units += 1u;
+      if (u0 < u1) {
+        const uint32_t gi = min((count + 31u) >> 5, (uint32_t)NGM) - 1u;
+        st_ng_t[gi] += t_end - t_loop; st_ng_sub[gi] += u1 - u0;
+      }
+      w_end = wall_clock64();
     }
   }
   if (STATS && lane == 0) {
@@ -464,6 +472,9 @@
     atomicAdd(&a.stats[0], st_pairs); atomicAdd(&a.stats[2], st_sub);
     atomicAdd(&a.stats[3], st_slow);  atomicAdd(&a.stats[4], st_t[0]); atomicAdd(&a.stats[5], st_t[1]);
     atomicAdd(&a.stats[6], st_t[2]);  atomicAdd(&a.stats[7], st_units);
+    for (int g = 0; g < 4; ++g) { atomicAdd(&a.stats[8 + g], st_ng_t[g]); atomicAdd(&a.stats[12 + g], st_ng_sub[g]); }
+    atomicMin(&a.stats[16], w_start); atomicMax(&a.stats[17], w_end);
+    atomicAdd(&a.stats[18], w_end - w_start); atomicAdd(&a.stats[19], 1ull);
   }
   if (s_chunk < a.n_chunks)
     for (uint32_t i = s_fill + lane; i < kSurvChunk; i += 64u) a.surv[(size_t)s_chunk * kSurvChunk + i] = make_uint2(0xffffffffu, 0u);
@@ -517,7 +528,7 @@
   g.n_lists = l.n_lists; g.bq = b.bq; g.thr = l.thr; g.cb16 = l.cb16; g.codes = l.codes; g.list_offsets = l.list_offsets;
   g.list_sizes = l.list_sizes; g.row_term = l.row_term; g.qflag = l.qflag; g.surv = static_cast<uint2*>(l.surv);
   g.surv_cnt = l.surv_cnt; g.n_chunks = l.surv_entries / kSurvChunk; g.n_probes = l.n_probes; g.unit_rows = l.unit_rows;
-  g.stats = l.stats;
+  g.stats = l.stats; g.strided = l.strided != 0 ? 1u : 0u;
   const size_t fsmem = l.per_cluster ? 4 * 4096 : 65536 + (size_t)l.nch * 8 * 512 * l.pl;
   const bool term = l.row_term != nullptr;
   auto launch = [&](auto kern) {
@@ -539,6 +550,7 @@
       case 81: launch(pq_filter4_kernel<4, 2, true, 81>); break;
       default:
         if (l.stats != nullptr && term) launch(pq_filter4_kernel<4, 2, true, 0, true>);
+        else if (l.stats != nullptr) launch(pq_filter4_kernel<4, 2, false, 0, true>);
         else if (term) launch(pq_filter4_kernel<4, 2, true, 0>);
         else launch(pq_filter4_kernel<4, 2, false, 0>);
         break;
@@ -550,6 +562,9 @@
     if (l.per_cluster) {
       if (term) launch(pq_filter4_kernel<N, P, true, 0, false, true>); else launch(pq_filter4_kernel<N, P, false, 0, false, true>);
     } else {
+      if constexpr (P == 2 && N <= 4) {
+        if (l.stats != nullptr && term) { launch(pq_filter4_kernel<N, P, true, 0, true>); return; }
+      }
       if (term) launch(pq_filter4_kernel<N, P, true, 0>); else launch(pq_filter4_kernel<N, P, false, 0>);
     }
   };
diff --git a/cuvs_amd/csrc/ivf_pq_filter_common.hpp b/cuvs_amd/csrc/ivf_pq_filter_common.hpp
--- a/cuvs_amd/csrc/ivf_pq_filter_common.hpp
+++ b/cuvs_amd/csrc/ivf_pq_filter_common.hpp
@@ -15,6 +15,32 @@
   uint32_t base_row, r_end;
   uint32_t pad0, pad1;
 };
+
+constexpr uint32_t kUnitKeys = 512u;
+__host__ __device__ inline uint32_t unit_group_weight(const uint32_t ng)
+{
+  return ng <= 1u ? 50u : ng == 2u ? 63u : ng == 3u ? 80u : 106u;
+}
+__host__ __device__ inline uint32_t unit_cost_key(const uint32_t rows, const uint32_t ng, const uint32_t unit_rows)
+{
+  if (rows == 0u) return 0u;
+  const uint64_t cost = (uint64_t)((rows + 31u) >> 5) * unit_group_weight(ng);
+  const uint64_t cmax = (uint64_t)(((unit_rows > rows ? unit_rows : rows) + 31u) >> 5) * unit_group_weight(4u);
+  const uint64_t k    = 1u + cost * (kUnitKeys - 2u) / cmax;
+  return (uint32_t)(k < kUnitKeys - 1u ? k : kUnitKeys - 1u);
+}
+__host__ __device__ inline uint32_t unit_share_len(const uint32_t n_units, const uint32_t xcd, const bool strided)
+{
+  if (strided) return (n_units - xcd + 7u) / 8u;
+  const uint32_t chunk = (n_units + 7u) / 8u, share0 = n_units < xcd * chunk ? n_units : xcd * chunk;
+  return chunk < n_units - share0 ? chunk : n_units - share0;
+}
+__host__ __device__ inline uint32_t unit_position(const uint32_t n_units, const uint32_t xcd, const uint32_t t, const bool strided)
+{
+  if (strided) return 8u * t + xcd;
+  const uint32_t chunk = (n_units + 7u) / 8u, share0 = n_units < xcd * chunk ? n_units : xcd * chunk;
+  return share0 + t;
+}
 
 template <typename P>
 __device__ inline float filter_threshold(const float bound, const float rn, const P& a)
@@ -72,6 +98,7 @@
   int flat = 0;
   int bprep_only = 0;
   int head_labels = 0;
+  int strided = 0;
 };
 void pq4_filter(resources& res, const filter4_launch& l);
 
diff --git a/cuvs_amd/csrc/ivf_pq_scan3.hip b/cuvs_amd/csrc/ivf_pq_scan3.hip
--- a/cuvs_amd/csrc/ivf_pq_scan3.hip
+++ b/cuvs_amd/csrc/ivf_pq_scan3.hip
@@ -152,6 +152,128 @@
   }
   const uint32_t w_end = unit_off[L] + ((e - b + group - 1u) / group) * n_ch;
   for (; w < w_end; ++w) units[w] = filter_unit{L, b, 1u, 0u, base, 0u, 0u, 0u};
+}
+
+constexpr uint32_t kOrdWaves = 8u, kOrdThreads = 64u * kOrdWaves;
+__global__ __launch_bounds__(512) __attribute__((amdgpu_waves_per_eu(6, 8))) void order_units_kernel(const filter_unit* __restrict__ in, const uint32_t* __restrict__ n_units,
+                                                           filter_unit* __restrict__ out, uint32_t unit_rows, int order)
+{
+  __shared__ uint32_t cnt[kOrdWaves][kUnitKeys];
+  __shared__ uint32_t head_pos[kOrdWaves];
+  __shared__ int scan_smem[17];
+  __shared__ uint32_t k_star_s;
+  const uint32_t n = *n_units;
+  const uint32_t lane = threadIdx.x & 63u, w = threadIdx.x >> 6;
+  const uint32_t per = (n + kOrdWaves * 64u - 1u) / (kOrdWaves * 64u) * 64u;
+  const uint32_t b = min(n, w * per), e = min(n, b + per);
+  for (uint32_t i = threadIdx.x; i < kOrdWaves * kUnitKeys; i += kOrdThreads) (&cnt[0][0])[i] = 0u;
+  if (threadIdx.x == 0) k_star_s = order == 1 ? kUnitKeys : 0u;
+  __syncthreads();
+  auto key_of = [&](const uint4 d0, const uint2 d1) {
+    return unit_cost_key(d1.y > d0.w ? d1.y - d0.w : 0u, (d0.z + 31u) >> 5, unit_rows);
+  };
+  constexpr uint32_t kOrdAhead = 4u;
+  static_assert(kUnitKeys <= kOrdThreads, "a thread per key in the scan of the costs");
+  for (uint32_t i0 = b; i0 < e; i0 += 64u * kOrdAhead) {
+    uint4 d0[kOrdAhead];
+    uint2 d1[kOrdAhead];
+#pragma unroll
+    for (uint32_t j = 0; j < kOrdAhead; ++j) {
+      const uint32_t i = min(i0 + j * 64u + lane, e - 1u);
+      d0[j] = *reinterpret_cast<const uint4*>(in + i);
+      d1[j] = *reinterpret_cast<const uint2*>(reinterpret_cast<const char*>(in + i) + 16);
+    }
+#pragma unroll
+    for (uint32_t j = 0; j < kOrdAhead; ++j)
+      if (i0 + j * 64u + lane < e) atomicAdd(&cnt[w][key_of(d0[j], d1[j])], 1u);
+  }
+  __syncthreads();
+  {
+    int v = 0;
+    if (threadIdx.x < kUnitKeys)
+      for (uint32_t ww = 0; ww < kOrdWaves; ++ww) v += (int)(cnt[ww][threadIdx.x] * threadIdx.x);
+    if (n > (1u << 21)) v = 0;
+    int total;
+    const int below = block_exclusive_scan(v, scan_smem, &total);
+    if (order == 2 && n <= (1u << 21) && threadIdx.x < kUnitKeys && (long long)below * 8 <= (long long)total)
+      atomicMax(&k_star_s, threadIdx.x);
+    __syncthreads();
+  }
+  const uint32_t k_star = k_star_s;
+  {
+    uint32_t s = 0;
+    for (uint32_t key = lane; key < kUnitKeys; key += 64u) s += key >= k_star ? cnt[w][key] : 0u;
+    for (uint32_t o = 32u; o > 0u; o >>= 1) s += __shfl_xor(s, o);
+    if (lane == 0) head_pos[w] = s;
+  }
+  __syncthreads();
+  {
+    constexpr uint32_t kPer = (kOrdWaves + kOrdWaves * kUnitKeys + kOrdThreads - 1u) / kOrdThreads;
+    uint32_t vals[kPer];
+    int sum = 0;
+#pragma unroll
+    for (uint32_t j = 0; j < kPer; ++j) {
+      const uint32_t s = threadIdx.x * kPer + j;
+      uint32_t v = 0u;
+      if (s < kOrdWaves) v = head_pos[s];
+      else if (s < kOrdWaves + kOrdWaves * kUnitKeys) {
+        const uint32_t key = kUnitKeys - 1u - (s - kOrdWaves) / kOrdWaves, ww = (s - kOrdWaves) % kOrdWaves;
+        v = key < k_star ? cnt[ww][key] : 0u;
+      }
+      vals[j] = v;
+      sum += (int)v;
+    }
+    int total;
+    uint32_t run = (uint32_t)block_exclusive_scan(sum, scan_smem, &total);
+#pragma unroll
+    for (uint32_t j = 0; j < kPer; ++j) {
+      const uint32_t s = threadIdx.x * kPer + j;
+      if (s < kOrdWaves) head_pos[s] = run;
+      else if (s < kOrdWaves + kOrdWaves * kUnitKeys) {
+        const uint32_t key = kUnitKeys - 1u - (s - kOrdWaves) / kOrdWaves, ww = (s - kOrdWaves) % kOrdWaves;
+        if (key < k_star) cnt[ww][key] = run;
+      }
+      run += vals[j];
+    }
+  }
+  __syncthreads();
+  volatile uint32_t* my_pos  = cnt[w];
+  volatile uint32_t* my_head = head_pos + w;
+  for (uint32_t i0 = b; i0 < e; i0 += 64u * kOrdAhead) {
+    uint4 a0[kOrdAhead], a1[kOrdAhead];
+#pragma unroll
+    for (uint32_t j = 0; j < kOrdAhead; ++j) {
+      const uint32_t i = min(i0 + j * 64u + lane, e - 1u);
+      a0[j] = reinterpret_cast<const uint4*>(in + i)[0];
+      a1[j] = reinterpret_cast<const uint4*>(in + i)[1];
+    }
+#pragma unroll
+    for (uint32_t j = 0; j < kOrdAhead; ++j) {
+      const uint4 d0 = a0[j], d1 = a1[j];
+      const bool valid = i0 + j * 64u + lane < e;
+      const uint32_t key = key_of(d0, make_uint2(d1.x, d1.y));
+      const uint32_t cls = !valid ? 2u * kUnitKeys - 1u : key >= k_star ? kUnitKeys : key;
+      unsigned long long peers = ~0ull;
+#pragma unroll
+      for (uint32_t bit = 0; (1u << bit) < 2u * kUnitKeys; ++bit) {
+        const bool mine = ((cls >> bit) & 1u) != 0u;
+        const unsigned long long m = __ballot(mine);
+        peers &= mine ? m : ~m;
+      }
+      const uint32_t rank = (uint32_t)__popcll(peers & ((1ull << lane) - 1ull)), same = (uint32_t)__popcll(peers);
+      uint32_t base = 0u;
+      if (valid) base = cls == kUnitKeys ? *my_head : my_pos[key];
+      __builtin_amdgcn_wave_barrier();
+      if (valid && rank == 0u) {
+        if (cls == kUnitKeys) *my_head = base + same; else my_pos[key] = base + same;
+      }
+      __builtin_amdgcn_wave_barrier();
+      if (valid) {
+        reinterpret_cast<uint4*>(out + base + rank)[0] = d0;
+        reinterpret_cast<uint4*>(out + base + rank)[1] = d1;
+      }
+    }
+  }
 }
 
 struct filter_params {
@@ -189,6 +311,7 @@
   uint32_t n_lists;
   float* xbuf;
   uint32_t ldx, lbase;
+  uint32_t strided;
 };
 
 template <int NCH, int DBG, bool FLAT = false>
@@ -211,23 +334,22 @@
   const uint32_t* cbh = cb + h * (8u * 256u);
 
   const uint32_t n_units = *a.n_units;
-  const uint32_t chunk = (n_units + 7u) / 8u;
+  const bool strided = a.strided != 0u;
   uint32_t xcd = blockIdx.x & 7u, hops = 0u;
   const uint4* codes16 = reinterpret_cast<const uint4*>(a.codes);
 
   unsigned long long st_pairs = 0, st_surv = 0, st_sub = 0, st_slow = 0, st_units = 0, st_t[3] = {0, 0, 0};
   for (;;) {
-    const uint32_t share0 = min(n_units, xcd * chunk), share_len = min(chunk, n_units - share0);
-    const filter_unit* share = a.units + share0;
     uint32_t t = 0;
     if (lane == 0) t = atomicAdd(a.xcd_ticket + xcd * 32, 1u);
     t = __builtin_amdgcn_readfirstlane(t);
-    if (t >= share_len) {
+    if (t >= unit_share_len(n_units, xcd, strided)) {
       if (++hops == 8u) break;
       xcd = (xcd + 1u) & 7u;
       continue;
     }
-    const uint4 uu = *reinterpret_cast<const uint4*>(share + t);
+    const filter_unit* const unit = a.units + unit_position(n_units, xcd, t, strided);
+    const uint4 uu = *reinterpret_cast<const uint4*>(unit);
     const uint32_t L = __builtin_amdgcn_readfirstlane(uu.x), first = __builtin_amdgcn_readfirstlane(uu.y),
                    count = __builtin_amdgcn_readfirstlane(uu.z), row0 = __builtin_amdgcn_readfirstlane(uu.w);
     const uint32_t base_row = a.list_offsets[L], len = a.list_sizes[L];
@@ -286,7 +408,7 @@
     const u32x4_t oq   = {h == 0u ? 0x3c003c00u : 0u, 0u, 0u, 0u};
     const f16x8_t ones = __builtin_bit_cast(f16x8_t, oq);
 
-    const uint32_t r_end = __builtin_amdgcn_readfirstlane(share[t].r_end);
+    const uint32_t r_end = __builtin_amdgcn_readfirstlane(unit->r_end);
     const uint32_t u0 = row0 >> 5, u1 = (r_end + 31u) >> 5;
     auto load_codes = [&](const uint32_t u, uint2 (&cw)[NCH]) {
       const uint32_t fr = base_row + (min(u, u1 - 1u) << 5) + ql;
@@ -2461,8 +2583,15 @@
     hipLaunchKernelGGL(fill_units_kernel, dim3(grid_blocks(idx.n_lists, 256)), dim3(256), 0, res.stream, r.pair_off, idx.n_lists,
                        idx.list_offsets.data(), idx.list_sizes.data(), r.unit_rows, r.unit_off, units, group, idx.n_lists);
   }
+  const bool ordered = r.unit_order != 0 && r.units_ord != nullptr;
+  if (ordered) {
+    if (r.stage != 2)
+      hipLaunchKernelGGL(order_units_kernel, dim3(1), dim3(kOrdThreads), 0, res.stream, units, r.unit_off + idx.n_lists,
+                         static_cast<filter_unit*>(r.units_ord), r.unit_rows, r.unit_order);
+    units = static_cast<filter_unit*>(r.units_ord);
+  }
   filter_params f{};
-  f.units = units; f.n_units = r.unit_off + idx.n_lists; f.xcd_ticket = r.xcd_ticket;
+  f.units = units; f.n_units = r.unit_off + idx.n_lists; f.xcd_ticket = r.xcd_ticket; f.strided = ordered ? 1u : 0u;
   f.sorted_pairs = r.sorted_pairs; f.rot_queries = r.rot_queries; f.centers_rot = idx.centers_rot.data();
   uint32_t nch8 = 0;
   const uint8_t* codes8 = pq3_codes(res, idx, &nch8);
@@ -2493,7 +2622,7 @@
     l.cbmax = f.cbmax; l.dmax = f.dmax; l.bound_max = f.bound_max; l.is_ip = r.is_ip; l.dbg = r.filter_dbg; l.nch = nch;
     l.pl = (int)idx.pq_len; l.per_cluster = idx.codebook_kind != 0 ? 1 : 0;
     l.n_pairs = r.nq * (int64_t)r.n_probes; l.stats = r.stats; l.grid = grid;
-    l.stage = r.stage; l.pair_norms = r.pair_norms;
+    l.stage = r.stage; l.pair_norms = r.pair_norms; l.strided = ordered ? 1 : 0;
     pq4_filter(res, l);
     if (r.stage == 1) return;
   } else {
@@ -3101,3 +3230,12 @@
 }
 
 }
+
+extern "C" __attribute__((visibility("default"))) void cuvsAmdIvfPqUnitOrderHook(uint32_t rows, uint32_t groups, uint32_t unit_rows,
+                                                                                 uint32_t n_units, uint32_t xcd, uint32_t t,
+                                                                                 int strided, uint32_t out[3])
+{
+  out[0] = cuvs_amd::unit_cost_key(rows, groups, unit_rows);
+  out[1] = cuvs_amd::unit_share_len(n_units, xcd, strided != 0);
+  out[2] = cuvs_amd::unit_position(n_units, xcd, t, strided != 0);
+}
diff --git a/cuvs_amd/csrc/ivf_pq_scan3.hpp b/cuvs_amd/csrc/ivf_pq_scan3.hpp
--- a/cuvs_amd/csrc/ivf_pq_scan3.hpp
+++ b/cuvs_amd/csrc/ivf_pq_scan3.hpp
@@ -8,6 +8,8 @@
   const uint32_t* row_term;
   float sc, cbmax, dmax;
 };
+
+constexpr int kPq3Stats = 24;
 
 struct pq3_run {
   int64_t nq;
@@ -36,6 +38,8 @@
   void* units;
   uint32_t* unit_off;
   uint32_t unit_rows;
+  int unit_order = 0;
+  void* units_ord = nullptr;
   uint32_t* xcd_ticket;
   void* fb_items;
   const uint32_t* filter_bits;
diff --git a/cuvs_amd/csrc/ivf_pq_search.hip b/cuvs_amd/csrc/ivf_pq_search.hip
--- a/cuvs_amd/csrc/ivf_pq_search.hip
+++ b/cuvs_amd/csrc/ivf_pq_search.hip
@@ -1970,7 +1970,7 @@
     query_kth = dev_buf<uint32_t>(res, bs); tickets = dev_buf<uint32_t>(res, 4 * 8 * 32);
     cand_r = dev_buf<uint32_t>(res, mc ? np * k : 0); qstate = dev_buf<uint32_t>(res, mc ? 4 * bs + 8 + pq3_regions(res) : 0);
     unit_off = dev_buf<uint32_t>(res, mc ? nl + 1 : 0); surv = dev_buf<uint2>(res, pl.surv_cap);
-    units3 = dev_buf<uint4>(res, 2 * pl.max_units); overflow3 = dev_buf<uint4>(res, (size_t)2 * pl.overflow_cap);
+    units3 = dev_buf<uint4>(res, (res.tune.pq_unit_order != 0 && !w ? 4 : 2) * pl.max_units); overflow3 = dev_buf<uint4>(res, (size_t)2 * pl.overflow_cap);
     fb_items = dev_buf<work_item>(res, mc ? np : 0);
     bq3 = dev_buf<uint4>(res, f4w ? (np + (w ? (size_t)32 * (nl + 1) : 0)) * (idx.rot_dim / 8) : 0);
     thr3 = dev_buf<float>(res, f4w ? np : 0);
@@ -2013,8 +2013,17 @@
 
 void report_filter_stats(resources& res, const unsigned long long* d_stats, const uint32_t* counters)
 {
-  auto hs = to_host(res, d_stats, 8);
+  auto hs = to_host(res, d_stats, kPq3Stats);
   g_pq3_last_stats[0] = hs[0]; g_pq3_last_stats[1] = hs[1]; g_pq3_last_stats[2] = hs[2]; g_pq3_last_stats[3] = hs[7];
+  if (hs[19] != 0) {
+    fprintf(stderr, "[pq_scan3] wave cycles per subtile at 1 / 2 / 3 / 4 query groups: %.0f / %.0f / %.0f / %.0f (subtiles %llu / %llu / %llu / %llu)\n",
+            (double)hs[8] / std::max<unsigned long long>(1, hs[12]), (double)hs[9] / std::max<unsigned long long>(1, hs[13]),
+            (double)hs[10] / std::max<unsigned long long>(1, hs[14]), (double)hs[11] / std::max<unsigned long long>(1, hs[15]),
+            hs[12], hs[13], hs[14], hs[15]);
+    const double span = (double)(hs[17] - hs[16]);
+    fprintf(stderr, "[pq_scan3] waves %llu, first ticket to last unit's end %.0f ticks of the real-time counter, tail idle share %.4f\n", hs[19],
+            span, 1.0 - (double)hs[18] / std::max(1.0, (double)hs[19] * span));
+  }
   fprintf(stderr, "[pq_scan3] units %llu; wave cycles per unit: prologue %.0f, loop %.0f (slow path %.0f); per subtile %.0f\n", hs[7],
           (double)hs[4] / std::max<unsigned long long>(1, hs[7]), (double)hs[5] / std::max<unsigned long long>(1, hs[7]),
           (double)hs[6] / std::max<unsigned long long>(1, hs[7]), (double)hs[5] / std::max<unsigned long long>(1, hs[2]));
@@ -2125,8 +2134,15 @@
   r.unit_rows = pl.unit_rows; r.xcd_ticket = s.tickets.data() + 2 * 8 * 32; r.fb_items = s.fb_items.data();
   r.filter_bits = c.filter_bits; r.overflow = s.overflow3.data(); r.overflow_cap = pl.overflow_cap;
   r.bq = (pl.filter4 || wide) ? s.bq3.data() : nullptr; r.thr = s.thr3.data();
-  dev_buf<unsigned long long> st3(res, (a.dbg & 1024) ? 8 : 0);
-  if (a.dbg & 1024) HIP_TRY(hipMemsetAsync(st3.data(), 0, st3.bytes(), res.stream));
+  if (res.tune.pq_unit_order != 0 && !wide) {
+    r.unit_order = res.tune.pq_unit_order;
+    r.units_ord  = s.units3.data() + 2 * pl.max_units;
+  }
+  dev_buf<unsigned long long> st3(res, (a.dbg & 1024) ? kPq3Stats : 0);
+  if (a.dbg & 1024) {
+    HIP_TRY(hipMemsetAsync(st3.data(), 0, st3.bytes(), res.stream));
+    HIP_TRY(hipMemsetAsync(st3.data() + 16, 0xff, sizeof(unsigned long long), res.stream));
+  }
   r.stats = st3.data(); r.filter_dbg = (a.dbg >> 16) & 255;
   if (pl.overlap) {
     r.stage = 1;
@@ -2150,6 +2166,11 @@
   if (pl.head1) launch_head_scan(c, a); else launch_lut_scan(res, pl, a);
   pq3_merge(res, r, s.top_d.data(), s.top_i.data());
   if (a.dbg & 1024) report_filter_stats(res, st3.data(), r.counters);
+  if ((a.dbg & 1024) && (a.dbg & (1 << 24))) {
+    const auto off = to_host(res, r.pair_off + c.idx.n_lists, (size_t)c.idx.n_lists + 1);
+    fprintf(stderr, "[pq_units] unit_rows %u\n", pl.unit_rows);
+    for (uint32_t L = 0; L < c.idx.n_lists; ++L) fprintf(stderr, "[pq_units] %u %u\n", c.idx.h_list_sizes[L], off[L + 1] - off[L]);
+  }
 }
 
 void pq_search_batch(const pq_search_ctx& c, const void* queries, elem_t et, int64_t q0, int64_t nq, int64_t* neighbors,
diff --git a/include/cuvs_amd/extensions.h b/include/cuvs_amd/extensions.h
--- a/include/cuvs_amd/extensions.h
+++ b/include/cuvs_amd/extensions.h
@@ -84,6 +84,8 @@
 CUVS_EXPORT int cuvsAmdProfileCollect(const char* name, double* total_ms);
 CUVS_EXPORT void cuvsAmdIvfPqLastFilterStats(unsigned long long out[4]);
 CUVS_EXPORT void cuvsAmdIvfPqLastFilterStats6(unsigned long long out[6]);
+CUVS_EXPORT void cuvsAmdIvfPqUnitOrderHook(uint32_t rows, uint32_t groups, uint32_t unit_rows, uint32_t n_units, uint32_t xcd,
+                                           uint32_t t, int strided, uint32_t out[3]);
 
 CUVS_EXPORT cuvsError_t cuvsAmdPcaLastSweeps(int* sweeps);
 
```

Measured after the change: 1.889 million queries/s (median of 6 runs). +2.3%, better.
